# Amanda-Zheng/MR-GNAS

Hardware: AMD Instinct MI355X
Metric: million edges/sec per supernet fwd+bwd step (FB15k-237, dim=200) (higher is better)
Workload: dtype f32

## Files before the change

### include/mrgnas.h

```cpp
#ifndef MRGNAS_H
#define MRGNAS_H

#include <stdint.h>

#ifdef __cplusplus
extern "C" {
#endif

#define MRG_ABI_VERSION 23

#define MRG_OK            0
#define MRG_E_NULLPTR    -1
#define MRG_E_SHAPE      -2
#define MRG_E_ENUM       -3
#define MRG_E_WORKSPACE  -4

#define MRG_COMPOSE_MULT 0
#define MRG_COMPOSE_SUB  1
#define MRG_COMPOSE_ADD  2
#define MRG_REDUCE_SUM   0
#define MRG_REDUCE_MEAN  1
#define MRG_REDUCE_MAX   2
#define MRG_GCS_SUB      0
#define MRG_GCS_MUL      1
#define MRG_GCS_COPY     2
#define MRG_GCS_NEGS     3
#define MRG_GCS_CCORR    4
#define MRG_GCS_CCONV    5
#define MRG_ACT_NONE     0
#define MRG_ACT_RELU     1
#define MRG_ACT_SIGMOID  2

int mrg_abi_version(void);
const char *mrg_error_string(int code);
const char *mrg_target_arch(void);

int mrg_compose_fwd(int op, const float *s, const float *hr, float *out,
                    int64_t rows, int D, void *stream);
int mrg_compose_bwd(int op, const float *gout, const float *s, const float *hr,
                    float *gs, float *ghr, int64_t rows, int D, void *stream);

int mrg_gather_compose_fwd(int op, const float *ent, const float *rel,
                           const int32_t *ent_idx, const int32_t *rel_idx,
                           float *out, int64_t rows, int D, void *stream);

#define MRG_GATE_LD(D) (2 * (D) + 4)

int mrg_gate_collapse3(const float *const *W_host, const float *const *b_host, const float *const *a_host, float *uvc,
                       int D, int in_dim, int fold, void *stream);
int mrg_gate_param_grad3(const float *const *W_host, const float *const *b_host, const float *const *a_host,
                         const float *d_uvc, float *const *gW_host, float *const *gb_host, float *const *ga_host,
                         int D, int in_dim, int fold, void *stream);
int mrg_fold_halves3(const float *const *W_host, float *Wt, int D, void *stream);
int mrg_unfold_halves3(const float *const *gWt_host, float *const *gW_host, int D, void *stream);

int mrg_gate_fwd(const float *s, const float *s_in, const float *norm, const float *uvc,
                 float *out, int64_t b0, int64_t b1, int64_t M, int D, float scale, void *stream);
int64_t mrg_gate_bwd_workspace_bytes(int64_t M, int D);
int mrg_gate_bwd(const float *gout, const float *s, const float *s_in, const float *norm,
                 const float *uvc, float *gs, float *gs_in, float *d_uvc, void *ws,
                 int64_t b0, int64_t b1, int64_t M, int D, float scale, void *stream);
int mrg_gate_row_fwd(const float *s, const float *s_in, const float *norm, const float *uvc, float *fvec, float *hvec,
                     int64_t b0, int64_t b1, int64_t M, int D, float scale, void *stream);
int64_t mrg_gate_row_colsum_blocks(int64_t b0, int64_t b1, int64_t M, int D, int vec4);
int mrg_gate_row_fwd_colsum(const float *s, const float *s_in, const float *norm, const float *uvc, float *fvec, float *hvec,
                            int64_t b0, int64_t b1, int64_t M, int D, float scale, void *stream, double *colsum, int64_t colsum_blocks);
int mrg_gate_row_bwd(const float *q, const float *hvec, const float *s, const float *s_in, const float *uvc, float *gs_in, float *d_uvc,
                     void *ws, int64_t b0, int64_t b1, int64_t M, int D, void *stream);

int64_t mrg_seg_reduce_workspace_bytes(int64_t n_slots, int D);
int mrg_seg_reduce_fwd(int mode, const float *msg, const float *self_rows,
                       const int32_t *eid,
                       const int32_t *chunk_node, const int32_t *chunk_start, const int32_t *chunk_end,
                       const int32_t *chunk_slot, int64_t n_chunks,
                       const int32_t *hub_node, const int32_t *hub_first, const int32_t *hub_count, int64_t n_hubs,
                       int64_t n_slots, const int32_t *in_degree,
                       float *out, int32_t *arg, void *ws,
                       int64_t N, int D, void *stream);
int mrg_seg_reduce_bwd(int mode, const float *gout, const int32_t *dst, const int32_t *in_degree,
                       const int32_t *arg, float *gmsg, float *gself, const float *relu_src,
                       int64_t E, int64_t N, int D, void *stream);
int mrg_seg_reduce_bwd_ordered(int mode, const float *gout, const int32_t *dst, const int32_t *in_degree, const int32_t *arg,
                               float *gmsg, float *gself, const float *relu_src, const unsigned *relu_bits, const int32_t *order,
                               int64_t E, int64_t N, int D, void *stream);
int mrg_segmax_bwd_input_ok(int D, int Kin);
int mrg_segmax_bwd_input(const float *gout, const float *mx, const int32_t *dst, const int32_t *arg, const float *W, float *gmsg,
                         float *gx, const int32_t *order, int64_t E, int64_t N, int D, int Kin, void *stream);

int64_t mrg_seg_std_workspace_bytes(int64_t n_slots, int D);
int mrg_seg_std_fwd(const float *msg, const int32_t *eid, const int32_t *chunk_node, const int32_t *chunk_start,
                    const int32_t *chunk_end, const int32_t *chunk_slot, int64_t n_chunks, const int32_t *hub_node,
                    const int32_t *hub_first, const int32_t *hub_count, int64_t n_hubs, int64_t n_slots,
                    const int32_t *in_degree, float *out, float *mean, float *coef, void *ws, int64_t N, int D, void *stream);
int mrg_seg_std_bwd(const float *gout, const float *msg, const int32_t *dst, const float *mean, const float *coef,
                    const int32_t *order, float *gmsg, int64_t E, int64_t N, int D, void *stream);

int mrg_fused_gcs(int mode, const float *X, const int32_t *xi, const float *Y, const int32_t *yi,
                  const float *scal, const int32_t *eid,
                  const int32_t *chunk_node, const int32_t *chunk_start, const int32_t *chunk_end,
                  const int32_t *chunk_slot, int64_t n_chunks,
                  const int32_t *hub_node, const int32_t *hub_first, const int32_t *hub_count, int64_t n_hubs,
                  int64_t n_slots, const int32_t *seg_len,
                  float *out, void *ws, int64_t nseg, int D, void *stream);

int mrg_span_gcs(int mode, const float *X, const float *Y, const void *meta, const float *ext_scal, int64_t E, int span,
                 const int32_t *span_slot, const int32_t *span_start, int64_t n_spans,
                 const int32_t *hub_seg, const int32_t *hub_first, const int32_t *hub_count, int64_t n_hubs,
                 int64_t n_slots, const int32_t *seg_len,
                 float *out, void *ws, int64_t nseg, int D, void *stream);

int mrg_sum_buffers(const float *const *xs_host, int K, float *out, int64_t n, int accumulate, void *stream);
int mrg_sum_rows_gather(const float *const *xs_host, int K, const float *gather_edge, const float *gather_self,
                        const int32_t *dst, int64_t E, int64_t rows, int D, float *out, void *stream);

int mrg_distmult_score(const float *ent, const float *rel, const int32_t *s_idx, const int32_t *r_idx,
                       const int32_t *o_idx, float *score, int64_t T, int D, void *stream);

int64_t mrg_mix_workspace_bytes(int K, int D);

int mrg_optim_chunk(void);
int mrg_clip_sgd_step(void *const *params, const void *const *grads, void *const *bufs, const int32_t *chunk_tensor,
                      const int64_t *chunk_off, const int32_t *chunk_len, int64_t n_chunks, double *partial, float *norm_coef,
                      float max_norm, float lr, float momentum, float weight_decay, void *stream);
int mrg_adam_step(void *const *params, const void *const *grads, void *const *exp_avg, void *const *exp_avg_sq, int64_t n_tensors,
                  const int32_t *chunk_tensor, const int64_t *chunk_off, const int32_t *chunk_len, int64_t n_chunks, float *step,
                  float *scal, const float *lr, double beta1, double beta2, float eps, float weight_decay, void *stream);
#define MRG_MIX_MAX_CANDIDATES 8
typedef struct mrg_gated_branch {
  int32_t k;
  const float *s;
  const float *rowscale;
  int32_t row_k;
  const float *row_f;
  const float *row_h;
  const float *row_uvc;
  int32_t row_ld;
  int64_t b0, b1;
  float *row_dq;
  int32_t act;
  const int32_t *valid_rows;
  const double *given[MRG_MIX_MAX_CANDIDATES];
  int32_t given_n[MRG_MIX_MAX_CANDIDATES];
  int64_t given_stride[MRG_MIX_MAX_CANDIDATES];
} mrg_gated_branch;
int mrg_mix_colstats(const float *const *y_host, int K, int64_t rows, int D, double *sums, void *ws,
                     const mrg_gated_branch *gated, void *stream);
int mrg_mix_finalize_fwd(const double *sums, const float *const *gamma_host, const float *const *beta_host,
                         float *const *rmean_host, float *const *rvar_host, int K, double total_rows, int D,
                         float eps, float momentum, float *coef, void *stream);
int mrg_mix_stats_coef(const float *const *y, const float *const *gamma, const float *const *beta,
                       float *const *running_mean, float *const *running_var, int K, int64_t rows, double total_rows,
                       int D, float eps, float momentum, float *coef, void *ws, const mrg_gated_branch *gated, void *stream);
int mrg_mix_fwd(const float *const *y_host, int K, const float *coef, const float *w, const float *addend, float *out,
                int64_t rows, int D, const mrg_gated_branch *gated, void *stream);
int mrg_mix_bwd_reduce(const float *g, const float *const *y_host, int K, const float *coef, const float *w,
                       float *red, void *ws, int64_t rows, int D, const mrg_gated_branch *gated, void *stream);
int mrg_mix_finalize_bwd(const float *red, int K, double total_rows, int D, float *coef2,
                         float *const *dgamma_host, float *const *dbeta_host, float *dw, const int32_t *valid_rows, void *stream);
int mrg_mix_bwd_apply(const float *g, const float *const *y_host, float *const *gy_host, int K,
                      const float *coef, const float *coef2, const float *w, const float *const *rs, const float *rs_scale,
                      const float *rs_self, const int64_t *rs_edge_rows, const int *rs_on, const float *const *rs_full,
                      const float *const *fold_s,
                      const float *const *fold_gate, float *const *fold_gs, const int *fold_add_from, int64_t rows, int D,
                      const mrg_gated_branch *gated, void *stream);

int64_t mrg_zero_workspace_bytes(int D);
int mrg_zero_colstats(const float *ent, const float *rel, const int32_t *ent_idx, const int32_t *rel_idx, const int *ops, int K,
                      int64_t rows, int D, double *sums, void *ws, void *stream);
int mrg_zero_stats_coef(const float *ent, const float *rel, const int32_t *ent_idx, const int32_t *rel_idx, const int *ops, int K,
                        const float *const *gamma, const float *const *beta, float *const *running_mean,
                        float *const *running_var, int64_t rows, double total_rows, int D, float eps, float momentum,
                        float *coef, void *ws, const int32_t *valid_rows, void *stream);
int mrg_zero_fwd(const float *ent, const float *rel, const int32_t *ent_idx, const int32_t *rel_idx, const int *ops, int K,
                 const float *coef, const float *w, float *out, int64_t rows, int D, const int32_t *valid_rows, void *stream);
int mrg_zero_bwd_reduce(const float *g, const float *ent, const float *rel, const int32_t *ent_idx, const int32_t *rel_idx,
                        const int *ops, int K, const float *coef, const float *w, float *red, void *ws, int64_t rows, int D,
                        const int32_t *valid_rows, void *stream);
int mrg_zero_bwd_apply(const float *g, const float *ent, const float *rel, const int32_t *ent_idx, const int32_t *rel_idx,
                       const int *ops, int K, const float *coef, const float *coef2, const float *w, float *g_ent_rows,
                       float *g_rel_rows, int64_t rows, int D, const int32_t *valid_rows, void *stream);


int64_t mrg_gemm_workspace_bytes(int K, int Nout);
int mrg_gemm_set_mode(int mode);
int mrg_gemm_set_wide8(int on);
int mrg_gemm_set_q(int on);
int mrg_gemm_set_small(int on);
int mrg_wgrad_set_variant(int variant);
int mrg_linear_fwd(const float *X, const float *W, const float *bias, float *Y, void *ws,
                   int64_t rows, int K, int Nout, int act, void *stream);
int64_t mrg_linear_relu_segmax_workspace_bytes(int64_t N, int K, int Nout);
int mrg_linear_relu_segmax_fwd(const float *X, const float *W, const float *bias, const int32_t *eid, const int32_t *dst,
                               const float *self_rows, float *out, int32_t *arg, float *mx, void *ws,
                               int64_t E, int64_t N, int K, int Nout, void *stream);
int mrg_linear_relu_segsum_fwd(const float *X, const float *W, const float *bias, const int32_t *eid, const int32_t *dst,
                               float *part, unsigned *relu_bits, void *ws, int64_t E, int K, int Nout, void *stream);
int mrg_seg_reduce_heads_fwd(int mode, const float *part, const float *self_rows, const int32_t *rowptr,
                             const int32_t *chunk_node, const int32_t *chunk_start, const int32_t *chunk_end,
                             const int32_t *chunk_slot, int64_t n_chunks, const int32_t *hub_node, const int32_t *hub_first,
                             const int32_t *hub_count, int64_t n_hubs, int64_t n_slots, const int32_t *in_degree, float *out,
                             void *ws, int64_t N, int D, void *stream);
int mrg_seg_reduce_bwd_bits(int mode, const float *gout, const int32_t *dst, const int32_t *in_degree, float *gmsg, float *gself,
                            const unsigned *relu_bits, int64_t E, int64_t N, int D, void *stream);
int64_t mrg_linear_bwd_input_workspace_bytes(int K, int Nout);
int mrg_linear_bwd_input(const float *gY, const float *W, float *gX, void *ws,
                         int64_t rows, int K, int Nout, int ldw, int accumulate, void *stream);
int64_t mrg_linear_bwd_weight_workspace_bytes(int64_t rows, int K, int Nout);
int mrg_linear_bwd_weight(const float *gY, const float *X1, const float *X2, float *gW, float *gbias, void *ws,
                          int64_t rows, int K1, int K2, int Nout, void *stream);
int mrg_linear_bwd_weight_share(const float *gY, const float *X1, const float *X2, float *gW, float *gbias, void *ws,
                                int64_t rows, int K1, int K2, int Nout, int share, void *stream);

int mrg_dense_filter_fwd(int kind, const float *s, const float *s_in, const float *W, const float *bias,
                         const float *rowscale, float scale, float *out, float *gate, void *ws,
                         int64_t rows, int D, void *stream);
int64_t mrg_dense_filter3_workspace_bytes(int D, int K);
int mrg_dense_filter_fwd3(int kind, const float *s, const float *s_in, const float *const *W, const float *const *bias,
                          const float *norm, float scale_edge, float scale_self, float *out, float *gate, void *ws,
                          int64_t b0, int64_t b1, int64_t M, int D, void *stream);
int64_t mrg_dense_filter3_colsum_blocks(int kind, int64_t b0, int64_t b1, int64_t M, int D, int K);
int mrg_dense_filter_fwd3_colsum(int kind, const float *s, const float *s_in, const float *const *W, const float *const *bias,
                                 const float *norm, float scale_edge, float scale_self, float *out, float *gate, void *ws,
                                 int64_t b0, int64_t b1, int64_t M, int D, void *stream, double *colsum, int64_t colsum_blocks);
int mrg_dense_filter_dz3(int kind, const float *g, const float *s, const float *gate, const float *norm, float scale_edge,
                         float scale_self, float *dz, float *gs, int64_t b1, int64_t M, int D, void *stream);
int64_t mrg_linear_bwd_input3_workspace_bytes(int K, int Nout);
int mrg_linear_bwd_input3(const float *gY, const float *const *W, float *gX, void *ws, int64_t b0, int64_t b1, int64_t M,
                          int K, int Nout, int ldw, int accumulate, void *stream);
int64_t mrg_linear_bwd_input3_pair_workspace_bytes(int K, int Nout);
int mrg_linear_bwd_input3_pair(const float *gY1, const float *gY2, const float *const *W1, const float *const *W2, float *gX,
                               void *ws, int64_t b0, int64_t b1, int64_t M, int K, int Nout, int ldw, int accumulate,
                               void *stream);
int64_t mrg_linear_bwd_weight3_workspace_bytes(int64_t b0, int64_t b1, int64_t M, int K1, int K2, int Nout);
int mrg_linear_bwd_weight3(const float *gY, const float *X1, const float *X2, float *const *gW, float *const *gbias, void *ws,
                           int64_t b0, int64_t b1, int64_t M, int K1, int K2, int Nout, void *stream);
int mrg_dense_filter_dz(int kind, const float *g, const float *s, const float *gate, const float *rowscale,
                        float scale, float *dz, float *gs, int64_t rows, int D, void *stream);

int64_t mrg_build_graph_workspace_bytes(int64_t T);
int mrg_build_graph(const int64_t *triples, int64_t T, int64_t N, int R, int sorted,
                    const float *deg_norm_table, int64_t table_len,
                    int64_t *src, int64_t *dst, int64_t *etype, float *norm, int32_t *in_degree,
                    int32_t *src32, int32_t *dst32, int32_t *etype32, int32_t *max_degree,
                    void *ws, int64_t ws_bytes, void *stream);

int64_t mrg_plan_workspace_bytes(int64_t E, int64_t nseg, int span);
int mrg_span_plan_build(const int32_t *seg, int64_t E, int64_t nseg, int span, int snap,
                        int32_t *perm, int32_t *seg_sorted, int32_t *seg_len, int32_t *span_slot, int32_t *span_start,
                        int32_t *hub_seg, int32_t *hub_first, int32_t *hub_count, int32_t *counts,
                        void *ws, int64_t ws_bytes, void *stream);
int mrg_span_meta_pack(const int32_t *perm, const int32_t *seg_sorted, const int32_t *xi, const int32_t *yi,
                       const float *scal, int w_is_index, void *meta, int64_t E, void *stream);

int64_t mrg_chunk_plan_workspace_bytes(int64_t E, int64_t N);
int mrg_chunk_plan_build(const int32_t *dst, int64_t E, int64_t N, int chunk,
                         int32_t *eid, int32_t *rowptr, int32_t *in_degree,
                         int32_t *chunk_node, int32_t *chunk_start, int32_t *chunk_end, int32_t *chunk_slot,
                         int32_t *hub_node, int32_t *hub_first, int32_t *hub_count, int32_t *counts,
                         void *ws, int64_t ws_bytes, void *stream);

int mrg_negative_sampling(const int64_t *pos, int64_t B, int rate, const int64_t *values, const double *choices,
                          int64_t *samples, float *labels, void *stream);
int64_t mrg_sample_neighborhood_workspace_bytes(int64_t N, int64_t T);
int mrg_sample_edge_neighborhood(const int32_t *rowptr, const int32_t *adj_edge, const int32_t *adj_other, const int32_t *degrees,
                                 int64_t N, int64_t T, int64_t sample_size, const double *u_vertex, const int64_t *tries,
                                 int64_t n_tries, const double *u_edge, int32_t *edges, int64_t *status, void *ws,
                                 int64_t ws_bytes, void *stream);
int64_t mrg_relabel_workspace_bytes(int64_t num_nodes);
int mrg_relabel_nodes(const int64_t *src, const int64_t *dst, int64_t n, int64_t num_nodes, int64_t *uniq,
                      int64_t *new_src, int64_t *new_dst, int32_t *count, void *ws, int64_t ws_bytes, void *stream);
int mrg_multi_hot_labels(const int64_t *keys, const int32_t *rowptr, const int32_t *objs, const int64_t *query,
                         int64_t B, int64_t U, int64_t num_ent, float v_zero, float v_one, float *out, void *stream);

int64_t mrg_block_sizes_workspace_bytes(int64_t n_dst);
int mrg_block_sizes(const int32_t *rowptr, const int64_t *dst_nodes, int64_t n_dst, int64_t N, int k, int32_t *first, void *ws,
                    int64_t ws_bytes, void *stream);
int mrg_block_emit(const int32_t *rowptr, const int32_t *in_eid, const int32_t *in_src, const int32_t *in_type,
                   const int64_t *dst_nodes, const int32_t *first, int64_t n_dst, int64_t N, int k, const double *u, int64_t E,
                   int64_t *eid, int64_t *etype, int64_t *ldst, int32_t *gsrc, int32_t *local, int32_t *firstpos, void *stream);
int64_t mrg_block_relabel_workspace_bytes(int64_t E);
int mrg_block_relabel(const int32_t *gsrc, const int64_t *dst_nodes, int64_t n_dst, int64_t N, int64_t E, int32_t *local,
                      int32_t *firstpos, int64_t *src_nodes, int64_t *lsrc, int32_t *n_new, void *ws, int64_t ws_bytes, void *stream);

int mrg_rank_filtered(const float *pred, const float *labels, const int64_t *obj, int64_t B, int64_t N,
                      int64_t *ranks, void *stream);
int64_t mrg_distmult_rank_workspace_bytes(int64_t Q, int64_t N, int D);
int mrg_distmult_rank(const float *ent, const float *rel, const int32_t *a_idx, const int32_t *r_idx, const int32_t *t_idx,
                      const int64_t *qkey, const int32_t *when, const int64_t *keys, const int32_t *rowptr, const int32_t *members,
                      const int32_t *gone_at, int64_t U, int64_t Q, int64_t N, int D, int64_t *ranks, void *ws, int64_t ws_bytes,
                      void *stream);
int64_t mrg_distmult_bce_workspace_bytes(int64_t B, int64_t N, int D);
int mrg_distmult_bce_fwd(const float *q, const float *ent, const int64_t *qkey, const int64_t *keys, const int32_t *rowptr,
                         const int32_t *objs, int64_t U, float v_zero, float v_one, int64_t B, int64_t N, int D, float *loss,
                         void *ws, int64_t ws_bytes, void *stream);
int mrg_distmult_bce_dlogit(const float *q, const float *ent, const int64_t *qkey, const int64_t *keys, const int32_t *rowptr,
                            const int32_t *objs, int64_t U, float v_zero, float v_one, int64_t B, int64_t N, int D, int64_t c0,
                            int64_t c1, const float *gscale, float *dl, void *ws, int64_t ws_bytes, void *stream);
int mrg_rows_rank(const float *q, const float *ent, const int32_t *t_idx, const int64_t *qkey, const int32_t *when, const int64_t *keys,
                  const int32_t *rowptr, const int32_t *members, const int32_t *gone_at, int64_t U, int64_t Q, int64_t N, int D,
                  int64_t *ranks, void *ws, int64_t ws_bytes, void *stream);
int64_t mrg_transe_bce_workspace_bytes(int64_t B, int64_t ncols, int D);
int mrg_transe_bce_fwd(const float *obj, const float *ent, const int64_t *qkey, const int64_t *keys, const int32_t *rowptr,
                       const int32_t *objs, int64_t U, float gamma, float v_zero, float v_one, int64_t B, int64_t N, int D, float *loss,
                       void *ws, int64_t ws_bytes, void *stream);
int mrg_transe_bce_dlogit(const float *obj, const float *ent, const int64_t *qkey, const int64_t *keys, const int32_t *rowptr,
                          const int32_t *objs, int64_t U, float gamma, float v_zero, float v_one, int64_t B, int64_t N, int D,
                          int64_t c0, int64_t c1, const float *gscale, float *dl, void *ws, int64_t ws_bytes, void *stream);
int mrg_transe_dist_bwd(const float *ent_c, const float *obj, const float *dl, int64_t ld, float *gent_c, float *gobj, int accumulate,
                        int64_t B, int64_t nc, int D, void *stream);
int64_t mrg_transe_rank_workspace_bytes(int64_t Q, int64_t N, int D);
int mrg_transe_rank(const float *obj, const float *ent, const int32_t *t_idx, const int64_t *qkey, const int32_t *when,
                    const int64_t *keys, const int32_t *rowptr, const int32_t *members, const int32_t *gone_at, int64_t U, int64_t Q,
                    int64_t N, int D, int64_t *ranks, void *ws, int64_t ws_bytes, void *stream);
int mrg_transe_score_fwd(const float *ent, const float *sub, const float *rel, float gamma, float *score,
                         int64_t B, int64_t N, int D, void *stream);
// ... 50 lines not shown
```

### mr-gnas_amd/_lib.py

```python
import ctypes
import os
import re

import torch

_HERE = os.path.dirname(os.path.abspath(__file__))
LIB_PATH = os.environ.get("MRG_LIB_PATH") or os.path.join(_HERE, "lib", "libmrgnas_hip.so")
HEADER_PATH = os.path.join(os.path.dirname(_HERE), "include", "mrgnas.h")

ABI_VERSION = 23


class MrgnasLibraryError(RuntimeError):
    pass


class MrgnasError(RuntimeError):
    """A C-ABI call returned a non-zero code."""


_P, _I, _L, _F = ctypes.c_void_p, ctypes.c_int, ctypes.c_int64, ctypes.c_float

SIGNATURES = {
    "mrg_abi_version": (_I, []),
    "mrg_error_string": (ctypes.c_char_p, [_I]),
    "mrg_target_arch": (ctypes.c_char_p, []),
    "mrg_compose_fwd": (_I, [_I, _P, _P, _P, _L, _I, _P]),
    "mrg_compose_bwd": (_I, [_I, _P, _P, _P, _P, _P, _L, _I, _P]),
    "mrg_gather_compose_fwd": (_I, [_I, _P, _P, _P, _P, _P, _L, _I, _P]),
    "mrg_gate_collapse3": (_I, [_P, _P, _P, _P, _I, _I, _I, _P]),
    "mrg_gate_param_grad3": (_I, [_P, _P, _P, _P, _P, _P, _P, _I, _I, _I, _P]),
    "mrg_fold_halves3": (_I, [_P, _P, _I, _P]),
    "mrg_unfold_halves3": (_I, [_P, _P, _I, _P]),
    "mrg_gate_fwd": (_I, [_P, _P, _P, _P, _P, _L, _L, _L, _I, _F, _P]),
    "mrg_gate_bwd_workspace_bytes": (_L, [_L, _I]),
    "mrg_gate_bwd": (_I, [_P, _P, _P, _P, _P, _P, _P, _P, _P, _L, _L, _L, _I, _F, _P]),
    "mrg_seg_reduce_workspace_bytes": (_L, [_L, _I]),
    "mrg_seg_reduce_fwd": (_I, [_I, _P, _P, _P, _P, _P, _P, _P, _L, _P, _P, _P, _L, _L, _P, _P, _P, _P, _L, _I, _P]),
    "mrg_seg_reduce_bwd": (_I, [_I, _P, _P, _P, _P, _P, _P, _P, _L, _L, _I, _P]),
    "mrg_fused_gcs": (_I, [_I, _P, _P, _P, _P, _P, _P, _P, _P, _P, _P, _L, _P, _P, _P, _L, _L, _P, _P, _P, _L, _I, _P]),
    "mrg_span_gcs": (_I, [_I, _P, _P, _P, _P, _L, _I, _P, _P, _L, _P, _P, _P, _L, _L, _P, _P, _P, _L, _I, _P]),
    "mrg_sum_buffers": (_I, [_P, _I, _P, _L, _I, _P]),
    "mrg_sum_rows_gather": (_I, [_P, _I, _P, _P, _P, _L, _L, _I, _P, _P]),
    "mrg_distmult_score": (_I, [_P, _P, _P, _P, _P, _P, _L, _I, _P]),
    "mrg_gate_row_fwd": (_I, [_P, _P, _P, _P, _P, _P, _L, _L, _L, _I, _F, _P]),
    "mrg_gate_row_colsum_blocks": (_L, [_L, _L, _L, _I, _I]),
    "mrg_gate_row_fwd_colsum": (_I, [_P, _P, _P, _P, _P, _P, _L, _L, _L, _I, _F, _P, _P, _L]),
    "mrg_gate_row_bwd": (_I, [_P, _P, _P, _P, _P, _P, _P, _P, _L, _L, _L, _I, _P]),
    "mrg_mix_workspace_bytes": (_L, [_I, _I]),
    "mrg_mix_colstats": (_I, [_P, _I, _L, _I, _P, _P, _P, _P]),
    "mrg_mix_finalize_fwd": (_I, [_P, _P, _P, _P, _P, _I, ctypes.c_double, _I, _F, _F, _P, _P]),
    "mrg_mix_stats_coef": (_I, [_P, _P, _P, _P, _P, _I, _L, ctypes.c_double, _I, _F, _F, _P, _P, _P, _P]),
    "mrg_zero_workspace_bytes": (_L, [_I]),
    "mrg_zero_colstats": (_I, [_P, _P, _P, _P, _P, _I, _L, _I, _P, _P, _P]),
    "mrg_zero_stats_coef": (_I, [_P, _P, _P, _P, _P, _I, _P, _P, _P, _P, _L, ctypes.c_double, _I, _F, _F, _P, _P, _P, _P]),
    "mrg_zero_fwd": (_I, [_P, _P, _P, _P, _P, _I, _P, _P, _P, _L, _I, _P, _P]),
    "mrg_zero_bwd_reduce": (_I, [_P, _P, _P, _P, _P, _P, _I, _P, _P, _P, _P, _L, _I, _P, _P]),
    "mrg_zero_bwd_apply": (_I, [_P, _P, _P, _P, _P, _P, _I, _P, _P, _P, _P, _P, _L, _I, _P, _P]),
    "mrg_mix_fwd": (_I, [_P, _I, _P, _P, _P, _P, _L, _I, _P, _P]),
    "mrg_mix_bwd_reduce": (_I, [_P, _P, _I, _P, _P, _P, _P, _L, _I, _P, _P]),
    "mrg_mix_finalize_bwd": (_I, [_P, _I, ctypes.c_double, _I, _P, _P, _P, _P, _P, _P]),
    "mrg_mix_bwd_apply": (_I, [_P, _P, _P, _I, _P, _P, _P, _P, _P, _P, _P, _P, _P, _P, _P, _P, _P, _L, _I, _P, _P]),
    "mrg_dense_filter_fwd": (_I, [_I, _P, _P, _P, _P, _P, _F, _P, _P, _P, _L, _I, _P]),
    "mrg_dense_filter_dz": (_I, [_I, _P, _P, _P, _P, _F, _P, _P, _L, _I, _P]),
    "mrg_gemm_workspace_bytes": (_L, [_I, _I]),
    "mrg_gemm_set_mode": (_I, [_I]),
    "mrg_gemm_set_wide8": (_I, [_I]),
    "mrg_gemm_set_q": (_I, [_I]),
    "mrg_gemm_set_small": (_I, [_I]),
    "mrg_segmax_bwd_input_ok": (_I, [_I, _I]),
    "mrg_segmax_bwd_input": (_I, [_P, _P, _P, _P, _P, _P, _P, _P, _L, _L, _I, _I, _P]),
    "mrg_seg_std_workspace_bytes": (_L, [_L, _I]),
    "mrg_seg_std_fwd": (_I, [_P, _P, _P, _P, _P, _P, _L, _P, _P, _P, _L, _L, _P, _P, _P, _P, _P, _L, _I, _P]),
    "mrg_seg_std_bwd": (_I, [_P, _P, _P, _P, _P, _P, _P, _L, _L, _I, _P]),
    "mrg_optim_chunk": (_I, []),
    "mrg_clip_sgd_step": (_I, [_P, _P, _P, _P, _P, _P, _L, _P, _P, _F, _F, _F, _F, _P]),
    "mrg_adam_step": (_I, [_P, _P, _P, _P, _L, _P, _P, _P, _L, _P, _P, _P, ctypes.c_double, ctypes.c_double, _F, _F, _P]),
    "mrg_act_grad_transpose": (_I, [_P, _P, _P, _L, _L, _I, _P]),
    "mrg_wgrad_set_variant": (_I, [_I]),
    "mrg_linear_fwd": (_I, [_P, _P, _P, _P, _P, _L, _I, _I, _I, _P]),
    "mrg_dense_filter3_workspace_bytes": (_L, [_I, _I]),
    "mrg_dense_filter_fwd3": (_I, [_I, _P, _P, _P, _P, _P, _F, _F, _P, _P, _P, _L, _L, _L, _I, _P]),
    "mrg_dense_filter3_colsum_blocks": (_L, [_I, _L, _L, _L, _I, _I]),
    "mrg_dense_filter_fwd3_colsum": (_I, [_I, _P, _P, _P, _P, _P, _F, _F, _P, _P, _P, _L, _L, _L, _I, _P, _P, _L]),
    "mrg_dense_filter_dz3": (_I, [_I, _P, _P, _P, _P, _F, _F, _P, _P, _L, _L, _I, _P]),
    "mrg_linear_bwd_input3_workspace_bytes": (_L, [_I, _I]),
    "mrg_linear_bwd_input3": (_I, [_P, _P, _P, _P, _L, _L, _L, _I, _I, _I, _I, _P]),
    "mrg_linear_bwd_input3_pair_workspace_bytes": (_L, [_I, _I]),
    "mrg_linear_bwd_input3_pair": (_I, [_P, _P, _P, _P, _P, _P, _L, _L, _L, _I, _I, _I, _I, _P]),
    "mrg_linear_bwd_weight3_workspace_bytes": (_L, [_L, _L, _L, _I, _I, _I]),
    "mrg_linear_bwd_weight3": (_I, [_P, _P, _P, _P, _P, _P, _L, _L, _L, _I, _I, _I, _P]),
    "mrg_linear_relu_segsum_fwd": (_I, [_P, _P, _P, _P, _P, _P, _P, _P, _L, _I, _I, _P]),
    "mrg_seg_reduce_heads_fwd": (_I, [_I, _P, _P, _P, _P, _P, _P, _P, _L, _P, _P, _P, _L, _L, _P, _P, _P, _L, _I, _P]),
    "mrg_seg_reduce_bwd_bits": (_I, [_I, _P, _P, _P, _P, _P, _P, _L, _L, _I, _P]),
    "mrg_seg_reduce_bwd_ordered": (_I, [_I, _P, _P, _P, _P, _P, _P, _P, _P, _P, _L, _L, _I, _P]),
    "mrg_linear_relu_segmax_workspace_bytes": (_L, [_L, _I, _I]),
    "mrg_linear_relu_segmax_fwd": (_I, [_P, _P, _P, _P, _P, _P, _P, _P, _P, _P, _L, _L, _I, _I, _P]),
    "mrg_linear_bwd_input_workspace_bytes": (_L, [_I, _I]),
    "mrg_linear_bwd_input": (_I, [_P, _P, _P, _P, _L, _I, _I, _I, _I, _P]),
    "mrg_linear_bwd_weight_workspace_bytes": (_L, [_L, _I, _I]),
    "mrg_linear_bwd_weight": (_I, [_P, _P, _P, _P, _P, _P, _L, _I, _I, _I, _P]),
    "mrg_linear_bwd_weight_share": (_I, [_P, _P, _P, _P, _P, _P, _L, _I, _I, _I, _I, _P]),
    "mrg_build_graph_workspace_bytes": (_L, [_L]),
    "mrg_build_graph": (_I, [_P, _L, _L, _I, _I, _P, _L, _P, _P, _P, _P, _P, _P, _P, _P, _P, _P, _L, _P]),
    "mrg_plan_workspace_bytes": (_L, [_L, _L, _I]),
    "mrg_span_plan_build": (_I, [_P, _L, _L, _I, _I, _P, _P, _P, _P, _P, _P, _P, _P, _P, _P, _L, _P]),
    "mrg_span_meta_pack": (_I, [_P, _P, _P, _P, _P, _I, _P, _L, _P]),
    "mrg_chunk_plan_workspace_bytes": (_L, [_L, _L]),
    "mrg_chunk_plan_build": (_I, [_P, _L, _L, _I, _P, _P, _P, _P, _P, _P, _P, _P, _P, _P, _P, _P, _L, _P]),
    "mrg_negative_sampling": (_I, [_P, _L, _I, _P, _P, _P, _P, _P]),
    "mrg_sample_neighborhood_workspace_bytes": (_L, [_L, _L]),
    "mrg_sample_edge_neighborhood": (_I, [_P, _P, _P, _P, _L, _L, _L, _P, _P, _L, _P, _P, _P, _P, _L, _P]),
    "mrg_relabel_workspace_bytes": (_L, [_L]),
    "mrg_relabel_nodes": (_I, [_P, _P, _L, _L, _P, _P, _P, _P, _P, _L, _P]),
    "mrg_multi_hot_labels": (_I, [_P, _P, _P, _P, _L, _L, _L, _F, _F, _P, _P]),
    "mrg_rank_filtered": (_I, [_P, _P, _P, _L, _L, _P, _P]),
    "mrg_distmult_rank_workspace_bytes": (_L, [_L, _L, _I]),
    "mrg_distmult_rank": (_I, [_P, _P, _P, _P, _P, _P, _P, _P, _P, _P, _P, _L, _L, _L, _I, _P, _P, _L, _P]),
    "mrg_distmult_bce_workspace_bytes": (_L, [_L, _L, _I]),
    "mrg_distmult_bce_fwd": (_I, [_P, _P, _P, _P, _P, _P, _L, _F, _F, _L, _L, _I, _P, _P, _L, _P]),
    "mrg_distmult_bce_dlogit": (_I, [_P, _P, _P, _P, _P, _P, _L, _F, _F, _L, _L, _I, _L, _L, _P, _P, _P, _L, _P]),
    "mrg_rows_rank": (_I, [_P, _P, _P, _P, _P, _P, _P, _P, _P, _L, _L, _L, _I, _P, _P, _L, _P]),
    "mrg_transe_bce_workspace_bytes": (_L, [_L, _L, _I]),
    "mrg_transe_bce_fwd": (_I, [_P, _P, _P, _P, _P, _P, _L, _F, _F, _F, _L, _L, _I, _P, _P, _L, _P]),
    "mrg_transe_bce_dlogit": (_I, [_P, _P, _P, _P, _P, _P, _L, _F, _F, _F, _L, _L, _I, _L, _L, _P, _P, _P, _L, _P]),
    "mrg_transe_dist_bwd": (_I, [_P, _P, _P, _L, _P, _P, _I, _L, _L, _I, _P]),
    "mrg_transe_rank_workspace_bytes": (_L, [_L, _L, _I]),
    "mrg_transe_rank": (_I, [_P, _P, _P, _P, _P, _P, _P, _P, _P, _L, _L, _L, _I, _P, _P, _L, _P]),
    "mrg_transe_score_fwd": (_I, [_P, _P, _P, _F, _P, _L, _L, _I, _P]),
    "mrg_transe_score_bwd": (_I, [_P, _P, _P, _P, _P, _P, _P, _L, _L, _I, _P]),
    "mrg_ccorr_rows": (_I, [_I, _P, _P, _P, _L, _I, _P]),
    "mrg_ccorr_matrix": (_I, [_I, _P, _P, _I, _P]),
    "mrg_ccorr_matrix_grad": (_I, [_I, _P, _P, _I, _P]),
    "mrg_conve_fc_workspace_bytes": (_L, [_L, _L, _I]),
    "mrg_conve_bwd_workspace_bytes": (_L, [_L, _I, _I, _I]),
    "mrg_conve_bn0_fwd": (_I, [_P, _P, _L, _I, _P, _P, _I, _F, _F, _P, _P]),
    "mrg_conve_conv_fwd": (_I, [_I, _P, _P, _L, _I, _I, _I, _P, _P, _P, _P, _P, _I, _I, _P, _P]),
    "mrg_conve_bn1_fwd": (_I, [_P, _L, _I, _I, _P, _P, _P, _P, _P, _I, _F, _F, _P, _P, _P]),
    "mrg_conve_fc_fwd": (_I, [_P, _P, _P, _P, _P, _P, _L, _L, _I, _P]),
    "mrg_conve_fc_bwd": (_I, [_P, _P, _P, _P, _P, _P, _P, _P, _L, _L, _I, _P]),
    "mrg_conve_bn1_bwd": (_I, [_P, _P, _P, _P, _P, _P, _I, _L, _I, _I, _P, _P, _P]),
    "mrg_conve_conv_bwd": (_I, [_I, _P, _P, _L, _I, _I, _I, _P, _P, _P, _P, _I, _I, _P, _P, _P]),
    "mrg_conve_finish_bwd": (_I, [_I, _P, _P, _L, _I, _I, _I, _P, _P, _I, _P, _P, _P, _P, _P, _P, _P, _P]),
    "mrg_cand_linear_colsum_blocks": (_L, [_L, _I]),
    "mrg_cand_linear_workspace_bytes": (_L, [_I, _I]),
    "mrg_cand_linear_fwd": (_I, [_I, _P, _P, _P, _P, _P, _L, _I, _P, _P, _L]),
    "mrg_cand_linear_bwd_input": (_I, [_I, _P, _P, _P, _P, _L, _I, _P]),
    "mrg_block_sizes_workspace_bytes": (_L, [_L]),
    "mrg_block_sizes": (_I, [_P, _P, _L, _L, _I, _P, _P, _L, _P]),
    "mrg_block_emit": (_I, [_P, _P, _P, _P, _P, _P, _L, _L, _I, _P, _L, _P, _P, _P, _P, _P, _P, _P]),
    "mrg_block_relabel_workspace_bytes": (_L, [_L]),
    "mrg_block_relabel": (_I, [_P, _P, _L, _L, _L, _P, _P, _P, _P, _P, _P, _L, _P]),
}

_lib = None


def declared_symbols():
    with open(HEADER_PATH) as f:
        text = re.sub(r"/\*.*?\*/", "", f.read(), flags=re.S)
    return sorted(set(re.findall(r"\b(mrg_[a-z0-9_]+)\s*\(", text)))


def load():
    global _lib
    if _lib is not None:
        return _lib
    if not os.path.exists(LIB_PATH):
        raise MrgnasLibraryError(
            f"{LIB_PATH} not found: build it with `python -c 'import __graft_entry__ as g; g.build()'` "
            "(or `make -C mr-gnas_amd/csrc`). mr_gnas_amd has no CPU fallback.")
    lib = ctypes.CDLL(LIB_PATH)
    for name, (res, args) in SIGNATURES.items():
        fn = getattr(lib, name)
        fn.restype, fn.argtypes = res, args
    if lib.mrg_abi_version() != ABI_VERSION:
        raise MrgnasLibraryError(f"ABI version {lib.mrg_abi_version()} != expected {ABI_VERSION}; rebuild the library")
    _lib = lib
    return lib


class KernelMeter:

    def __init__(self):
        self.names = None
        self.records = {}

    def start(self, names=None):
        self.names = set(names) if names is not None else True
        self.records = {}

    def active(self, name):
        return self.names is not None and (self.names is True or name in self.names)

    def stop(self):
        torch.cuda.synchronize()
        out = {}
        for name, recs in self.records.items():
            ms = sum(a.elapsed_time(b) for a, b, _, _ in recs)
            out[name] = {"launches": len(recs), "ms": ms, "bytes": sum(r[2] for r in recs), "flops": sum(r[3] for r in recs)}
        self.names, self.records = None, {}
        return out


meter = KernelMeter()


_FN = {}
TRACE = os.environ.get("MRG_TRACE") == "1"


def _trace(name, args):
    import sys
    shown = [hex(a.value) if isinstance(a, ctypes.c_void_p) and a.value else ("NULL" if isinstance(a, ctypes.c_void_p) or a is None else a)
             for a in args]
    print(f"[mrg] {name} {shown}", file=sys.stderr, flush=True)


def call(name, args, nbytes=0, flops=0, symbol=None):
    sym = symbol or name
    fn = _FN.get(sym)
    if fn is None:
        fn = _FN[sym] = getattr(load(), sym)
    if TRACE:
        _trace(name, args)
        code = fn(*args)
        torch.cuda.synchronize()
        if code != 0:
            check(code, name)
        return
    if meter.names is not None and meter.active(name):
        a, b = torch.cuda.Event(enable_timing=True), torch.cuda.Event(enable_timing=True)
        a.record()
        code = fn(*args)
        b.record()
        meter.records.setdefault(name, []).append((a, b, nbytes, flops))
    else:
        code = fn(*args)
    if code != 0:
        check(code, name)


def check(code, what=""):
    if code != 0:
        msg = load().mrg_error_string(code).decode()
        raise MrgnasError(f"{what}: {msg} (code {code})")


def ptr(t):
    return None if t is None else ctypes.c_void_p(t.data_ptr())


def ptr_array(tensors):
    arr = (ctypes.c_void_p * len(tensors))()
    for i, t in enumerate(tensors):
        arr[i] = None if t is None else t.data_ptr()
    return arr


class GatedBranch(ctypes.Structure):
    _fields_ = [("k", ctypes.c_int32), ("s", ctypes.c_void_p), ("rowscale", ctypes.c_void_p),
                ("row_k", ctypes.c_int32), ("row_f", ctypes.c_void_p), ("row_h", ctypes.c_void_p), ("row_uvc", ctypes.c_void_p),
                ("row_ld", ctypes.c_int32), ("b0", ctypes.c_int64), ("b1", ctypes.c_int64), ("row_dq", ctypes.c_void_p),
                ("act", ctypes.c_int32), ("valid_rows", ctypes.c_void_p),
                ("given", ctypes.c_void_p * 8), ("given_n", ctypes.c_int32 * 8), ("given_stride", ctypes.c_int64 * 8)]


class ColSums:

    __slots__ = ("buf", "offset", "n", "stride", "rows")

    def __init__(self, buf, offset, n, stride, rows):
        self.buf, self.offset, self.n, self.stride, self.rows = buf, int(offset), int(n), int(stride), int(rows)


ACTS = {"relu": 0, "tanh": 1}


def gated_branch(spec, row_dq=None, act=0, valid_rows=None, given=None):
    dp = lambda t: None if t is None else t.data_ptr()
    if given is not None and not any(c is not None for c in given):
        given = None
    if spec is None:
        if not act and valid_rows is None and given is None:
            return None
        g = GatedBranch(-1, None, None, -1, None, None, None, 0, 0, 0, None, int(act), dp(valid_rows))
    else:
        g = GatedBranch(int(spec.get("k", -1)), dp(spec["s"]), dp(spec.get("c")), int(spec.get("row_k", -1)), dp(spec.get("row_f")),
                        dp(spec.get("row_h")), dp(spec.get("row_uvc")), int(spec.get("row_ld", 0)), int(spec.get("b0", 0)), int(spec.get("b1", 0)),
                        dp(row_dq), int(act), dp(valid_rows))
    for k, c in enumerate(given or ()):
        if c is not None:
            g.given[k], g.given_n[k], g.given_stride[k] = c.buf.data_ptr() + c.offset, c.n, c.stride
    return ctypes.byref(g)


_RAW_STREAM = getattr(torch._C, "_cuda_getCurrentRawStream", None) if os.environ.get("MRG_RAW_STREAM", "1") == "1" else None


def stream_of(t):
    if _RAW_STREAM is not None:
        return ctypes.c_void_p(_RAW_STREAM(t.device.index if t.device.index is not None else torch.cuda.current_device()))
    return ctypes.c_void_p(torch.cuda.current_stream(t.device).cuda_stream)
# ... 20 lines not shown
```

### mr-gnas_amd/csrc/gate.hip

```cpp
#include "common.hpp"

namespace mrg {

struct SegPlan {
  int64_t lo[3], hi[3];
  int blk[4];
};

static SegPlan make_plan(int64_t b0, int64_t b1, int64_t M, int grid) {
  SegPlan p;
  p.lo[0] = 0;  p.hi[0] = b0;
  p.lo[1] = b0; p.hi[1] = b1;
  p.lo[2] = b1; p.hi[2] = M;
  int nseg = 0;
  for (int s = 0; s < 3; ++s) nseg += (p.hi[s] > p.lo[s]);
  int spare = grid - nseg;
  p.blk[0] = 0;
  for (int s = 0; s < 3; ++s) {
    int64_t rows = p.hi[s] - p.lo[s];
    int nb = rows > 0 ? 1 + (int)((double)spare * (double)rows / (double)M) : 0;
    p.blk[s + 1] = p.blk[s] + nb;
  }
  return p;
}
// ... 222 lines not shown
        }
      }
    }
    const float z = group_sum<LPR>(dot) + cc;
    const float gt = sigmoidf_fast(z);
    const float nv = use_norm ? norm[r] : 1.0f;
    if (sl == 0) {
      fvec[r] = gt * scale * nv;
      const float t = scale * nv;
      hvec[r] = t * gt * (1.0f - gt);
    }
  }
}

template <int VEC, int LPR, bool HAS_IN>
__global__ __launch_bounds__(MRG_BLOCK) void gate_row_fwd_colsum_k(const float* __restrict__ s, const float* __restrict__ sin_,
                                                                   const float* __restrict__ norm, const float* __restrict__ uvc,
                                                                   float* __restrict__ fvec, float* __restrict__ hvec, SegPlan p, int D, float scale,
                                                                   double* __restrict__ colsum) {
  constexpr int RPB = MRG_BLOCK / LPR;
  constexpr int WIDTH = LPR * VEC;
  __shared__ double red[RPB * WIDTH];
  const int b = blockIdx.x;
  if (b >= p.blk[3]) return;
  const int seg = (b >= p.blk[1]) + (b >= p.blk[2]);
  const int jb = b - p.blk[seg], nb = p.blk[seg + 1] - p.blk[seg];
  const int sl = threadIdx.x % LPR, rw = row_group_of_thread<LPR>();
  const int dv = D / VEC;
  const float* u = uvc + (int64_t)seg * MRG_GATE_LD(D);
  const float cc = u[HAS_IN ? 2 * D : D];
  const bool mine = sl < dv;
  const Vec<VEC> uk = mine ? Vec<VEC>::load(u + sl * VEC) : Vec<VEC>::fill(0.f);
  const Vec<VEC> vk = (HAS_IN && mine) ? Vec<VEC>::load(u + D + sl * VEC) : Vec<VEC>::fill(0.f);
  const bool use_norm = norm != nullptr && seg < 2;
  double st[4][VEC];
#pragma unroll
  for (int q = 0; q < 4; ++q)
#pragma unroll
    for (int j = 0; j < VEC; ++j) st[q][j] = 0.0;
  for (int64_t r = p.lo[seg] + (int64_t)jb * RPB + rw; r < p.hi[seg]; r += (int64_t)nb * RPB) {
    float dot = 0.f;
    Vec<VEC> sk = Vec<VEC>::fill(0.f);
    if (mine) {
      sk = Vec<VEC>::load(s + r * D + sl * VEC);
#pragma unroll
      for (int j = 0; j < VEC; ++j) dot += sk[j] * uk[j];
      if (HAS_IN) {
        Vec<VEC> x = Vec<VEC>::load(sin_ + r * D + sl * VEC);
#pragma unroll
        for (int j = 0; j < VEC; ++j) dot += x[j] * vk[j];
      }
    }
    const float z = group_sum<LPR>(dot) + cc;
    const float gt = sigmoidf_fast(z);
    const float nv = use_norm ? norm[r] : 1.0f;
    const float rf = gt * scale * nv;
    if (sl == 0) {
      fvec[r] = rf;
      const float t = scale * nv;
      hvec[r] = t * gt * (1.0f - gt);
    }
#pragma unroll
    for (int j = 0; j < VEC; ++j) {
      double d = (double)sk[j]; st[0][j] += d; st[1][j] += d * d;
      d = (double)(sk[j] * rf); st[2][j] += d; st[3][j] += d * d;
    }
  }
  double* __restrict__ dst = colsum + (int64_t)b * 4 * D;
#pragma unroll
  for (int q = 0; q < 4; ++q) {
#pragma unroll
    for (int j = 0; j < VEC; ++j) red[rw * WIDTH + sl * VEC + j] = st[q][j];
    __syncthreads();
    for (int c = threadIdx.x; c < D; c += MRG_BLOCK) {
      double acc = 0.0;
#pragma unroll
      for (int g = 0; g < RPB; ++g) acc += red[g * WIDTH + c];
      dst[q * D + c] = acc;
    }
    __syncthreads();
  }
}

template <int VEC, int LPR, int KMAX, bool HAS_IN>
__global__ __launch_bounds__(MRG_BLOCK) void gate_row_bwd_k(const float* __restrict__ qv, const float* __restrict__ hv, const float* __restrict__ s,
                                                            const float* __restrict__ sin_, const float* __restrict__ uvc,
                                                            float* __restrict__ gsin, float* __restrict__ ws, SegPlan p, int D) {
  constexpr int RPB = MRG_BLOCK / LPR;
  constexpr int WIDTH = LPR * KMAX * VEC;
  __shared__ float red[RPB * (2 * WIDTH + 1)];
  const int b = blockIdx.x;
  if (b >= p.blk[3]) return;
  const int seg = (b >= p.blk[1]) + (b >= p.blk[2]);
  const int jb = b - p.blk[seg], nb = p.blk[seg + 1] - p.blk[seg];
  const int sl = threadIdx.x % LPR, rw = row_group_of_thread<LPR>();
  const int dv = D / VEC;
  const int ld = MRG_GATE_LD(D);
  const int cidx = HAS_IN ? 2 * D : D;
  const float* u = uvc + (int64_t)seg * ld;
  Vec<VEC> vk[KMAX], du[KMAX], dvv[KMAX];
  double dc = 0.0;
#pragma unroll
  for (int k = 0; k < KMAX; ++k) {
    int c = sl + k * LPR;
    vk[k] = (HAS_IN && c < dv) ? Vec<VEC>::load(u + D + c * VEC) : Vec<VEC>::fill(0.f);
    du[k] = Vec<VEC>::fill(0.f);
    dvv[k] = Vec<VEC>::fill(0.f);
  }
  for (int64_t r = p.lo[seg] + (int64_t)jb * RPB + rw; r < p.hi[seg]; r += (int64_t)nb * RPB) {
    const float dz = qv[r] * hv[r];
    dc += (double)dz;
#pragma unroll
    for (int k = 0; k < KMAX; ++k) {
      int c = sl + k * LPR;
      if (c < dv) {
        const Vec<VEC> sk = Vec<VEC>::load(s + r * D + c * VEC);
#pragma unroll
        for (int j = 0; j < VEC; ++j) du[k][j] += dz * sk[j];
        if (HAS_IN) {
          const Vec<VEC> xk = Vec<VEC>::load(sin_ + r * D + c * VEC);
          Vec<VEC> o2;
#pragma unroll
          for (int j = 0; j < VEC; ++j) {
            o2[j] = dz * vk[k][j];
            dvv[k][j] += dz * xk[j];
          }
          o2.store(gsin + r * D + c * VEC);
        }
      }
    }
  }
  float* mine = red + rw * (2 * WIDTH + 1);
#pragma unroll
  for (int k = 0; k < KMAX; ++k) {
    int c = sl + k * LPR;
#pragma unroll
    for (int j = 0; j < VEC; ++j) {
      mine[c * VEC + j] = du[k][j];
      mine[WIDTH + c * VEC + j] = dvv[k][j];
    }
  }
  if (sl == 0) mine[2 * WIDTH] = (float)dc;
  __syncthreads();
  float* dst = ws + (int64_t)b * ld;
  for (int t = threadIdx.x; t < ld; t += MRG_BLOCK) {
    int srcidx = t < D ? t : ((HAS_IN && t < 2 * D) ? WIDTH + (t - D) : (t == cidx ? 2 * WIDTH : -1));
    double acc = 0.0;
    if (srcidx >= 0) {
#pragma unroll
      for (int q = 0; q < RPB; ++q) acc += (double)red[q * (2 * WIDTH + 1) + srcidx];
    }
    dst[t] = (float)acc;
  }
}

__global__ void gate_reduce_k(const float* __restrict__ ws, float* __restrict__ d_uvc, SegPlan p, int ld) {
  int seg = blockIdx.y;
  int t = blockIdx.x * blockDim.x + threadIdx.x;
  if (t >= ld) return;
  double acc = 0.0;
  for (int b = p.blk[seg]; b < p.blk[seg + 1]; ++b) acc += (double)ws[(int64_t)b * ld + t];
  d_uvc[seg * ld + t] = (float)acc;
}

}

using namespace mrg;

struct Ptr3 { const float* p[3]; };
struct MPtr3 { float* p[3]; };

__global__ void gate_collapse3_k(Ptr3 W, Ptr3 b, Ptr3 a, float* __restrict__ uvc, int D, int in_dim, int fold) {
  __shared__ float part[16][64];
  const int seg = blockIdx.y;
  const int tx = threadIdx.x & 63, ty = threadIdx.x >> 6;
  const int k = blockIdx.x * 64 + tx;
  const int width = fold ? D : in_dim;
  float* out = uvc + (int64_t)seg * MRG_GATE_LD(D);
  const float* Ws = W.p[seg];
  const float* as = a.p[seg];
  const float* bs = b.p[seg];
  float acc = 0.f;
  if (Ws != nullptr) {
    if (k < width) {
      for (int j = ty; j < D; j += 16) {
        float w = Ws[(int64_t)j * in_dim + k];
        if (fold) w += Ws[(int64_t)j * in_dim + k + D];
        acc += w * as[j];
      }
    } else if (k == width && bs) {
      for (int j = ty; j < D; j += 16) acc += as[j] * bs[j];
    }
  }
  part[ty][tx] = acc;
  __syncthreads();
  if (ty == 0 && k <= width) {
    float tot = part[0][tx];
#pragma unroll
    for (int i = 1; i < 16; ++i) tot += part[i][tx];
    out[k] = tot;
  }
}

__global__ void gate_param_grad3_k(Ptr3 W, Ptr3 b, Ptr3 a, const float* __restrict__ d_uvc, MPtr3 gW, MPtr3 gb, MPtr3 ga, int D, int in_dim,
                                   int fold) {
  __shared__ float part[MRG_BLOCK / MRG_WAVE];
  const int seg = blockIdx.y, j = blockIdx.x;
  const float* Ws = W.p[seg];
  if (Ws == nullptr) return;
// ... 113 lines not shown
extern "C" int mrg_gate_bwd(const float* gout, const float* s, const float* s_in, const float* norm, const float* uvc,
                            float* gs, float* gs_in, float* d_uvc, void* ws, int64_t b0, int64_t b1, int64_t M, int D,
                            float scale, void* stream) {
  if (D <= 0 || M < 0 || b0 < 0 || b1 < b0 || M < b1) return MRG_E_SHAPE;
  if (!uvc || !d_uvc) return MRG_E_NULLPTR;
  if (M > 0 && (!gout || !s || !gs)) return MRG_E_NULLPTR;
  if (s_in && !gs_in) return MRG_E_NULLPTR;
  if (!ws) return MRG_E_WORKSPACE;
  hipStream_t st = (hipStream_t)stream;
  const int ld = MRG_GATE_LD(D);
  RowGeom g = row_geom(D, aligned16(gout) && aligned16(s) && aligned16(s_in) && aligned16(gs) && aligned16(gs_in) && aligned16(uvc));
  if (!g.ok) return MRG_E_SHAPE;
  SegPlan p{};
#define CALL(V, L, K)                                                                                                   \
  do {                                                                                                                  \
    int grid = grid_for(M, (MRG_BLOCK / L) * 4);                                                                               \
    if (grid < 3) grid = 3;                                                                                             \
    p = make_plan(b0, b1, M, grid);                                                                                     \
    if (M > 0) {                                                                                                        \
      if (s_in) hipLaunchKernelGGL((gate_bwd_k<V, L, K, true, gate_rpt(L)>), dim3(p.blk[3]), dim3(MRG_BLOCK), 0, st, gout, s, s_in, norm, uvc, gs, gs_in, (float*)ws, p, D, scale); \
      else hipLaunchKernelGGL((gate_bwd_k<V, L, K, false, gate_rpt(L)>), dim3(p.blk[3]), dim3(MRG_BLOCK), 0, st, gout, s, s_in, norm, uvc, gs, gs_in, (float*)ws, p, D, scale); \
    }                                                                                                                   \
  } while (0)
  MRG_DISPATCH_GEOM(g, CALL);
#undef CALL
  MRG_LAUNCH_CHECK();
  launch_ordered_reduce_ranges<float>((const float*)ws, d_uvc, p.blk, 3, ld, ld, ld, st);
  MRG_LAUNCH_CHECK();
  return MRG_OK;
}

static int gate_row_plan(int64_t b0, int64_t b1, int64_t M, int lpr, SegPlan* p) {
  int grid = grid_for(M, (MRG_BLOCK / lpr) * 4);
  if (grid < 3) grid = 3;
  *p = make_plan(b0, b1, M, grid);
  return p->blk[3];
}

static int gate_row_fwd(const float* s, const float* s_in, const float* norm, const float* uvc, float* fvec, float* hvec,
                        int64_t b0, int64_t b1, int64_t M, int D, float scale, void* stream, double* colsum, int64_t colsum_blocks) {
  if (D <= 0 || M < 0 || b0 < 0 || b1 < b0 || M < b1) return MRG_E_SHAPE;
  if (M == 0) return MRG_OK;
  if (!s || !uvc || !fvec || !hvec) return MRG_E_NULLPTR;
  RowGeom g = row_geom(D, aligned16(s) && aligned16(s_in) && aligned16(uvc));
  if (!g.ok) return MRG_E_SHAPE;
  if (colsum && g.kmax != 1) return MRG_E_SHAPE;
  hipStream_t st = (hipStream_t)stream;
#define CALL(V, L, K)                                                                                                   \
  do {                                                                                                                  \
    SegPlan p;                                                                                                          \
    gate_row_plan(b0, b1, M, L, &p);                                                                                    \
    if (colsum && p.blk[3] != colsum_blocks) return MRG_E_SHAPE;     \
    if (colsum) {                                                                                                       \
      if (s_in) hipLaunchKernelGGL((gate_row_fwd_colsum_k<V, L, true>), dim3(p.blk[3]), dim3(MRG_BLOCK), 0, st, s, s_in, norm, uvc, fvec, hvec, p, D, scale, colsum); \
      else hipLaunchKernelGGL((gate_row_fwd_colsum_k<V, L, false>), dim3(p.blk[3]), dim3(MRG_BLOCK), 0, st, s, s_in, norm, uvc, fvec, hvec, p, D, scale, colsum); \
    } else if (s_in) hipLaunchKernelGGL((gate_row_fwd_k<V, L, K, true>), dim3(p.blk[3]), dim3(MRG_BLOCK), 0, st, s, s_in, norm, uvc, fvec, hvec, p, D, scale); \
    else hipLaunchKernelGGL((gate_row_fwd_k<V, L, K, false>), dim3(p.blk[3]), dim3(MRG_BLOCK), 0, st, s, s_in, norm, uvc, fvec, hvec, p, D, scale); \
  } while (0)
  MRG_DISPATCH_GEOM(g, CALL);
#undef CALL
  MRG_LAUNCH_CHECK();
  return MRG_OK;
}

extern "C" int mrg_gate_row_fwd(const float* s, const float* s_in, const float* norm, const float* uvc, float* fvec, float* hvec,
                                int64_t b0, int64_t b1, int64_t M, int D, float scale, void* stream) {
  return gate_row_fwd(s, s_in, norm, uvc, fvec, hvec, b0, b1, M, D, scale, stream, nullptr, 0);
}

extern "C" int64_t mrg_gate_row_colsum_blocks(int64_t b0, int64_t b1, int64_t M, int D, int vec4) {
  if (D <= 0 || M <= 0 || b0 < 0 || b1 < b0 || M < b1) return 0;
  RowGeom g = row_geom(D, vec4 != 0);
  if (!g.ok || g.kmax != 1 || (vec4 && g.vec != 4)) return 0;
  SegPlan p;
  return gate_row_plan(b0, b1, M, g.lpr, &p);
}

extern "C" int mrg_gate_row_fwd_colsum(const float* s, const float* s_in, const float* norm, const float* uvc, float* fvec, float* hvec,
                                       int64_t b0, int64_t b1, int64_t M, int D, float scale, void* stream, double* colsum, int64_t colsum_blocks) {
  if (!colsum) return MRG_E_NULLPTR;
  return gate_row_fwd(s, s_in, norm, uvc, fvec, hvec, b0, b1, M, D, scale, stream, colsum, colsum_blocks);
}

extern "C" int mrg_gate_row_bwd(const float* q, const float* hvec, const float* s, const float* s_in, const float* uvc, float* gs_in, float* d_uvc,
                                void* ws, int64_t b0, int64_t b1, int64_t M, int D, void* stream) {
  if (D <= 0 || M < 0 || b0 < 0 || b1 < b0 || M < b1) return MRG_E_SHAPE;
  if (!uvc || !d_uvc) return MRG_E_NULLPTR;
  if (M > 0 && (!q || !hvec || !s)) return MRG_E_NULLPTR;
  if (s_in && !gs_in) return MRG_E_NULLPTR;
  if (!ws) return MRG_E_WORKSPACE;
  hipStream_t st = (hipStream_t)stream;
  const int ld = MRG_GATE_LD(D);
  RowGeom g = row_geom(D, aligned16(s) && aligned16(s_in) && aligned16(gs_in) && aligned16(uvc));
  if (!g.ok) return MRG_E_SHAPE;
  SegPlan p{};
#define CALL(V, L, K)                                                                                                   \
  do {                                                                                                                  \
    int grid = grid_for(M, (MRG_BLOCK / L) * 4);                                                                        \
    if (grid < 3) grid = 3;                                                                                             \
    p = make_plan(b0, b1, M, grid);                                                                                     \
    if (M > 0) {                                                                                                        \
      if (s_in) hipLaunchKernelGGL((gate_row_bwd_k<V, L, K, true>), dim3(p.blk[3]), dim3(MRG_BLOCK), 0, st, q, hvec, s, s_in, uvc, gs_in, (float*)ws, p, D); \
      else hipLaunchKernelGGL((gate_row_bwd_k<V, L, K, false>), dim3(p.blk[3]), dim3(MRG_BLOCK), 0, st, q, hvec, s, s_in, uvc, gs_in, (float*)ws, p, D); \
    }                                                                                                                   \
  } while (0)
  MRG_DISPATCH_GEOM(g, CALL);
#undef CALL
  MRG_LAUNCH_CHECK();
  launch_ordered_reduce_ranges<float>((const float*)ws, d_uvc, p.blk, 3, ld, ld, ld, st);
  MRG_LAUNCH_CHECK();
  return MRG_OK;
}
```

### mr-gnas_amd/csrc/gemm.hpp

```cpp
#pragma once
#include "common.hpp"

namespace mrg {

typedef float f32x16 __attribute__((ext_vector_type(16)));
typedef float v4f __attribute__((ext_vector_type(4)));
typedef __attribute__((address_space(3))) void* lds_ptr_t;
typedef const __attribute__((address_space(1))) void* gbl_ptr_t;

constexpr int GBM_MAX = 256;

enum { EPI_BIAS_ACT = 0, EPI_GATE = 1, EPI_SCALE = 2, EPI_ACCUM = 3, EPI_SEGMAX = 4, EPI_SEGSUM = 5 };
enum { EPI_GATE_SUMS = 6, EPI_SCALE_SUMS = 7 };
constexpr bool epi_sums(int epi) { return epi == EPI_GATE_SUMS || epi == EPI_SCALE_SUMS; }
constexpr int epi_base(int epi) { return epi == EPI_GATE_SUMS ? EPI_GATE : (epi == EPI_SCALE_SUMS ? EPI_SCALE : epi); }
enum { EPI_RANK = 8, EPI_RANK_DIAG = 9 };
constexpr bool epi_diag(int epi) { return epi == EPI_RANK_DIAG; }
enum { EPI_BCE = 10, EPI_BCE_GRAD = 11 };

struct GemmGroups {
  int n;
  int tile0[4];
  int64_t lo[3], hi[3];
  int64_t bp_stride;
  const float* bias[3];
  float scale[3];
  int use_rowscale[3];
};
inline int gemm_group_tiles(GemmGroups& g, int gbm) {
  g.tile0[0] = 0;
  for (int i = 0; i < 3; ++i) {
    const int64_t r = i < g.n && g.hi[i] > g.lo[i] ? g.hi[i] - g.lo[i] : 0;
    g.tile0[i + 1] = g.tile0[i] + (int)((r + gbm - 1) / gbm);
  }
  return g.tile0[3];
}

struct GemmArgs {
  const float* A1; const float* A2;
  int K1, K2;
  const float* B; int ldb;
  const float* bias;
  float* C; int ldc; int N;
  int64_t rows;
  int act;
  const float* S; int ld_s;
  const float* rowscale; float scale;
  float* aux;
  const float* Cin; int ld_cin;
  const int32_t* row_index;
  const int32_t* row_seg;
  unsigned long long* seg_out;
  float* seg_part;
  unsigned* relu_bits; int bits_ld;
  int pad0;
  int wave_lds_floats;
  GemmGroups grp;
};

inline void gemm_set_colsum(GemmArgs& a, double* colsum) { a.seg_part = reinterpret_cast<float*>(colsum); }
__host__ __device__ __forceinline__ double* gemm_colsum(const GemmArgs& a) { return reinterpret_cast<double*>(a.seg_part); }

template <bool DUAL>
__device__ __forceinline__ const float* gemm_a_ptr(const float* r1, const float* r2, int K1, int K2, int K, int k) {
  if (DUAL) {
    const bool first = k < K1;
    const int kk = first ? k : k - K1, ld = first ? K1 : K2;
    return (first ? r1 : r2) + (kk + 4 <= ld ? kk : ld - 4);
  }
  return r1 + (k + 4 <= K ? k : K - 4);
}

struct RankEpi {
  const float* tscore;
  float* tscore_out;
  const int32_t* qinfo;
  const int32_t* members;
  const int32_t* gone_at;
  unsigned* counts;
};
inline void gemm_set_rank(GemmArgs& a, const RankEpi& r) {
  a.S = r.tscore; a.aux = r.tscore_out; a.row_seg = r.qinfo;
  a.Cin = reinterpret_cast<const float*>(r.members); a.rowscale = reinterpret_cast<const float*>(r.gone_at); a.relu_bits = r.counts;
}
__device__ __forceinline__ RankEpi gemm_rank(const GemmArgs& a) {
  return RankEpi{a.S, a.aux, a.row_seg, reinterpret_cast<const int32_t*>(a.Cin), reinterpret_cast<const int32_t*>(a.rowscale), a.relu_bits};
}

template <int NT>
__device__ __forceinline__ void gemm_epilogue_rank(const GemmArgs& a, f32x16 (&acc)[NT], int64_t rowbase, int col0, int li, int lh) {
  if (rowbase >= a.rows) return;
  const RankEpi k = gemm_rank(a);
  float ts[16];
  int tg[16];
#pragma unroll
  for (int r = 0; r < 16; ++r) {
    const int64_t row = rowbase + (r & 3) + 8 * (r >> 2) + 4 * lh;
    const int64_t rc = row < a.rows ? row : a.rows - 1;
    ts[r] = k.tscore[rc];
    tg[r] = k.qinfo[rc * 4];
  }
  const int lane = lh * 32 + li;
  unsigned word[NT];
#pragma unroll
  for (int n = 0; n < NT; ++n) {
    const int col = col0 + n * 32 + li;
    const bool cok = col < a.N;
    unsigned w = 0;
#pragma unroll
    for (int r = 0; r < 16; ++r) {
      const float x = acc[n][r];
      const bool hit = cok && col != tg[r] && (x > ts[r] || (x == ts[r] && col < tg[r]));
      const unsigned long long ball = __ballot(hit);
      const int rl = (r & 3) + 8 * (r >> 2);
      w = lane == rl ? (unsigned)ball : (lane == rl + 4 ? (unsigned)(ball >> 32) : w);
    }
    word[n] = w;
  }
  const int64_t row = rowbase + lane;
  if (lane >= 32 || row >= a.rows) return;
  const int4 qi = *reinterpret_cast<const int4*>(k.qinfo + row * 4);
  const int hi = qi.z, when = qi.w;
  if (qi.y < hi) {
    const int cend = col0 + NT * 32;
    int b = qi.y, e = hi;
    while (b < e) {
      const int mid = b + ((e - b) >> 1);
      if (k.members[mid] < col0) b = mid + 1; else e = mid;
    }
    for (; b < hi; ++b) {
      const int m = k.members[b];
      if (m >= cend) break;
      if (k.gone_at[b] > when) {
        const int d = m - col0;
#pragma unroll
        for (int n = 0; n < NT; ++n) word[n] &= ~((d >> 5) == n ? 1u << (d & 31) : 0u);
      }
    }
  }
  unsigned cnt = 0;
#pragma unroll
  for (int n = 0; n < NT; ++n) cnt += __popc(word[n]);
// ... 212 lines not shown
  }
}

template <bool VEC4>
__device__ __forceinline__ float4 gemm_raw4(const float* __restrict__ base, int64_t row, int64_t nrows, int k, int K, int ld) {
  const int64_t rc = row < nrows ? row : nrows - 1;
  const float* p = base + rc * ld;
  if (VEC4) {
    const int kc = k + 4 <= K ? k : (K >= 4 ? K - 4 : 0);
    return *reinterpret_cast<const float4*>(p + kc);
  }
  const int km = K - 1;
  return make_float4(p[k < K ? k : km], p[k + 1 < K ? k + 1 : km], p[k + 2 < K ? k + 2 : km], p[k + 3 < K ? k + 3 : km]);
}

template <bool VEC4>
__device__ __forceinline__ float4 gemm_mask4(float4 v, int64_t row, int64_t nrows, int k, int K) {
  const bool rv = row < nrows;
  if (VEC4) {
    const bool ok = rv && k + 4 <= K;
    v.x = ok ? v.x : 0.f; v.y = ok ? v.y : 0.f; v.z = ok ? v.z : 0.f; v.w = ok ? v.w : 0.f;
  } else {
    v.x = (rv && k < K) ? v.x : 0.f; v.y = (rv && k + 1 < K) ? v.y : 0.f;
    v.z = (rv && k + 2 < K) ? v.z : 0.f; v.w = (rv && k + 3 < K) ? v.w : 0.f;
  }
  return v;
}

struct ASel { const float* base; int ld, kk; };
__device__ __forceinline__ ASel gemm_sel_a(const GemmArgs& a, int k) {
  const bool first = k < a.K1 || a.K2 == 0;
  ASel s;
  s.base = first ? a.A1 : a.A2;
  s.ld = first ? a.K1 : a.K2;
  s.kk = first ? k : k - a.K1;
  return s;
}

template <bool VEC4>
__device__ __forceinline__ float4 gemm_raw_a(const GemmArgs& a, int64_t row, int k) {
  if (VEC4) {
    const ASel sa = gemm_sel_a(a, k);
    return gemm_raw4<true>(sa.base, row, a.rows, sa.kk, sa.ld, sa.ld);
  }
  const int64_t rc = row < a.rows ? row : a.rows - 1;
  float v[4];
#pragma unroll
  for (int j = 0; j < 4; ++j) {
    const ASel sa = gemm_sel_a(a, k + j);
    const int kc = sa.kk < sa.ld ? sa.kk : sa.ld - 1;
    v[j] = sa.base[rc * sa.ld + kc];
  }
  return make_float4(v[0], v[1], v[2], v[3]);
}

template <bool VEC4>
__device__ __forceinline__ float4 gemm_mask_a(float4 v, const GemmArgs& a, int64_t row, int k) {
  if (VEC4) {
    const ASel sa = gemm_sel_a(a, k);
    return gemm_mask4<true>(v, row, a.rows, sa.kk, sa.ld);
  }
  const int K = a.K1 + a.K2;
  const bool rv = row < a.rows;
  v.x = (rv && k < K) ? v.x : 0.f; v.y = (rv && k + 1 < K) ? v.y : 0.f;
  v.z = (rv && k + 2 < K) ? v.z : 0.f; v.w = (rv && k + 3 < K) ? v.w : 0.f;
  return v;
}

template <int NT, int EPI, bool SUMS = false>
__device__ __forceinline__ void gemm_epilogue(const GemmArgs& a, f32x16 (&acc)[NT], int64_t rowbase, int col0, int li, int lh,
                                              bool full, double* __restrict__ sums = nullptr) {
  static_assert(!SUMS || EPI == EPI_GATE || EPI == EPI_SCALE, "column sums: gate and scale epilogues only");
  if (rowbase >= a.rows) {
    if constexpr (SUMS) {
#pragma unroll
      for (int n = 0; n < NT; ++n) { sums[(lh * 2 + 0) * NT * 32 + n * 32 + li] = 0.0; sums[(lh * 2 + 1) * NT * 32 + n * 32 + li] = 0.0; }
    }
    return;
  }
  const int last = (int)((a.rows - 1 - rowbase) < 31 ? (a.rows - 1 - rowbase) : 31);
  const int colw = col0 + li < a.N ? col0 + li : a.N - 1;
  float* crow[16];
  const float* srow[16];
  float* xrow[16];
  float cs[16];
  bool rok[16];
  const bool cstore = EPI != EPI_GATE || a.C != nullptr;
#pragma unroll
  for (int r = 0; r < 16; ++r) {
    const int row = (r & 3) + 8 * (r >> 2) + 4 * lh;
    const int rc = row < last ? row : last;
    rok[r] = row <= last;
    crow[r] = a.C + (rowbase + rc) * a.ldc + colw;
    if (EPI == EPI_GATE) srow[r] = a.S + (rowbase + rc) * a.ld_s + colw;
    if (EPI == EPI_ACCUM) srow[r] = a.Cin + (rowbase + rc) * a.ld_cin + colw;
    if (EPI == EPI_GATE) xrow[r] = a.aux ? a.aux + (rowbase + rc) * a.N + colw : nullptr;
    cs[r] = 1.0f;
    if (EPI == EPI_GATE || EPI == EPI_SCALE) cs[r] = a.scale * (a.rowscale ? a.rowscale[rowbase + rc] : 1.0f);
  }
#pragma unroll
  for (int n = 0; n < NT; ++n) {
    const int col = col0 + n * 32 + li;
    const bool cok = col < a.N;
    const int off = cok ? n * 32 : 0;
    const float bv = a.bias ? a.bias[cok ? col : colw] : 0.f;
    float in[16], v[16], g[16];
#pragma unroll
    for (int r = 0; r < 16; ++r) in[r] = 0.f;
    if ((EPI == EPI_GATE && (cstore || SUMS)) || EPI == EPI_ACCUM) {
#pragma unroll
      for (int r = 0; r < 16; ++r) in[r] = srow[r][off];
    }
#pragma unroll
    for (int r = 0; r < 16; ++r) {
      float x = acc[n][r] + bv;
      if (EPI == EPI_BIAS_ACT) {
        v[r] = (a.act == MRG_ACT_RELU) ? (x > 0.f ? x : 0.f) : (a.act == MRG_ACT_SIGMOID ? sigmoidf_fast(x) : x);
      } else if (EPI == EPI_GATE) {
        g[r] = sigmoidf_fast(x);
        v[r] = g[r] * in[r] * cs[r];
      } else if (EPI == EPI_SCALE) {
        v[r] = x * cs[r];
      } else {
        v[r] = x + in[r];
      }
    }
    if constexpr (SUMS) {
      double s1 = 0.0, s2 = 0.0;
#pragma unroll
      for (int r = 0; r < 16; ++r) {
        const double d = (full || rok[r]) ? (double)v[r] : 0.0;
        s1 += d; s2 += d * d;
      }
      sums[(lh * 2 + 0) * NT * 32 + n * 32 + li] = cok ? s1 : 0.0;
      sums[(lh * 2 + 1) * NT * 32 + n * 32 + li] = cok ? s2 : 0.0;
    }
    if (full) {
      if (cok) {
        if (cstore) {
#pragma unroll
          for (int r = 0; r < 16; ++r) crow[r][n * 32] = v[r];
        }
        if (EPI == EPI_GATE && a.aux) {
#pragma unroll
          for (int r = 0; r < 16; ++r) xrow[r][n * 32] = g[r];
        }
      }
    } else {
#pragma unroll
      for (int r = 0; r < 16; ++r) {
        if (cok && rok[r]) {
          if (cstore) crow[r][n * 32] = v[r];
          if (EPI == EPI_GATE && a.aux) xrow[r][n * 32] = g[r];
        }
      }
    }
  }
}

template <int W, int NSLOT>
__device__ __forceinline__ void gemm_colsum_flush(const double* __restrict__ lds, double* __restrict__ colsum, int N, int col0) {
  double* __restrict__ dst = colsum + (int64_t)blockIdx.x * 2 * N;
  for (int t = threadIdx.x; t < 2 * W; t += blockDim.x) {
    const int which = t / W, c = t - which * W;
    if (col0 + c >= N) continue;
    double acc = 0.0;
#pragma unroll
    for (int q = 0; q < NSLOT; ++q) acc += lds[(q * 2 + which) * W + c];
    dst[which * N + col0 + c] = acc;
  }
}

template <int NT, int MT, int GBK, int EPI, bool VEC4>
__global__ __launch_bounds__(MRG_BLOCK, (MT == 1 ? 2 : 1)) void rowgemm_k(GemmArgs a) {
  constexpr int GBM = 128 * MT;
  constexpr int GLD = GBK + 4;
  constexpr int F4R = GBK / 4;
  constexpr int NA = GBM * F4R / MRG_BLOCK;
  constexpr int NBT = NT * 32 * F4R;
  constexpr int NB = (NBT + MRG_BLOCK - 1) / MRG_BLOCK;
  extern __shared__ __align__(16) float smem[];
  constexpr int A_TILE = GBM * GLD, B_TILE = NT * 32 * GLD, STAGE = A_TILE + B_TILE;
  const int tid = threadIdx.x, wave = tid >> 6, lane = tid & 63, li = lane & 31, lh = lane >> 5;
  const int64_t row0 = (int64_t)blockIdx.x * GBM;
  const int col0 = (epi_diag(EPI) ? blockIdx.x : blockIdx.y) * (NT * 32);
  const int K = a.K1 + a.K2;
  const int nkt = (K + GBK - 1) / GBK;

  f32x16 acc[MT][NT];
#pragma unroll
  for (int m = 0; m < MT; ++m)
#pragma unroll
    for (int n = 0; n < NT; ++n)
#pragma unroll
      for (int r = 0; r < 16; ++r) acc[m][n][r] = 0.f;

  float4 pa[NA];
  float4 pb[NB];
  auto fetch = [&](int k0) {
#pragma unroll
    for (int i = 0; i < NA; ++i) {
      int f = tid + i * MRG_BLOCK;
      pa[i] = gemm_raw_a<VEC4>(a, row0 + f / F4R, k0 + (f % F4R) * 4);
    }
#pragma unroll
// ... 269 lines not shown
```

### mr-gnas_amd/csrc/gemm_x3q.hpp

```cpp
#pragma once
#include "gemm_x3.hpp"

namespace mrg {

constexpr int X3Q_CHUNK = X3Q_HT * 3 * 1024;
constexpr int X3Q_ROWS = 64;

inline size_t x3q_bsplit_bytes(int K) { return (size_t)x3q_slabs(K) * 2 * X3Q_CHUNK; }

template <int EPI, bool SUMS = false>
__device__ __forceinline__ void gemm_epilogue_q(const GemmArgs& a, f32x4v (&acc)[X3Q_NT], int64_t rowbase, int li, int lh, bool full,
                                                double* __restrict__ sums = nullptr) {
  static_assert(!SUMS || EPI == EPI_GATE || EPI == EPI_SCALE, "column sums: gate and scale epilogues only");
  constexpr int W = X3Q_HT * 32;
  if (rowbase >= a.rows) {
    if constexpr (SUMS) {
#pragma unroll
      for (int j = 0; j < X3Q_HT; ++j) { sums[(lh * 2 + 0) * W + j * 32 + li] = 0.0; sums[(lh * 2 + 1) * W + j * 32 + li] = 0.0; }
    }
    return;
  }
  const int last = (int)((a.rows - 1 - rowbase) < 15 ? (a.rows - 1 - rowbase) : 15);
  const int colw = li < a.N ? li : a.N - 1;
  float* crow[8];
  const float* srow[8];
  float* xrow[8];
  float cs[8];
  bool rok[8];
  const bool cstore = EPI != EPI_GATE || a.C != nullptr;
#pragma unroll
  for (int i = 0; i < 8; ++i) {
    const int row = i + 8 * lh;
    const int rc = row < last ? row : last;
    rok[i] = row <= last;
    crow[i] = a.C + (rowbase + rc) * a.ldc + colw;
    if (EPI == EPI_GATE) srow[i] = a.S + (rowbase + rc) * a.ld_s + colw;
    if (EPI == EPI_ACCUM) srow[i] = a.Cin + (rowbase + rc) * a.ld_cin + colw;
    if (EPI == EPI_GATE) xrow[i] = a.aux ? a.aux + (rowbase + rc) * a.N + colw : nullptr;
    cs[i] = 1.0f;
    if (EPI == EPI_GATE || EPI == EPI_SCALE) cs[i] = a.scale * (a.rowscale ? a.rowscale[rowbase + rc] : 1.0f);
  }
  const int lc = li & 15;
#pragma unroll
  for (int j = 0; j < X3Q_HT; ++j) {
    const int ca = (2 * j) * 16 + lc, cb = (2 * j + 1) * 16 + lc;
    const float bva = a.bias ? a.bias[ca < a.N ? ca : a.N - 1] : 0.f;
    const float bvb = a.bias ? a.bias[cb < a.N ? cb : a.N - 1] : 0.f;
    float acc8[8];
#pragma unroll
    for (int r = 0; r < 4; ++r) {
      float xa = acc[2 * j][r] + bva, xb = acc[2 * j + 1][r] + bvb;
      asm volatile("s_nop 1\n\tv_permlane16_swap_b32 %0, %1" : "+v"(xa), "+v"(xb));
      acc8[r] = xa;
      acc8[4 + r] = xb;
    }
    const int col = j * 32 + li;
    const bool cok = col < a.N;
    const int off = cok ? j * 32 : 0;
    float in[8], v[8], g[8];
#pragma unroll
    for (int i = 0; i < 8; ++i) in[i] = 0.f;
    if ((EPI == EPI_GATE && (cstore || SUMS)) || EPI == EPI_ACCUM) {
#pragma unroll
      for (int i = 0; i < 8; ++i) in[i] = srow[i][off];
    }
#pragma unroll
    for (int i = 0; i < 8; ++i) {
      const float x = acc8[i];
      if (EPI == EPI_BIAS_ACT) {
        v[i] = (a.act == MRG_ACT_RELU) ? (x > 0.f ? x : 0.f) : (a.act == MRG_ACT_SIGMOID ? sigmoidf_fast(x) : x);
      } else if (EPI == EPI_GATE) {
        g[i] = sigmoidf_fast(x);
        v[i] = g[i] * in[i] * cs[i];
      } else if (EPI == EPI_SCALE) {
        v[i] = x * cs[i];
      } else {
        v[i] = x + in[i];
      }
    }
    if constexpr (SUMS) {
      double s1 = 0.0, s2 = 0.0;
#pragma unroll
      for (int i = 0; i < 8; ++i) {
        const double d = (full || rok[i]) ? (double)v[i] : 0.0;
        s1 += d; s2 += d * d;
      }
      sums[(lh * 2 + 0) * W + j * 32 + li] = cok ? s1 : 0.0;
      sums[(lh * 2 + 1) * W + j * 32 + li] = cok ? s2 : 0.0;
    }
    if (full) {
      if (cok) {
        if (cstore) {
#pragma unroll
          for (int i = 0; i < 8; ++i) crow[i][j * 32] = v[i];
        }
        if (EPI == EPI_GATE && a.aux) {
#pragma unroll
          for (int i = 0; i < 8; ++i) xrow[i][j * 32] = g[i];
        }
      }
    } else {
#pragma unroll
      for (int i = 0; i < 8; ++i) {
        if (cok && rok[i]) {
          if (cstore) crow[i][j * 32] = v[i];
          if (EPI == EPI_GATE && a.aux) xrow[i][j * 32] = g[i];
        }
      }
    }
  }
}

constexpr int X3Q_WPS = 3;

template <int EPI, bool DUAL>
__global__ __launch_bounds__(256, X3Q_WPS) void rowgemm_x3q_k(GemmArgs a, const char* __restrict__ Bp) {
  constexpr int NCH = X3Q_HT * 3;
  constexpr int NBW = (NCH + 3) / 4;
  extern __shared__ __align__(16) char smem_q[];
  const int tid = threadIdx.x, wave = __builtin_amdgcn_readfirstlane(tid >> 6), lane = tid & 63;
  const int lr = lane & 15, lg = lane >> 4;
  MRG_GROUP_SELECT(X3Q_ROWS)
  const int64_t roww = row0 + wave * 16;
  const int K = a.K1 + a.K2;
  const int nslab = (K + 31) >> 5;

  f32x4v acc[X3Q_NT];
#pragma unroll
  for (int n = 0; n < X3Q_NT; ++n)
#pragma unroll
    for (int r = 0; r < 4; ++r) acc[n][r] = 0.f;

  const float* ar1; const float* ar2;
  x3_a_row(a, roww + lr, ar1, ar2);
  v4f xr[2][2];
  auto load_a = [&](int slab, v4f (&x)[2]) { x3_load_a<32, DUAL>(x, slab, nslab, lg, ar1, ar2, a.K1, a.K2, K); };
  auto fetch_b = [&](int c) { x3_fetch_b<NCH>(Bq + (int64_t)c * X3Q_CHUNK, smem_q + (c & 1) * X3Q_CHUNK, wave, lane); };
  const unsigned lds0 = (unsigned)(size_t)(lds_ptr_t)smem_q + (unsigned)lane * 16u;
  u32x4 bq[2][3];
  auto read_b = [&](int t, int buf, u32x4 (&q)[3]) { x3_read_b(lds0 + (unsigned)(buf * X3Q_CHUNK + t * 3072), q); };
  u32x4 ch, cm, cl, nh, nm, nl;
  load_a(0, xr[0]);
  fetch_b(0);
  fetch_b(1);
  load_a(1, xr[1]);
  asm volatile("s_waitcnt vmcnt(%0)" ::"n"(NBW + 2) : "memory");
  __builtin_amdgcn_sched_barrier(0);
#pragma unroll
  for (int q = 0; q < 4; ++q) split_pair_of(xr[0], q, ch, cm, cl);
  __builtin_amdgcn_s_barrier();

  auto half_slab = [&](auto half_c, auto split_c, const v4f (&xn)[2]) {
    constexpr int HF = decltype(half_c)::value;
    constexpr bool SPLIT = decltype(split_c)::value;
    read_b(0, HF, bq[0]);
#pragma unroll
// ... 80 lines not shown
```

### mr-gnas_amd/csrc/linear.hip

```cpp
#include "gemm_dispatch.hpp"

namespace mrg {

__global__ void segmax_finalize_k(const unsigned long long* __restrict__ keys, const float* __restrict__ self_rows,
                                  const int32_t* __restrict__ eid, float* __restrict__ out, int32_t* __restrict__ arg,
                                  float* __restrict__ mx, int64_t total) {
  for (int64_t i = (int64_t)blockIdx.x * blockDim.x + threadIdx.x; i < total; i += (int64_t)gridDim.x * blockDim.x) {
    const unsigned long long k = keys[i];
    const unsigned lo = (unsigned)k;
    const float v = __uint_as_float((unsigned)(k >> 32));
    out[i] = self_rows ? v + self_rows[i] : v;
    if (arg) arg[i] = lo == 0u ? -1 : eid[0xFFFFFFFFu - lo];
    if (mx) mx[i] = v;
  }
}

}

using namespace mrg;

static bool segmax_shape_ok(int K, int Nout) { return K > 48 && K % 4 == 0 && Nout > 0; }

extern "C" int64_t mrg_linear_relu_segmax_workspace_bytes(int64_t N, int K, int Nout) {
  if (N < 0 || !segmax_shape_ok(K, Nout) || gemm_mode() == 1) return 0;
// ... 28 lines not shown
  hipLaunchKernelGGL(segmax_finalize_k, dim3(stream_grid_for(total, 256 * 4)), dim3(256), 0, st, keys, self_rows, eid, out, arg, mx, total);
  MRG_LAUNCH_CHECK();
  return MRG_OK;
}

extern "C" int mrg_linear_relu_segsum_fwd(const float* X, const float* W, const float* bias, const int32_t* eid, const int32_t* dst,
                                          float* part, unsigned* relu_bits, void* ws, int64_t E, int K, int Nout, void* stream) {
  if (E < 0 || K <= 0 || Nout <= 0 || E >= ((int64_t)1 << 31)) return MRG_E_SHAPE;
  if (!segmax_shape_ok(K, Nout)) return MRG_E_SHAPE;
  if (E == 0) return MRG_OK;
  if (!X || !W || !eid || !dst || !part) return MRG_E_NULLPTR;
  if (!ws) return MRG_E_WORKSPACE;
  if (!aligned16(X) || !aligned16(ws)) return MRG_E_SHAPE;
  hipStream_t st = (hipStream_t)stream;
  GemmArgs a{};
  a.A1 = X; a.K1 = K; a.B = W; a.bias = bias; a.N = Nout; a.rows = E; a.act = MRG_ACT_RELU;
  a.row_index = eid; a.row_seg = dst; a.seg_part = part; a.relu_bits = relu_bits; a.bits_ld = (Nout + 31) / 32;
  if (!x3_eligible(a)) return MRG_E_SHAPE;
  launch_bsplit_any(EPI_SEGSUM, E, W, K, 1, Nout, K, ws, st);
  return launch_rowgemm_x3_mode<EPI_SEGSUM>(a, ws, st);
}

extern "C" int64_t mrg_gemm_workspace_bytes(int K, int Nout) {
  if (K <= 0 || Nout <= 0) return 0;
  return (int64_t)gemm_workspace_bytes(K, Nout);
}

extern "C" int mrg_gemm_set_mode(int mode) {
  if (mode < 0 || mode > 2) return MRG_E_ENUM;
  gemm_switches().mode = mode;
  return MRG_OK;
}

extern "C" int mrg_gemm_set_wide8(int on) {
  if (on < 0 || on > 1) return MRG_E_ENUM;
  gemm_switches().wide8 = on;
  return MRG_OK;
}

extern "C" int mrg_gemm_set_small(int on) {
  if (on < 0 || on > 1) return MRG_E_ENUM;
  gemm_switches().small_rows = on ? X3N_MAX_ROWS : 0;
  return MRG_OK;
}

extern "C" int mrg_gemm_set_q(int on) {
  if (on < 0 || on > 2) return MRG_E_ENUM;
  gemm_switches().q = on;
  return MRG_OK;
}

extern "C" int mrg_linear_fwd(const float* X, const float* W, const float* bias, float* Y, void* ws, int64_t rows, int K, int Nout,
                              int act, void* stream) {
  if (rows < 0 || K <= 0 || Nout <= 0) return MRG_E_SHAPE;
  if (act != MRG_ACT_NONE && act != MRG_ACT_RELU && act != MRG_ACT_SIGMOID) return MRG_E_ENUM;
  if (rows == 0) return MRG_OK;
  if (!X || !W || !Y) return MRG_E_NULLPTR;
  GemmArgs a{};
  a.A1 = X; a.K1 = K; a.B = W; a.bias = bias; a.C = Y; a.ldc = Nout; a.N = Nout; a.rows = rows; a.act = act;
  return launch_gemm<EPI_BIAS_ACT>(a, K, 1, ws, (hipStream_t)stream);
}

extern "C" int64_t mrg_linear_bwd_input_workspace_bytes(int K, int Nout) {
  if (K <= 0 || Nout <= 0) return 0;
  return (int64_t)gemm_workspace_bytes(Nout, K);
}

extern "C" int mrg_linear_bwd_input(const float* gY, const float* W, float* gX, void* ws, int64_t rows, int K, int Nout,
                                    int ldw, int accumulate, void* stream) {
  if (rows < 0 || K <= 0 || Nout <= 0 || ldw < K) return MRG_E_SHAPE;
  if (rows == 0) return MRG_OK;
  if (!gY || !W || !gX) return MRG_E_NULLPTR;
  if (!ws) return MRG_E_WORKSPACE;
  hipStream_t st = (hipStream_t)stream;
  GemmArgs a{};
  a.A1 = gY; a.K1 = Nout; a.B = W; a.C = gX; a.ldc = K; a.N = K; a.rows = rows; a.act = MRG_ACT_NONE;
  if (accumulate) {
    a.Cin = gX; a.ld_cin = K;
    return launch_gemm<EPI_ACCUM>(a, 1, ldw, ws, st);
  }
  return launch_gemm<EPI_BIAS_ACT>(a, 1, ldw, ws, st);
}

static size_t bwd_input3_each(int K, int Nred) { return (size_t)(((int64_t)bsplit_bytes_any(K, Nred) + 255) / 256 * 256); }

static int bwd_input3(const float* gY1, const float* gY2, const float* const* W1_host, const float* const* W2_host, float* gX, void* ws,
                      int64_t b0, int64_t b1, int64_t M, int K, int Nout, int ldw, int accumulate, hipStream_t st) {
  const bool pair = gY2 != nullptr;
  const int Nred = pair ? 2 * Nout : Nout;
  GemmArgs a{};
  a.A1 = gY1; a.K1 = Nout; a.C = gX; a.ldc = K; a.N = K; a.rows = M; a.act = MRG_ACT_NONE;
  if (pair) { a.A2 = gY2; a.K2 = Nout; }
  if (accumulate) { a.Cin = gX; a.ld_cin = K; }
  if (!x3_eligible(a)) return MRG_E_SHAPE;
  const int64_t lo[3] = {0, b0, b1}, hi[3] = {b0, b1, M};
  const size_t each = bwd_input3_each(K, Nred);
  const float* Bs[3]; const float* Bs2[3]; void* outs[3];
  a.grp.n = 3;
  a.grp.bp_stride = (int64_t)each;
  for (int i = 0; i < 3; ++i) {
    const bool live = hi[i] > lo[i];
    if (live && (!W1_host[i] || (pair && !W2_host[i]))) return MRG_E_NULLPTR;
    Bs[i] = live ? W1_host[i] : nullptr;
    Bs2[i] = live && pair ? W2_host[i] : nullptr;
    outs[i] = (char*)ws + i * each;
    a.grp.lo[i] = lo[i]; a.grp.hi[i] = live ? hi[i] : lo[i];
    a.grp.scale[i] = 1.0f;
  }
  launch_bsplit3_any(accumulate ? EPI_ACCUM : EPI_BIAS_ACT, M, Bs, 1, ldw, K, Nred, outs, st, pair ? Bs2 : nullptr, pair ? Nout : 0);
  MRG_LAUNCH_CHECK();
  if (accumulate) return launch_rowgemm_x3_mode<EPI_ACCUM>(a, outs[0], st);
  return launch_rowgemm_x3_mode<EPI_BIAS_ACT>(a, outs[0], st);
}

extern "C" int64_t mrg_linear_bwd_input3_workspace_bytes(int K, int Nout) {
  if (K <= 0 || Nout <= 48 || Nout % 4 != 0 || gemm_mode() == 1) return 0;
  return 3 * (int64_t)bwd_input3_each(K, Nout);
}

extern "C" int mrg_linear_bwd_input3(const float* gY, const float* const* W_host, float* gX, void* ws, int64_t b0, int64_t b1, int64_t M,
                                     int K, int Nout, int ldw, int accumulate, void* stream) {
  if (K <= 0 || Nout <= 0 || ldw < K || M < 0 || b0 < 0 || b1 < b0 || M < b1) return MRG_E_SHAPE;
  if (K <= 0 || Nout <= 48 || Nout % 4 != 0) return MRG_E_SHAPE;
  if (M == 0) return MRG_OK;
  if (!gY || !W_host || !gX) return MRG_E_NULLPTR;
  if (!ws) return MRG_E_WORKSPACE;
  return bwd_input3(gY, nullptr, W_host, nullptr, gX, ws, b0, b1, M, K, Nout, ldw, accumulate, (hipStream_t)stream);
}

extern "C" int64_t mrg_linear_bwd_input3_pair_workspace_bytes(int K, int Nout) {
  if (K <= 0 || Nout <= 24 || Nout % 4 != 0 || gemm_mode() == 1) return 0;
  return 3 * (int64_t)bwd_input3_each(K, 2 * Nout);
}

extern "C" int mrg_linear_bwd_input3_pair(const float* gY1, const float* gY2, const float* const* W1_host, const float* const* W2_host, float* gX,
                                          void* ws, int64_t b0, int64_t b1, int64_t M, int K, int Nout, int ldw, int accumulate, void* stream) {
  if (K <= 0 || Nout <= 24 || Nout % 4 != 0 || ldw < K || M < 0 || b0 < 0 || b1 < b0 || M < b1) return MRG_E_SHAPE;
  if (M == 0) return MRG_OK;
  if (!gY1 || !gY2 || !W1_host || !W2_host || !gX) return MRG_E_NULLPTR;
  if (!ws) return MRG_E_WORKSPACE;
  return bwd_input3(gY1, gY2, W1_host, W2_host, gX, ws, b0, b1, M, K, Nout, ldw, accumulate, (hipStream_t)stream);
}
```

### mr-gnas_amd/csrc/segreduce.hip

```cpp
#include "segcommon.hpp"

namespace mrg {

__device__ __forceinline__ bool seg_is_head(int j, int list_start) {
  const int q = j & 31;
  const int prev = (q & 3) ? j - 1 : (q >= 8 ? j - 5 : -1);
  return prev < list_start;
}

template <int VEC, int LPR, int KMAX, bool IS_MAX, bool HEADS = false>
__global__ __launch_bounds__(MRG_BLOCK) void seg_chunk_k(const float* __restrict__ msg, const float* __restrict__ self_rows,
                                                         const int32_t* __restrict__ eid, const int32_t* __restrict__ chunk_node,
                                                         const int32_t* __restrict__ chunk_start, const int32_t* __restrict__ chunk_end,
                                                         const int32_t* __restrict__ chunk_slot, int64_t n_chunks,
                                                         const int32_t* __restrict__ in_degree, float* __restrict__ out,
                                                         int32_t* __restrict__ arg, float* __restrict__ ws_val,
                                                         int32_t* __restrict__ ws_arg, int D, int is_mean,
                                                         const int32_t* __restrict__ head_rowptr = nullptr) {
  constexpr int RPB = MRG_BLOCK / LPR;
  constexpr int U = 4;
  const int sl = threadIdx.x % LPR, rw = row_group_of_thread<LPR>();
  const int dv = D / VEC;
  for (int64_t ch = (int64_t)blockIdx.x * RPB + rw; ch < n_chunks; ch += (int64_t)gridDim.x * RPB) {
    const int v = chunk_node[ch];
// ... 14 lines not shown
#pragma unroll
      for (int q = 0; q < U; ++q) {
#pragma unroll
        for (int k = 0; k < KMAX; ++k) {
          int c = sl + k * LPR;
          if (e[q] >= 0 && c < dv) x[q][k] = Vec<VEC>::load(msg + (int64_t)e[q] * D + c * VEC);
        }
      }
#pragma unroll
      for (int q = 0; q < U; ++q) {
        if (e[q] >= 0) {
#pragma unroll
          for (int k = 0; k < KMAX; ++k) {
            if (sl + k * LPR < dv) acc.take(k, x[q][k], e[q]);
          }
        }
      }
    }
    if (slot < 0) {
      finalize_row<VEC, LPR, KMAX, IS_MAX>(acc, v, in_degree[v], is_mean != 0, self_rows, out, arg, D, sl);
    } else {
#pragma unroll
      for (int k = 0; k < KMAX; ++k) {
        int c = sl + k * LPR;
        if (c < dv) {
          acc.val[k].store(ws_val + (int64_t)slot * D + c * VEC);
          if (IS_MAX) acc.arg[k].store(ws_arg + (int64_t)slot * D + c * VEC);
        }
      }
    }
  }
}

template <int VEC, int LPR, int KMAX, int MODE>
__global__ __launch_bounds__(MRG_BLOCK) void seg_bwd_k(const float* __restrict__ gout, const int32_t* __restrict__ dst,
                                                       const int32_t* __restrict__ in_degree, const int32_t* __restrict__ arg,
                                                       float* __restrict__ gmsg, float* __restrict__ gself,
                                                       const float* __restrict__ relu_src, int64_t E, int64_t rows, int D,
                                                       const unsigned* __restrict__ relu_bits = nullptr,
                                                       const int32_t* __restrict__ order = nullptr) {
  constexpr int RPB = MRG_BLOCK / LPR;
  const int sl = threadIdx.x % LPR, rw = row_group_of_thread<LPR>();
  const int dv = D / VEC;
  for (int64_t pos = (int64_t)blockIdx.x * RPB + rw; pos < rows; pos += (int64_t)gridDim.x * RPB) {
    const bool edge = pos < E;
    const int64_t r = (edge && order) ? (int64_t)order[pos] : pos;
    const int64_t v = edge ? dst[r] : r - E;
    float inv = 1.0f;
    if (MODE == MRG_REDUCE_MEAN && edge) { int d = in_degree[v]; inv = (float)(d > 1 ? d : 1); }
    float* o = edge ? gmsg + r * D : gself + (r - E) * D;
#pragma unroll
    for (int k = 0; k < KMAX; ++k) {
      int c = sl + k * LPR;
      if (c < dv) {
        Vec<VEC> g = Vec<VEC>::load(gout + v * D + c * VEC);
        if (edge) {
          if (MODE == MRG_REDUCE_MEAN) {
#pragma unroll
            for (int j = 0; j < VEC; ++j) g[j] = g[j] / inv;
          } else if (MODE == MRG_REDUCE_MAX) {
            IVec<VEC> a = IVec<VEC>::load(arg + v * D + c * VEC);
#pragma unroll
            for (int j = 0; j < VEC; ++j) g[j] = (a[j] == (int)r) ? g[j] : 0.f;
          }
          if (relu_src) {
            Vec<VEC> y = Vec<VEC>::load(relu_src + r * D + c * VEC);
#pragma unroll
            for (int j = 0; j < VEC; ++j) g[j] = y[j] > 0.f ? g[j] : 0.f;
          } else if (relu_bits) {
            const int bld = (D + 31) >> 5;
#pragma unroll
            for (int j = 0; j < VEC; ++j) {
              const int col = c * VEC + j;
              g[j] = ((relu_bits[r * bld + (col >> 5)] >> (col & 31)) & 1u) ? g[j] : 0.f;
            }
          }
        }
        g.store(o + c * VEC);
      }
    }
  }
}

__global__ __launch_bounds__(1024) void segmax_bwd_gx_k(const float* __restrict__ gout, const float* __restrict__ mx,
                                                      const int32_t* __restrict__ dst, const int32_t* __restrict__ arg,
                                                      const float* __restrict__ W, float* __restrict__ gmsg, float* __restrict__ gx,
                                                      const int32_t* __restrict__ order, int64_t E, int D, int Kin) {
  extern __shared__ __align__(16) float wl[];
  constexpr int THREADS = 1024, WAVES = THREADS / 64;
  const int tid = threadIdx.x, lane = tid & 63, wave = __builtin_amdgcn_readfirstlane(tid >> 6);
  const int n4 = D * Kin / 4;
  for (int i = tid; i < n4; i += THREADS) reinterpret_cast<float4*>(wl)[i] = reinterpret_cast<const float4*>(W)[i];
  __syncthreads();
  const float* __restrict__ wsrc = wl;
  const int dv = D >> 2, kv = Kin >> 2;
  const int64_t stride = (int64_t)gridDim.x * WAVES;
  auto edge_at = [&](int64_t p) -> int { const int64_t q = p < E ? p : E - 1; return order ? order[q] : (int)q; };
  const bool lv = lane < dv;
  auto load_row = [&](int64_t v, float4& g4, int4& a4, float4& x4) {
    g4 = make_float4(0.f, 0.f, 0.f, 0.f); a4 = make_int4(-1, -1, -1, -1); x4 = make_float4(1.f, 1.f, 1.f, 1.f);
    if (lv) {
      g4 = *reinterpret_cast<const float4*>(gout + v * D + lane * 4);
      a4 = *reinterpret_cast<const int4*>(arg + v * D + lane * 4);
      if (mx) x4 = *reinterpret_cast<const float4*>(mx + v * D + lane * 4);
    }
  };
  const int64_t first = (int64_t)blockIdx.x * WAVES + wave;
  if (first >= E) return;
  int r0 = __builtin_amdgcn_readfirstlane(edge_at(first));
  int r1 = __builtin_amdgcn_readfirstlane(edge_at(first + stride));
  int64_t v1 = __builtin_amdgcn_readfirstlane(dst[r1]);
  float4 g4, x4; int4 a4;
  load_row((int64_t)__builtin_amdgcn_readfirstlane(dst[r0]), g4, a4, x4);
  for (int64_t pos = first; pos < E; pos += stride) {
    const int r2 = __builtin_amdgcn_readfirstlane(edge_at(pos + 2 * stride));
    const int v2 = dst[r2];
    float4 gn, xn; int4 an;
    load_row(v1, gn, an, xn);
    const int r = r0;
    float m[4];
    m[0] = (a4.x == r && x4.x > 0.f) ? g4.x : 0.f;
    m[1] = (a4.y == r && x4.y > 0.f) ? g4.y : 0.f;
    m[2] = (a4.z == r && x4.z > 0.f) ? g4.z : 0.f;
    m[3] = (a4.w == r && x4.w > 0.f) ? g4.w : 0.f;
    if (lv && gmsg) *reinterpret_cast<float4*>(gmsg + (int64_t)r * D + lane * 4) = make_float4(m[0], m[1], m[2], m[3]);
    float4 acc = make_float4(0.f, 0.f, 0.f, 0.f);
#pragma unroll
    for (int j = 0; j < 4; ++j) {
      unsigned long long live = __ballot(m[j] != 0.f);
      while (live) {
        const int src = __builtin_amdgcn_readfirstlane((int)__builtin_ctzll(live));
        live &= live - 1;
        const float val = __int_as_float(__builtin_amdgcn_readlane(__float_as_int(m[j]), src));
        const int c = src * 4 + j;
        if (lane < kv) {
          const float4 w4 = *reinterpret_cast<const float4*>(wsrc + c * Kin + lane * 4);
          acc.x += val * w4.x; acc.y += val * w4.y; acc.z += val * w4.z; acc.w += val * w4.w;
        }
      }
    }
    if (lane < kv) *reinterpret_cast<float4*>(gx + (int64_t)r * Kin + lane * 4) = acc;
    g4 = gn; a4 = an; x4 = xn;
    r0 = r1; r1 = r2;
    v1 = __builtin_amdgcn_readfirstlane(v2);
  }
}

}

using namespace mrg;

extern "C" int mrg_segmax_bwd_input_ok(int D, int Kin) {
  return (D > 0 && Kin > 0 && D % 4 == 0 && Kin % 4 == 0 && D <= 256 && Kin <= 256 && (size_t)D * Kin * 4 <= 160 * 1024) ? 1 : 0;
}

extern "C" int mrg_segmax_bwd_input(const float* gout, const float* mx, const int32_t* dst, const int32_t* arg, const float* W, float* gmsg,
                                    float* gx, const int32_t* order, int64_t E, int64_t N, int D, int Kin, void* stream) {
  if (E < 0 || N < 0 || E >= ((int64_t)1 << 31)) return MRG_E_SHAPE;
  if (!mrg_segmax_bwd_input_ok(D, Kin)) return MRG_E_SHAPE;
  if (E == 0) return MRG_OK;
  if (!gout || !dst || !arg || !W || !gx) return MRG_E_NULLPTR;
  if (!aligned16(gout) || !aligned16(arg) || !aligned16(W) || !aligned16(gx) || !aligned16(gmsg) || !aligned16(mx)) return MRG_E_SHAPE;
  const size_t lds = (size_t)D * Kin * sizeof(float);
  (void)hipFuncSetAttribute(reinterpret_cast<const void*>(&segmax_bwd_gx_k), hipFuncAttributeMaxDynamicSharedMemorySize, (int)lds);
  int64_t grid = (E + 15) / 16;
  if (grid > 256) grid = 256;
  hipLaunchKernelGGL(segmax_bwd_gx_k, dim3((unsigned)grid), dim3(1024), lds, (hipStream_t)stream, gout, mx, dst, arg, W, gmsg, gx, order, E, D, Kin);
  MRG_LAUNCH_CHECK();
  return MRG_OK;
}

extern "C" int64_t mrg_seg_reduce_workspace_bytes(int64_t n_slots, int D) {
  if (n_slots < 0 || D <= 0) return 0;
  return (n_slots + 1) * (int64_t)D * 8 + 64;
}

static int seg_reduce_fwd_impl(int mode, const float* msg, const float* self_rows, const int32_t* eid,
                               const int32_t* chunk_node, const int32_t* chunk_start, const int32_t* chunk_end,
                               const int32_t* chunk_slot, int64_t n_chunks, const int32_t* hub_node,
                               const int32_t* hub_first, const int32_t* hub_count, int64_t n_hubs, int64_t n_slots,
                               const int32_t* in_degree, float* out, int32_t* arg, void* ws, int64_t N, int D,
                               void* stream, const int32_t* head_rowptr);

extern "C" int mrg_seg_reduce_fwd(int mode, const float* msg, const float* self_rows, const int32_t* eid,
                                  const int32_t* chunk_node, const int32_t* chunk_start, const int32_t* chunk_end,
                                  const int32_t* chunk_slot, int64_t n_chunks, const int32_t* hub_node,
                                  const int32_t* hub_first, const int32_t* hub_count, int64_t n_hubs, int64_t n_slots,
                                  const int32_t* in_degree, float* out, int32_t* arg, void* ws, int64_t N, int D,
                                  void* stream) {
  return seg_reduce_fwd_impl(mode, msg, self_rows, eid, chunk_node, chunk_start, chunk_end, chunk_slot, n_chunks, hub_node, hub_first,
                             hub_count, n_hubs, n_slots, in_degree, out, arg, ws, N, D, stream, nullptr);
}

extern "C" int mrg_seg_reduce_heads_fwd(int mode, const float* part, const float* self_rows, const int32_t* rowptr,
                                        const int32_t* chunk_node, const int32_t* chunk_start, const int32_t* chunk_end,
                                        const int32_t* chunk_slot, int64_t n_chunks, const int32_t* hub_node,
                                        const int32_t* hub_first, const int32_t* hub_count, int64_t n_hubs, int64_t n_slots,
                                        const int32_t* in_degree, float* out, void* ws, int64_t N, int D, void* stream) {
  if (mode != MRG_REDUCE_SUM && mode != MRG_REDUCE_MEAN) return MRG_E_ENUM;
  if (!rowptr) return MRG_E_NULLPTR;
  return seg_reduce_fwd_impl(mode, part, self_rows, nullptr, chunk_node, chunk_start, chunk_end, chunk_slot, n_chunks, hub_node, hub_first,
                             hub_count, n_hubs, n_slots, in_degree, out, nullptr, ws, N, D, stream, rowptr);
}

static int seg_reduce_fwd_impl(int mode, const float* msg, const float* self_rows, const int32_t* eid,
                               const int32_t* chunk_node, const int32_t* chunk_start, const int32_t* chunk_end,
                               const int32_t* chunk_slot, int64_t n_chunks, const int32_t* hub_node,
                               const int32_t* hub_first, const int32_t* hub_count, int64_t n_hubs, int64_t n_slots,
                               const int32_t* in_degree, float* out, int32_t* arg, void* ws, int64_t N, int D,
                               void* stream, const int32_t* head_rowptr) {
  if (mode < 0 || mode > 2) return MRG_E_ENUM;
  if (N < 0 || D <= 0 || n_chunks < N || n_hubs < 0 || n_slots < 0) return MRG_E_SHAPE;
  if (N == 0) return MRG_OK;
  if (!out || !chunk_node || !chunk_start || !chunk_end || !chunk_slot || !in_degree) return MRG_E_NULLPTR;
  if (mode == MRG_REDUCE_MAX && !arg) return MRG_E_NULLPTR;
  if (n_hubs > 0 && (!hub_node || !hub_first || !hub_count)) return MRG_E_NULLPTR;
  if (n_slots > 0 && !ws) return MRG_E_WORKSPACE;
  hipStream_t st = (hipStream_t)stream;
  float* ws_val = (float*)ws;
  int32_t* ws_arg = ws ? (int32_t*)((float*)ws + (n_slots + 1) * (int64_t)D) : nullptr;
  RowGeom g = row_geom(D, aligned16(msg) && aligned16(self_rows) && aligned16(out) && aligned16(arg) && aligned16(ws));
  if (!g.ok) return MRG_E_SHAPE;
  const int is_mean = mode == MRG_REDUCE_MEAN;
#define CALL(V, L, K)                                                                                                  \
  do {                                                                                                                 \
    int grid = grid_for(n_chunks, MRG_BLOCK / L);                                                                      \
    if (mode == MRG_REDUCE_MAX)                                                                                        \
      hipLaunchKernelGGL((seg_chunk_k<V, L, K, true>), dim3(grid), dim3(MRG_BLOCK), 0, st, msg, self_rows, eid, chunk_node, chunk_start, chunk_end, chunk_slot, n_chunks, in_degree, out, arg, ws_val, ws_arg, D, is_mean); \
    else if (head_rowptr)                                                                                              \
      hipLaunchKernelGGL((seg_chunk_k<V, L, K, false, true>), dim3(grid), dim3(MRG_BLOCK), 0, st, msg, self_rows, eid, chunk_node, chunk_start, chunk_end, chunk_slot, n_chunks, in_degree, out, arg, ws_val, ws_arg, D, is_mean, head_rowptr); \
    else                                                                                                               \
      hipLaunchKernelGGL((seg_chunk_k<V, L, K, false>), dim3(grid), dim3(MRG_BLOCK), 0, st, msg, self_rows, eid, chunk_node, chunk_start, chunk_end, chunk_slot, n_chunks, in_degree, out, arg, ws_val, ws_arg, D, is_mean); \
    if (n_hubs > 0) {                                                                                                  \
      int gh = n_hubs < 4096 ? (int)n_hubs : 4096;                                                                        \
      if (mode == MRG_REDUCE_MAX)                                                                                      \
        hipLaunchKernelGGL((seg_hub_k<V, L, K, true>), dim3(gh), dim3(MRG_BLOCK), 0, st, self_rows, hub_node, hub_first, hub_count, n_hubs, in_degree, out, arg, ws_val, ws_arg, D, is_mean); \
      else                                                                                                             \
        hipLaunchKernelGGL((seg_hub_k<V, L, K, false>), dim3(gh), dim3(MRG_BLOCK), 0, st, self_rows, hub_node, hub_first, hub_count, n_hubs, in_degree, out, arg, ws_val, ws_arg, D, is_mean); \
    }                                                                                                                  \
  } while (0)
  MRG_DISPATCH_GEOM(g, CALL);
#undef CALL
  MRG_LAUNCH_CHECK();
  return MRG_OK;
}

static int seg_reduce_bwd_impl(int mode, const float* gout, const int32_t* dst, const int32_t* in_degree, const int32_t* arg, float* gmsg,
                               float* gself, const float* relu_src, const unsigned* relu_bits, int64_t E, int64_t N, int D, void* stream,
                               const int32_t* order = nullptr);

extern "C" int mrg_seg_reduce_bwd_ordered(int mode, const float* gout, const int32_t* dst, const int32_t* in_degree, const int32_t* arg,
                                          float* gmsg, float* gself, const float* relu_src, const unsigned* relu_bits, const int32_t* order,
// ... 44 lines not shown
```

### mr-gnas_amd/functional/dense.py

```python
import weakref

import torch

from .. import _lib
from .._lib import ptr_array, call, f32c, ptr, require_hip, stream_of
from . import switches as SW
from ._base import Fork, _ws, _ws_bytes, same_rows
from .candidates import Candidate, Link, RowScale, wants_stats


class _DenseFilter(torch.autograd.Function):

    @staticmethod
    def forward(ctx, link, kind, s, s_in, norm, b0, b1, scale_edge, scale_self, *params):
        s, s_in, norm = f32c(s), f32c(s_in), f32c(norm)
        params = tuple(f32c(p) for p in params)
        require_hip(s, s_in, norm, *params)
        M, D = s.shape
        st = stream_of(s)
        out = torch.empty_like(s)
        gate = torch.empty_like(s) if kind == 0 else None
        ctx.link = link
        if link is not None:
            link.s, link.gate = s, (gate.detach() if gate is not None else None)
        K_ = 2 * D if s_in is not None else D
        ws3 = int(_lib.load().mrg_dense_filter3_workspace_bytes(D, K_)) if (SW.GROUPED_SEGMENTS and all(params[2 * i] is not None for i in range(3))) else 0
        if ws3 > 0:
            call("mrg_dense_filter_fwd3", (kind, ptr(s), ptr(s_in), ptr_array([params[0], params[2], params[4]]),
                                           ptr_array([params[1], params[3], params[5]]), ptr(norm), scale_edge, scale_self, ptr(out), ptr(gate),
                                           ptr(_ws(ws3, s)), b0, b1, M, D, st),
                 nbytes=4 * M * (K_ + D * (2 if kind == 0 else 1)), flops=2 * M * K_ * D)
            ctx.cfg = (kind, b0, b1, scale_edge, scale_self)
            ctx.save_for_backward(s, s_in, norm, gate, *params)
            return out
        segs = [(i, lo, hi, scale, edge) for i, (lo, hi, scale, edge) in
                enumerate(((0, b0, scale_edge, True), (b0, b1, scale_edge, True), (b1, M, scale_self, False))) if hi > lo]
        gws = [_ws(_ws_bytes("mrg_gemm_workspace_bytes", K_, D), s) for _ in segs]
        fork = Fork(s.device, len(segs) if M >= SW.FORK_MIN_ROWS else 1)
        for j, (i, lo, hi, scale, edge) in enumerate(segs):
            W, b = params[2 * i], params[2 * i + 1]
            rs = norm[lo:hi] if (edge and norm is not None) else None
            with fork.on(j):
                call("mrg_dense_filter_fwd", (kind, ptr(s[lo:hi]), ptr(s_in[lo:hi]) if s_in is not None else None, ptr(W), ptr(b),
                                              ptr(rs), scale, ptr(out[lo:hi]), ptr(gate[lo:hi]) if gate is not None else None,
                                              ptr(gws[j]), hi - lo, D, stream_of(s)),
                     nbytes=4 * (hi - lo) * (K_ + D * (2 if kind == 0 else 1)), flops=2 * (hi - lo) * K_ * D)
        fork.join()
        ctx.cfg = (kind, b0, b1, scale_edge, scale_self)
        ctx.save_for_backward(s, s_in, norm, gate, *params)
        return out

    @staticmethod
    def backward(ctx, g):
        s, s_in, norm, gate, *params = ctx.saved_tensors
        kind, b0, b1, scale_edge, scale_self = ctx.cfg
        g = f32c(g)
        M, D = s.shape
        st = stream_of(s)
        prescaled = ctx.link is not None and ctx.link.arrived(0, g, "dense filter")
        if prescaled and kind == 0:
            gs = ctx.link.gs_direct
            gs.record_stream(torch.cuda.current_stream())
        else:
            gs = torch.empty_like(s)
        gs_in = torch.empty_like(s) if s_in is not None else None
        K_ = 2 * D if s_in is not None else D
        lib = _lib.load()
        if SW.GROUPED_SEGMENTS and all(params[2 * i] is not None for i in range(3)):
            wsi, wsw = int(lib.mrg_linear_bwd_input3_workspace_bytes(D, D)), int(lib.mrg_linear_bwd_weight3_workspace_bytes(b0, b1, M, D, K_ - D, D))
            if wsi > 0 and wsw > 0:
                Ws = [params[0], params[2], params[4]]
                gWs = [torch.empty_like(W) for W in Ws]
                gbs = [torch.empty_like(params[2 * i + 1]) if params[2 * i + 1] is not None else None for i in range(3)]
                if prescaled:
                    dz = g
                else:
                    dz = torch.empty(M, D, dtype=torch.float32, device=s.device)
                    call("mrg_dense_filter_dz3", (kind, ptr(g), ptr(s), ptr(gate), ptr(norm), scale_edge, scale_self, ptr(dz), ptr(gs), b1, M, D, st),
                         nbytes=4 * M * D * (5 if kind == 0 else 2))
                gwork = dict(nbytes=4 * M * 2 * D + 12 * D * D, flops=2 * M * D * D)
                call("mrg_linear_bwd_input3", (ptr(dz), ptr_array(Ws), ptr(gs), ptr(_ws(wsi, s)), b0, b1, M, D, D, K_, int(kind == 0), st), **gwork)
                if s_in is not None:
                    call("mrg_linear_bwd_input3", (ptr(dz), ptr_array([W[:, D:] for W in Ws]), ptr(gs_in), ptr(_ws(wsi, s)), b0, b1, M, D, D, K_, 0, st),
                         **gwork)
                call("mrg_linear_bwd_weight3", (ptr(dz), ptr(s), ptr(s_in), ptr_array(gWs), ptr_array(gbs), ptr(_ws(wsw, s)), b0, b1, M, D, K_ - D, D, st),
                     nbytes=4 * M * (D + K_), flops=2 * M * K_ * D)
                grads = [t for pair in zip(gWs, gbs) for t in pair]
                return (None, None, gs, gs_in, None, None, None, None, None, *grads)
        grads = []
        segs = ((0, b0, scale_edge, True), (b0, b1, scale_edge, True), (b1, M, scale_self, False))
        work = []
        for i, (lo, hi, scale, edge) in enumerate(segs):
            W, b = params[2 * i], params[2 * i + 1]
            if W is None:
                grads += [None, None]
                continue
            rows = max(hi - lo, 0)
            gW = torch.empty_like(W)
            gb = torch.empty_like(b) if b is not None else None
            grads += [gW, gb]
            work.append(dict(W=W, gW=gW, gb=gb, rows=rows, sl=slice(lo, hi), scale=scale,
                             rs=norm[lo:hi] if (edge and norm is not None and rows > 0) else None,
                             dz=torch.empty(rows, D, dtype=torch.float32, device=s.device),
                             wt=_ws(_ws_bytes("mrg_linear_bwd_input_workspace_bytes", D, D), s),
                             wt2=_ws(_ws_bytes("mrg_linear_bwd_input_workspace_bytes", D, D), s) if s_in is not None else None,
                             ws=_ws(_ws_bytes("mrg_linear_bwd_weight_workspace_bytes", rows, K_, D), s)))
        fork = Fork(s.device, len(work) if M >= SW.FORK_MIN_ROWS else 1)
        share = max(1, min(3, sum(1 for w in work if w["rows"] > 0)))
        for j, w in enumerate(work):
            W, rows, sl = w["W"], w["rows"], w["sl"]
            with fork.on(j):
                st = stream_of(s)
                if prescaled:
                    w["dz"] = g[sl]
                else:
                    call("mrg_dense_filter_dz", (kind, ptr(g[sl]), ptr(s[sl]), ptr(gate[sl]) if gate is not None else None, ptr(w["rs"]),
                                                 w["scale"], ptr(w["dz"]), ptr(gs[sl]), rows, D, st), nbytes=4 * rows * D * (5 if kind == 0 else 2))
                gwork = dict(nbytes=4 * rows * 2 * D + 4 * D * D, flops=2 * rows * D * D)
                call("mrg_linear_bwd_input", (ptr(w["dz"]), ptr(W), ptr(gs[sl]), ptr(w["wt"]), rows, D, D, K_, int(kind == 0), st), **gwork)
                if s_in is not None:
                    call("mrg_linear_bwd_input", (ptr(w["dz"]), ptr(W[:, D:]), ptr(gs_in[sl]), ptr(w["wt2"]), rows, D, D, K_, 0, st), **gwork)
                call("mrg_linear_bwd_weight_share", (ptr(w["dz"]), ptr(s[sl]), ptr(s_in[sl]) if s_in is not None else None, ptr(w["gW"]),
                                                     ptr(w["gb"]), ptr(w["ws"]), rows, D, D if s_in is not None else 0, D, share, st),
                     nbytes=4 * rows * (D + K_), flops=2 * rows * K_ * D)
        fork.join()
        return (None, None, gs, gs_in, None, None, None, None, None, *grads)


class _FoldHalves(torch.autograd.Function):

    @staticmethod
    def forward(ctx, *Ws):
        Ws = tuple(f32c(W) for W in Ws)
        Ws3 = (Ws + (None, None, None))[:3]
        ref = next(W for W in Ws3 if W is not None)
        require_hip(*Ws3)
        D = ref.shape[0]
        buf = torch.empty(3, D, D, dtype=torch.float32, device=ref.device)
        call("mrg_fold_halves3", (ptr_array(Ws3), ptr(buf), D, stream_of(ref)), nbytes=12 * D * D * sum(W is not None for W in Ws3))
        ctx.meta = (D, [W is not None for W in Ws3], len(Ws), ref.device)
        return tuple(buf[i] if Ws3[i] is not None else None for i in range(len(Ws)))

    @staticmethod
    def backward(ctx, *gs):
        D, present, n, dev = ctx.meta
        src = [f32c(gs[i]) if (i < n and present[i] and gs[i] is not None) else None for i in range(3)]
        gWs = [torch.empty(D, 2 * D, dtype=torch.float32, device=dev) if (i < n and present[i]) else None for i in range(3)]
        ref = next(t for t in gWs if t is not None)
        call("mrg_unfold_halves3", (ptr_array(src), ptr_array(gWs), D, stream_of(ref)), nbytes=12 * D * D * sum(present))
        return tuple(gWs[:n])


def dense_filter_comp(kind, s, s_in, norm, b0, b1, W_in, b_in, W_out, b_out, W_self, b_self, self_scale, for_epilogue=False):
    if s_in is not None and same_rows(s, s_in):
        W_in, W_out, W_self = _FoldHalves.apply(W_in, W_out, W_self)
        s_in = None
    norm = f32c(norm)
    if norm is not None and norm.numel() < int(b1):
        raise _lib.MrgnasError(f"dense filter: edge norm has {norm.numel()} entries, the edge rows need {int(b1)}")
    fold = for_epilogue and SW.FOLD_ROW_SCALE and f32c(s).is_cuda and torch.is_grad_enabled()
    link = Link() if fold else None
    y = _DenseFilter.apply(link, kind, s, s_in, norm, int(b0), int(b1), 1.0 / 3.0, float(self_scale),
                           W_in, b_in, W_out, b_out, W_self, b_self)
    if fold and y.requires_grad:
        return Candidate("stored", y, link=link, slot=0, rowscale=RowScale(norm, int(b1), 1.0 / 3.0, float(self_scale), kind == 0))
    return y


class _DensePair(torch.autograd.Function):

    @staticmethod
    def forward(ctx, link, sums, s, s_in, norm, b0, b1, gate_only, *params):
        s, s_in, norm = f32c(s), f32c(s_in), f32c(norm)
        params = tuple(f32c(p) for p in params)
        require_hip(s, s_in, norm, *params)
        M, D = s.shape
        st = stream_of(s)
        K_ = 2 * D if s_in is not None else D
        ws3 = int(_lib.load().mrg_dense_filter3_workspace_bytes(D, K_))
        out_c, gate = torch.empty_like(s), torch.empty_like(s)
        out_d = gate if gate_only else torch.empty_like(s)
        dW, dB, cW = [params[0], params[2], params[4]], [params[1], params[3], params[5]], list(params[6:9])
        work = dict(flops=2 * M * K_ * D)
        wsp = _ws(ws3, s)
        args_d = (0, ptr(s), ptr(s_in), ptr_array(dW), ptr_array(dB), ptr(norm), 1.0 / 3.0, 1.0 / 3.0,
                  None if gate_only else ptr(out_d), ptr(gate), ptr(wsp), b0, b1, M, D, st)
        args_c = (1, ptr(s), ptr(s_in), ptr_array(cW), ptr_array([None, None, None]), ptr(norm), 1.0 / 3.0, 1.0, ptr(out_c), None,
                  ptr(wsp), b0, b1, M, D, st)
        for kind, args, nb in ((0, args_d, 4 * M * (K_ + (1 if gate_only else 2) * D)), (1, args_c, 4 * M * (K_ + D))):
            blocks = int(_lib.load().mrg_dense_filter3_colsum_blocks(kind, b0, b1, M, D, K_)) if sums is not None else 0
            if blocks > 0:
                part = _ws(blocks * 2 * D * 8, s)
                call("mrg_dense_filter_fwd3", args + (ptr(part), blocks), nbytes=nb + part.numel() + (4 * M * D if kind == 0 and gate_only else 0),
                     symbol="mrg_dense_filter_fwd3_colsum", **work)
                sums.append(_lib.ColSums(part, 0, blocks, 2 * D, M))
            else:
                call("mrg_dense_filter_fwd3", args, nbytes=nb, **work)
                if sums is not None:
                    sums.append(None)
        del wsp
        ctx.cfg = (b0, b1)
        ctx.save_for_backward(s, s_in, norm, gate, *params)
        ctx.link = link
        if link is not None:
            link.s, link.gate = s, gate.detach()
        return out_d, out_c

    @staticmethod
    def backward(ctx, g_d, g_c):
        s, s_in, norm, gate, *params = ctx.saved_tensors
        b0, b1 = ctx.cfg
        M, D = s.shape
        st = stream_of(s)
        g_d, g_c = f32c(g_d), f32c(g_c)
        pres = [ctx.link is not None and ctx.link.arrived(i, g, "dense filter pair") for i, g in enumerate((g_d, g_c))]
        K_ = 2 * D if s_in is not None else D
        dW, cW = [params[0], params[2], params[4]], list(params[6:9])
        if pres[0]:
            dz_d, gs = g_d, ctx.link.gs_direct
            gs.record_stream(torch.cuda.current_stream())
        else:
            dz_d, gs = torch.empty_like(s), torch.empty_like(s)
            call("mrg_dense_filter_dz3", (0, ptr(g_d), ptr(s), ptr(gate), ptr(norm), 1.0 / 3.0, 1.0 / 3.0, ptr(dz_d), ptr(gs), b1, M, D, st),
                 nbytes=4 * M * D * 5)
        if pres[1]:
            dz_c = g_c
        else:
            dz_c = torch.empty_like(s)
            call("mrg_dense_filter_dz3", (1, ptr(g_c), ptr(s), None, ptr(norm), 1.0 / 3.0, 1.0, ptr(dz_c), None, b1, M, D, st), nbytes=4 * M * D * 2)
        lib = _lib.load()
        wsp = int(lib.mrg_linear_bwd_input3_pair_workspace_bytes(D, D))
        gwork = dict(nbytes=4 * M * 3 * D + 24 * D * D, flops=4 * M * D * D)
        call("mrg_linear_bwd_input3_pair", (ptr(dz_d), ptr(dz_c), ptr_array(dW), ptr_array(cW), ptr(gs), ptr(_ws(wsp, s)), b0, b1, M, D, D, K_, 1, st),
             nbytes=4 * M * 4 * D + 24 * D * D, flops=4 * M * D * D)
        gs_in = None
        if s_in is not None:
            gs_in = torch.empty_like(s)
            call("mrg_linear_bwd_input3_pair", (ptr(dz_d), ptr(dz_c), ptr_array([W[:, D:] for W in dW]), ptr_array([W[:, D:] for W in cW]), ptr(gs_in),
                                                ptr(_ws(wsp, s)), b0, b1, M, D, D, K_, 0, st), **gwork)
        wsw = int(lib.mrg_linear_bwd_weight3_workspace_bytes(b0, b1, M, D, K_ - D, D))
        g_dW = [torch.empty_like(W) for W in dW]
        g_dB = [torch.empty_like(params[2 * i + 1]) for i in range(3)]
        g_cW = [torch.empty_like(W) for W in cW]
        wwork = dict(nbytes=4 * M * (D + K_), flops=2 * M * K_ * D)
        call("mrg_linear_bwd_weight3", (ptr(dz_d), ptr(s), ptr(s_in), ptr_array(g_dW), ptr_array(g_dB), ptr(_ws(wsw, s)), b0, b1, M, D, K_ - D, D, st), **wwork)
        call("mrg_linear_bwd_weight3", (ptr(dz_c), ptr(s), ptr(s_in), ptr_array(g_cW), ptr_array([None, None, None]), ptr(_ws(wsw, s)), b0, b1, M, D, K_ - D, D, st),
             **wwork)
        grads_d = [t for pair in zip(g_dW, g_dB) for t in pair]
        return (None, None, gs, gs_in, None, None, None, None, *grads_d, *g_cW)


def dense_pair_available(D, tied):
    if not (SW.DENSE_PAIR and SW.GROUPED_SEGMENTS):
        return False
    lib = _lib.load()
    K_ = D if tied else 2 * D
    return (int(lib.mrg_dense_filter3_workspace_bytes(D, K_)) > 0 and int(lib.mrg_linear_bwd_input3_pair_workspace_bytes(D, D)) > 0
            and int(lib.mrg_linear_bwd_weight3_workspace_bytes(1, 2, 3, D, K_ - D, D)) > 0)
_GATED_C = {}


def _gated_rowscale(norm, b1, M, scale_edge, scale_self, device):
    base = None if norm is None else (norm._base if norm._base is not None else norm)
    key = (None if norm is None else (norm.data_ptr(), norm._version), b1, M, scale_edge, scale_self, str(device))
    hit = _GATED_C.get(key)
    if hit is not None and (norm is None or hit[0]() is base):
        return hit[1]
    c = torch.empty(M, dtype=torch.float32, device=device)
    if norm is None:
        c[:b1] = scale_edge
    else:
        torch.mul(norm[:b1], scale_edge, out=c[:b1])
    c[b1:] = scale_self
    if len(_GATED_C) > 64:
        _GATED_C.clear()
    import weakref
    _GATED_C[key] = (weakref.ref(base) if base is not None else None, c)
    return c


def dense_filter_pair(s, s_in, norm, b0, b1, dense_params, comp_weights, gate_only=False, for_epilogue=False):
    dW, dB = list(dense_params[0::2]), list(dense_params[1::2])
    cW = list(comp_weights)
    if s_in is not None and same_rows(s, s_in):
        dW = list(_FoldHalves.apply(*dW))
        cW = list(_FoldHalves.apply(*cW))
        s_in = None
    norm = f32c(norm)
    if norm is not None and norm.numel() < int(b1):
        raise _lib.MrgnasError(f"dense filter: edge norm has {norm.numel()} entries, the edge rows need {int(b1)}")
    s = f32c(s)
    gate_only = bool(gate_only and for_epilogue and s.is_cuda)
    fold = for_epilogue and SW.FOLD_ROW_SCALE and s.is_cuda and torch.is_grad_enabled()
    link = Link(2) if fold else None
    sums = [] if (wants_stats(for_epilogue) and s.is_cuda) else None
    y_d, y_c = _DensePair.apply(link, sums, s, s_in, norm, int(b0), int(b1), gate_only, dW[0], dB[0], dW[1], dB[1], dW[2], dB[2], *cW)
    if not for_epilogue:
        return y_d, y_c
    fold = fold and y_d.requires_grad
    rs_d = RowScale(norm, int(b1), 1.0 / 3.0, 1.0 / 3.0, True) if fold else None
    rs_c = RowScale(norm, int(b1), 1.0 / 3.0, 1.0, False) if fold else None
    sums_d, sums_c = sums if sums else (None, None)
    if gate_only:
        c_d = Candidate("gate", y_d, link=link, slot=0, s=s, c=_gated_rowscale(norm, int(b1), s.shape[0], 1.0 / 3.0, 1.0 / 3.0, s.device), rowscale=rs_d,
                        sums=sums_d)
    else:
        c_d = Candidate("stored", y_d, link=link, slot=0, rowscale=rs_d, sums=sums_d)
    return c_d, Candidate("stored", y_c, link=link, slot=1, rowscale=rs_c, sums=sums_c)


def dense_filter_single(s, s_in, W, b):
    if s_in is not None and same_rows(s, s_in):
        (W,) = _FoldHalves.apply(W)
        s_in = None
    return _DenseFilter.apply(None, 0, s, s_in, None, 0, 0, 1.0, 1.0, None, None, None, None, W, b)
```

### mr-gnas_amd/functional/fanin.py

```python
import weakref

import torch

from .._lib import ptr_array, call, f32c, ptr, require_hip, stream_of
from .reducers import _seg_bwd


def sum_buffers(xs):
    xs = [f32c(x) for x in xs]
    require_hip(*xs)
    out = torch.empty_like(xs[0])
    n = out.numel()
    for i in range(0, len(xs), 8):
        part = xs[i:i + 8]
        call("mrg_sum_buffers", (ptr_array(part), len(part), ptr(out), n, int(i > 0), stream_of(out)),
             nbytes=4 * n * (len(part) + 1 + int(i > 0)))
    return out


class _Fanout(torch.autograd.Function):

    @staticmethod
    def forward(ctx, x, k, box):
        ctx.set_materialize_grads(False)
        ctx.box = box
        return tuple(x.view_as(x) for _ in range(k))

    @staticmethod
    def backward(ctx, *grads):
        gs = [g for g in grads if g is not None]
        gathered = ctx.box.gathered
        if gathered is not None:
            gh, gself, graph, ev = gathered
            ctx.box.gathered = None
            cur = torch.cuda.current_stream(gh.device)
            cur.wait_event(ev)
            for t in (gh, gself):
                if t is not None:
                    t.record_stream(cur)
            E, N, D = graph.num_edges(), graph.number_of_nodes(), gh.shape[1]
            if len(gs) <= 8 and all(g.is_cuda and g.shape == (E + N, D) for g in gs):
                gs = [f32c(g) for g in gs]
                out = torch.empty(E + N, D, dtype=torch.float32, device=gh.device)
                call("mrg_sum_rows_gather", (ptr_array(gs), len(gs), ptr(f32c(gh)), ptr(f32c(gself)), ptr(graph.i32("dst")), E, E + N, D, ptr(out),
                                             stream_of(out)), nbytes=4 * D * (E + N) * (len(gs) + 1))
                return out, None, None
            gx = torch.empty(E + N, D, dtype=torch.float32, device=gh.device)
            if gself is not None:
                gx[E:] = gself
            else:
                gx[E:].zero_()
            _seg_bwd(0, gh, graph, None, gx, None)
            gs.append(gx)
        if not gs:
            return None, None, None
        if len(gs) == 1:
            return gs[0], None, None
        if not gs[0].is_cuda or any(g.shape != gs[0].shape for g in gs):
            tot = gs[0]
            for g in gs[1:]:
                tot = tot + g
            return tot, None, None
        return sum_buffers(gs), None, None


class _FanBox:
    __slots__ = ("gathered",)

    def __init__(self):
        self.gathered = None


class Fan:

    BATCH = 12

    def __init__(self, x, cap):
        self.x = x
        self.left = cap
        self._live = torch.is_grad_enabled() and x.requires_grad and cap > 1
        self._views = []
        self._root = x

    def take(self):
        if not self._live:
            return self.x
        if self.left <= 0:
            raise RuntimeError("Fan: more readers than announced")
        self.left -= 1
        if not self._views:
            self._box = _FanBox()
            views = list(_Fanout.apply(self._root, self.BATCH, self._box))
            self._root = views.pop()
            self._views = views
        v = self._views.pop()
        Fan._remember(v, self._box)
        return v

    _NODE = {}

    @staticmethod
    def _remember(v, box):
        key = id(v)
        Fan._NODE[key] = (weakref.ref(v, lambda _r, key=key: Fan._NODE.pop(key, None)), box)

    @staticmethod
    def node_of(x):
        hit = Fan._NODE.get(id(x))
        return hit[1] if hit is not None and hit[0]() is x else None
```

### mr-gnas_amd/functional/gates.py

```python
import torch

from .. import _lib
from .._lib import ptr_array, call, f32c, ptr, require_hip, stream_of
from ._base import _ws, _ws_bytes, gate_ld, same_rows
from .candidates import Candidate, Link, wants_stats


class _Gate(torch.autograd.Function):

    @staticmethod
    def forward(ctx, s, s_in, norm, b0, b1, scale, *params):
        tied = s_in is not None and same_rows(s, s_in)
        s, s_in, norm = f32c(s), (None if tied else f32c(s_in)), f32c(norm)
        params = tuple(f32c(p) for p in params)
        require_hip(s, s_in, norm, *params)
        M, D = s.shape
        st = stream_of(s)
        in_dim = 2 * D if (s_in is not None or tied) else D
        Ws, bs, as_ = params[0::3], params[1::3], params[2::3]
        uvc = torch.empty(3, gate_ld(D), dtype=torch.float32, device=s.device)
        call("mrg_gate_collapse3", (ptr_array(Ws), ptr_array(bs), ptr_array(as_), ptr(uvc), D, in_dim, int(tied), st),
             nbytes=4 * D * in_dim * sum(W is not None for W in Ws))
        out = torch.empty_like(s)
        nb = 4 * D * M * (3 if s_in is not None else 2) + (4 * b1 if norm is not None else 0)
        call("mrg_gate_fwd", (ptr(s), ptr(s_in), ptr(norm), ptr(uvc), ptr(out), b0, b1, M, D, scale, st), nbytes=nb)
        ctx.save_for_backward(s, s_in, norm, uvc, *params)
        ctx.cfg = (b0, b1, scale, in_dim, tied)
        return out

    @staticmethod
    def backward(ctx, g):
        s, s_in, norm, uvc, *params = ctx.saved_tensors
        b0, b1, scale, in_dim, tied = ctx.cfg
        g = f32c(g)
        M, D = s.shape
        st = stream_of(s)
        gs = torch.empty_like(s)
        gs_in = torch.empty_like(s) if s_in is not None else None
        d_uvc = torch.empty(3, gate_ld(D), dtype=torch.float32, device=s.device)
        ws = _ws(_ws_bytes("mrg_gate_bwd_workspace_bytes", M, D), s)
        nb = 4 * D * M * (5 if s_in is not None else 3) + (4 * b1 if norm is not None else 0)
        call("mrg_gate_bwd", (ptr(g), ptr(s), ptr(s_in), ptr(norm), ptr(uvc), ptr(gs), ptr(gs_in), ptr(d_uvc), ptr(ws),
                              b0, b1, M, D, scale, st), nbytes=nb)
        Ws, bs, as_ = params[0::3], params[1::3], params[2::3]
        gWs = [None if W is None else torch.empty_like(W) for W in Ws]
        gbs = [None if b is None else torch.empty_like(b) for b in bs]
        gas = [None if a is None else torch.empty_like(a) for a in as_]
        call("mrg_gate_param_grad3", (ptr_array(Ws), ptr_array(bs), ptr_array(as_), ptr(d_uvc), ptr_array(gWs), ptr_array(gbs), ptr_array(gas),
                                      D, in_dim, int(tied), st), nbytes=8 * D * in_dim * sum(W is not None for W in Ws))
        gparams = []
        for gW, gb, ga in zip(gWs, gbs, gas):
            gparams += [gW, gb, ga]
        return (gs, gs_in, None, None, None, None, *gparams)


def gate_comp(s, s_in, norm, b0, b1, W_in, b_in, a_in, W_out, b_out, a_out, W_self, b_self, a_self):
    return _Gate.apply(s, s_in, norm, int(b0), int(b1), 1.0 / 3.0, W_in, b_in, a_in, W_out, b_out, a_out, W_self, b_self, a_self)


def gate_last(s, W, b, a):
    return _Gate.apply(s, None, None, 0, 0, 1.0, None, None, None, None, None, None, W, b, a)


class _GateRow(torch.autograd.Function):

    @staticmethod
    def forward(ctx, link, sums, s, s_in, norm, b0, b1, scale, *params):
        tied = s_in is not None and same_rows(s, s_in)
        s, s_in, norm = f32c(s), (None if tied else f32c(s_in)), f32c(norm)
        params = tuple(f32c(p) for p in params)
        require_hip(s, s_in, norm, *params)
        M, D = s.shape
        st = stream_of(s)
        in_dim = 2 * D if (s_in is not None or tied) else D
        Ws, bs, as_ = params[0::3], params[1::3], params[2::3]
        uvc = torch.empty(3, gate_ld(D), dtype=torch.float32, device=s.device)
        call("mrg_gate_collapse3", (ptr_array(Ws), ptr_array(bs), ptr_array(as_), ptr(uvc), D, in_dim, int(tied), st),
             nbytes=4 * D * in_dim * sum(W is not None for W in Ws))
        fvec = torch.empty(M, dtype=torch.float32, device=s.device)
        hvec = torch.empty(M, dtype=torch.float32, device=s.device)
        nb = 4 * D * M * (2 if s_in is not None else 1) + (4 * b1 if norm is not None else 0) + 8 * M
        args = (ptr(s), ptr(s_in), ptr(norm), ptr(uvc), ptr(fvec), ptr(hvec), b0, b1, M, D, scale, st)
        vec4 = D % 4 == 0 and all(t is None or t.data_ptr() % 16 == 0 for t in (s, s_in, uvc))
        blocks = int(_lib.load().mrg_gate_row_colsum_blocks(b0, b1, M, D, int(vec4))) if sums is not None else 0
        if blocks > 0:
            part = _ws(blocks * 4 * D * 8, s)
            call("mrg_gate_row_fwd", args + (ptr(part), blocks), nbytes=nb + part.numel(), symbol="mrg_gate_row_fwd_colsum")
            sums += [_lib.ColSums(part, 0, blocks, 4 * D, M), _lib.ColSums(part, 2 * D * 8, blocks, 4 * D, M)]
        else:
            call("mrg_gate_row_fwd", args, nbytes=nb)
        ctx.save_for_backward(s, s_in, norm, uvc, hvec, *params)
        ctx.cfg = (b0, b1, scale, in_dim, tied)
        ctx.link = link
        if link is not None:
            link.row_h, link.row_uvc = hvec, uvc
        return fvec

    @staticmethod
    def backward(ctx, gq):
        s, s_in, norm, uvc, hvec, *params = ctx.saved_tensors
        b0, b1, scale, in_dim, tied = ctx.cfg
        gq = f32c(gq)
        M, D = s.shape
        st = stream_of(s)
        gs_in = torch.empty_like(s) if s_in is not None else None
        d_uvc = torch.empty(3, gate_ld(D), dtype=torch.float32, device=s.device)
        ws = _ws(_ws_bytes("mrg_gate_bwd_workspace_bytes", M, D), s)
        nb = 4 * D * M * (3 if s_in is not None else 1) + 8 * M
        call("mrg_gate_row_bwd", (ptr(gq), ptr(hvec), ptr(s), ptr(s_in), ptr(uvc), ptr(gs_in), ptr(d_uvc), ptr(ws), b0, b1, M, D, st), nbytes=nb)
        Ws, bs, as_ = params[0::3], params[1::3], params[2::3]
        gWs = [None if W is None else torch.empty_like(W) for W in Ws]
        gbs = [None if b is None else torch.empty_like(b) for b in bs]
        gas = [None if a is None else torch.empty_like(a) for a in as_]
        call("mrg_gate_param_grad3", (ptr_array(Ws), ptr_array(bs), ptr_array(as_), ptr(d_uvc), ptr_array(gWs), ptr_array(gbs), ptr_array(gas),
                                      D, in_dim, int(tied), st), nbytes=8 * D * in_dim * sum(W is not None for W in Ws))
        gparams = []
        for gW, gb, ga in zip(gWs, gbs, gas):
            gparams += [gW, gb, ga]
        gs = None
        folded = ctx.link.row_written if ctx.link is not None else None
        if ctx.link is not None:
            ctx.link.row_written = None
        if folded is not None and folded != gq.data_ptr():
            raise _lib.MrgnasError("f_sparse_comp (row factor): the MixedOp epilogue folded the gradient w.r.t. s, but a different gradient "
                                   "tensor reached the factor's node -- the factor has a second consumer, which the folded form does not support")
        if folded is None:
            dz = gq * hvec
            gs = torch.empty_like(s)
            for seg, (lo, hi) in enumerate(((0, b0), (b0, b1), (b1, M))):
                if hi > lo:
                    torch.mul(dz[lo:hi, None], uvc[seg, :D][None, :], out=gs[lo:hi])
        return (None, None, gs, gs_in, None, None, None, None, *gparams)


def gate_comp_row_factor(s, s_in, norm, b0, b1, W_in, b_in, a_in, W_out, b_out, a_out, W_self, b_self, a_self, for_epilogue=True):
    s = f32c(s)
    link = Link()
    sums = [] if (wants_stats(for_epilogue) and s.is_cuda) else None
    fvec = _GateRow.apply(link, sums, s, s_in, norm, int(b0), int(b1), 1.0 / 3.0, W_in, b_in, a_in, W_out, b_out, a_out, W_self, b_self, a_self)
    s_sums, f_sums = sums if sums else (None, None)
    return Candidate("rowfactor", fvec, link=link, s=s, b0=int(b0), b1=int(b1), sums=f_sums, s_sums=s_sums)
```

### mr-gnas_amd/functional/reducers.py

```python
import os

import torch

from .. import _lib
from .._lib import call, f32c, ptr, require_hip, stream_of
from . import switches as SW
from ._base import REDUCE, _chunk_plan_args, _ws, _ws_bytes
from .gcs import span_gcs


def _seg_fwd(mode, msg, self_rows, p, N, D, want_arg=True):
    out = torch.empty(N, D, dtype=torch.float32, device=msg.device)
    arg = torch.empty(N, D, dtype=torch.int32, device=msg.device) if mode == 2 else None
    plan_args, ws = _chunk_plan_args(p, D, msg, "mrg_seg_reduce_workspace_bytes")
    E = int(p["eid"].numel())
    nb = 4 * D * E + 4 * E + 4 * D * N * (1 + (self_rows is not None) + (mode == 2))
    call("mrg_seg_reduce_fwd", (mode, ptr(msg), ptr(self_rows), ptr(p["eid"]), *plan_args, ptr(p["in_degree"]),
                                ptr(out), ptr(arg), ptr(ws), N, D, stream_of(msg)), nbytes=nb)
    return out, arg


def _heads_fwd(mode, part, self_rows, p, N, D):
    out = torch.empty(N, D, dtype=torch.float32, device=part.device)
    plan_args, ws = _chunk_plan_args(p, D, part, "mrg_seg_reduce_workspace_bytes")
    call("mrg_seg_reduce_heads_fwd", (mode, ptr(part), ptr(self_rows), ptr(p["rowptr"]), *plan_args, ptr(p["in_degree"]), ptr(out), ptr(ws),
                                      N, D, stream_of(part)), nbytes=8 * N * D + 4 * part.shape[0])
    return out


ORDERED_BWD = os.environ.get("MRG_SEG_BWD_ORDERED", "1") == "1"
ORDERED_BWD_MIN_BYTES = int(os.environ.get("MRG_SEG_BWD_ORDERED_MIN_BYTES", str(128 << 20)))


def _seg_bwd(mode, g, graph, arg, gmsg, gself, relu_src=None, relu_bits=None):
    p = graph.plan()
    E, N, D = graph.num_edges(), graph.number_of_nodes(), g.shape[1]
    nb = 4 * D * E * (1 + (relu_src is not None)) + 4 * E + 4 * D * N * (1 + (gself is not None) + (mode == 2))
    big = 4 * D * N * (2 if mode == 2 else 1) > ORDERED_BWD_MIN_BYTES
    order = p["eid"] if (ORDERED_BWD and g.is_cuda and big) else None
    call("mrg_seg_reduce_bwd_ordered", (mode, ptr(g), ptr(graph.i32("dst")), ptr(p["in_degree"]), ptr(arg), ptr(gmsg), ptr(gself),
                                        ptr(relu_src), ptr(relu_bits), ptr(order), E, N, D, stream_of(g)), nbytes=nb)



def _amax_bwd_sparse(g, mx, arg, W, graph, gy, gx):
    E, N, D = graph.num_edges(), graph.number_of_nodes(), g.shape[1]
    if not (SW.SPARSE_AMAX_BWD and g.is_cuda and _lib.load().mrg_segmax_bwd_input_ok(D, W.shape[1])):
        return False
    p = graph.plan()
    big = 4 * D * N * 3 > ORDERED_BWD_MIN_BYTES
    order = p["eid"] if (ORDERED_BWD and big) else None
    call("mrg_segmax_bwd_input", (ptr(g), ptr(mx), ptr(graph.i32("dst")), ptr(arg), ptr(W), ptr(gy), ptr(gx), ptr(order), E, N, D, W.shape[1],
                                  stream_of(g)), nbytes=4 * E * (D + W.shape[1]) + 4 * E + 12 * N * D)
    return True

class _SegReduce(torch.autograd.Function):
    @staticmethod
    def forward(ctx, mode, msg, self_rows, graph):
        msg, self_rows = f32c(msg), f32c(self_rows)
        require_hip(msg, self_rows)
        if msg.shape[0] != graph.num_edges():
            raise _lib.MrgnasError(f"message rows {msg.shape[0]} != number of edges {graph.num_edges()}")
        if mode != 2 and hasattr(graph, "agg_plan"):
            sp, meta = graph.agg_plan("mean" if mode == 1 else "sum")
            out, arg = span_gcs("copy", msg, None, meta, sp), None
            if self_rows is not None:
                out += self_rows
        else:
            out, arg = _seg_fwd(mode, msg, self_rows, graph.plan(), graph.number_of_nodes(), msg.shape[1])
        ctx.mode, ctx.graph, ctx.has_self = mode, graph, self_rows is not None
        ctx.save_for_backward(*((arg,) if arg is not None else ()))
        return out

    @staticmethod
    def backward(ctx, g):
        g = f32c(g)
        arg = ctx.saved_tensors[0] if ctx.mode == 2 else None
        gmsg = torch.empty(ctx.graph.num_edges(), g.shape[1], dtype=torch.float32, device=g.device)
        _seg_bwd(ctx.mode, g, ctx.graph, arg, gmsg, None)
        return None, gmsg, (g if ctx.has_self else None), None


def seg_reduce(kind, msg, self_rows, graph):
    return _SegReduce.apply(REDUCE[kind], msg, self_rows, graph)


class _AggRows(torch.autograd.Function):

    @staticmethod
    def forward(ctx, mode, x, graph, add_self, keep):
        x = f32c(x)
        require_hip(x, keep)
        E, N, D = graph.num_edges(), graph.number_of_nodes(), x.shape[1]
        if x.shape[0] != E + N:
            raise _lib.MrgnasError(f"expected {E + N} rows (E + N), got {x.shape[0]}")
        if mode != 2 and hasattr(graph, "agg_plan"):
            sp, meta = graph.agg_plan("mean" if mode == 1 else "sum")
            out, arg = span_gcs("copy", x, None, meta, sp), None
            if keep is not None:
                out *= keep
            if add_self:
                out += x[E:]
        else:
            out, arg = _seg_fwd(mode, x, x[E:] if (add_self and keep is None) else None, graph.plan(), N, D)
            if keep is not None:
                out *= keep
                if add_self:
                    out += x[E:]
        ctx.mode, ctx.graph, ctx.add_self = mode, graph, add_self
        ctx.save_for_backward(*[t for t in (arg, keep) if t is not None])
        ctx.has = (arg is not None, keep is not None)
        from .fanin import Fan
        ctx.fan_node = Fan.node_of(x) if (SW.LAZY_ASUM and mode == 0 and x.is_cuda) else None
        return out

    @staticmethod
    def backward(ctx, g):
        g = f32c(g)
        graph = ctx.graph
        saved = list(ctx.saved_tensors)
        arg = saved.pop(0) if ctx.has[0] else None
        keep = saved.pop(0) if ctx.has[1] else None
        E, N, D = graph.num_edges(), graph.number_of_nodes(), g.shape[1]
        gh = g * keep if keep is not None else g
        node = ctx.fan_node
        if node is not None and ctx.mode == 0 and node.gathered is None:
            ev = torch.cuda.Event()
            ev.record(torch.cuda.current_stream(g.device))
            node.gathered = (gh, g if ctx.add_self else None, graph, ev)
            return None, None, None, None, None
        gx = torch.empty(E + N, D, dtype=torch.float32, device=g.device)
        if ctx.add_self:
            gx[E:] = g
        else:
            gx[E:].zero_()
        _seg_bwd(ctx.mode, gh, graph, arg, gx, None)
        return None, gx, None, None, None


def aggregate_rows(kind, x, graph, add_self=True, keep=None):
    return _AggRows.apply(REDUCE[kind], x, graph, add_self, keep)


def _fused_agg_ws(N, D):
    return int(_lib.load().mrg_linear_relu_segmax_workspace_bytes(N, D, D))


def _lin_relu_forward(ctx, mode, x, W, b, graph, partial):
    x, W, b = f32c(x), f32c(W), f32c(b)
    require_hip(x, W, b)
    E, N, D = graph.num_edges(), graph.number_of_nodes(), x.shape[1]
    if not partial and x.shape[0] != E + N:
        raise _lib.MrgnasError(f"expected {E + N} rows (E + N), got {x.shape[0]}")
    st = stream_of(x)
    self_rows = None if partial else x[E:]
    ctx.mode, ctx.graph = mode, graph
    run_sums = mode != 2 if partial else (mode == 1 and hasattr(graph, "plan"))
    fused_ws = _fused_agg_ws(N, D) if (mode == 2 and SW.FUSED_AMAX and E >= SW.FUSED_AMAX_MIN_ROWS) else 0
    if fused_ws > 0:
        p = graph.plan()
        out = torch.empty(N, D, dtype=torch.float32, device=x.device)
        arg = torch.empty(N, D, dtype=torch.int32, device=x.device)
        mx = torch.empty(N, D, dtype=torch.float32, device=x.device)
        call("mrg_linear_relu_segmax_fwd", (ptr(x), ptr(W), ptr(b), ptr(p["eid"]), ptr(graph.i32("dst")), ptr(self_rows), ptr(out), ptr(arg),
                                            ptr(mx), ptr(_ws(fused_ws, x)), E, N, D, D, st),
             nbytes=4 * E * D + 8 * E + 4 * D * D + 4 * N * D * (3 if partial else 4), flops=2 * E * D * D)
        ctx.fused = True
        ctx.save_for_backward(x, W, arg, mx)
        if SW.MASK_TAP is not None:
            SW.MASK_TAP(("a_max", W.data_ptr()), [arg, mx > 0])
    elif run_sums and SW.FUSED_AMEAN and E >= SW.FUSED_AMAX_MIN_ROWS and _fused_agg_ws(N, D) > 0:
        p = graph.plan()
        part = torch.empty(E, D, dtype=torch.float32, device=x.device)
        bits = torch.empty(E, (D + 31) // 32, dtype=torch.int32, device=x.device)
        gws = _ws(_ws_bytes("mrg_gemm_workspace_bytes", D, D), x)
        call("mrg_linear_relu_segsum_fwd", (ptr(x), ptr(W), ptr(b), ptr(p["eid"]), ptr(graph.i32("dst")), ptr(part), ptr(bits), ptr(gws),
                                            E, D, D, st), nbytes=4 * E * D + 8 * E + 4 * D * D, flops=2 * E * D * D)
        ctx.fused = "sum" if partial else "mean"
        out = _heads_fwd(REDUCE[ctx.fused], part, self_rows, p, N, D)
        ctx.save_for_backward(x, W, bits)
        if SW.MASK_TAP is not None and not partial:
            SW.MASK_TAP(("a_mean", W.data_ptr()), [bits])
    else:
        y = torch.empty(E, D, dtype=torch.float32, device=x.device)
        gws = _ws(_ws_bytes("mrg_gemm_workspace_bytes", D, D), x)
        call("mrg_linear_fwd", (ptr(x), ptr(W), ptr(b), ptr(y), ptr(gws), E, D, D, 1, st),
             nbytes=4 * E * 2 * D + 4 * D * D, flops=2 * E * D * D)
        if mode == 2:
            out, arg = _seg_fwd(2, y, self_rows, graph.plan(), N, D)
        else:
            sp, meta = graph.agg_plan("mean" if (mode == 1 and not partial) else "sum")
            out, arg = span_gcs("copy", y, None, meta, sp), None
            if not partial:
                out += self_rows
        ctx.fused = False
        ctx.save_for_backward(x, W, y, *((arg,) if arg is not None else ()))
    return (out, x[E:].clone()) if partial else out


def _lin_relu_backward(ctx, g, gself, partial):
    graph, mode, fused = ctx.graph, ctx.mode, ctx.fused
    x, W, *saved = ctx.saved_tensors
    E, N, D = graph.num_edges(), graph.number_of_nodes(), x.shape[1]
    g = f32c(g) if g is not None else torch.zeros(N, D, dtype=torch.float32, device=x.device)
    st = stream_of(x)
    gx = torch.empty_like(x)
    gy = torch.empty(E, D, dtype=torch.float32, device=x.device)
    own = None
    if partial and gself is not None:
        gx[E:] = gself
    elif partial:
        gx[E:].zero_()
    elif fused is True:
        gx[E:] = g
    else:
        own = gx[E:]
    have_gx = False
    if fused is True:
        arg, mx = saved
        have_gx = _amax_bwd_sparse(g, mx, arg, W, graph, gy, gx)
        if not have_gx:
            _seg_bwd(mode, g * (mx > 0), graph, arg, gy, None)
    elif fused:
        _seg_bwd(REDUCE[fused], g, graph, None, gy, own, relu_bits=saved[0])
    else:
        y, *arg = saved
        _seg_bwd(mode, g, graph, arg[0] if arg else None, gy, own, relu_src=y)
    work = dict(nbytes=4 * E * 2 * D + 4 * D * D, flops=2 * E * D * D)
    if not have_gx:
        wt = _ws(_ws_bytes("mrg_linear_bwd_input_workspace_bytes", D, D), x)
        call("mrg_linear_bwd_input", (ptr(gy), ptr(W), ptr(gx), ptr(wt), E, D, D, D, 0, st), **work)
    gW = torch.empty_like(W)
    gb = torch.empty(D, dtype=torch.float32, device=x.device)
    ws = _ws(_ws_bytes("mrg_linear_bwd_weight_workspace_bytes", E, D, D), x)
    call("mrg_linear_bwd_weight", (ptr(gy), ptr(x), None, ptr(gW), ptr(gb), ptr(ws), E, D, 0, D, st), **work)
    return None, gx, gW, gb, None


class _LinReluAgg(torch.autograd.Function):

    @staticmethod
    def forward(ctx, mode, x, W, b, graph):
        return _lin_relu_forward(ctx, mode, x, W, b, graph, partial=False)

    @staticmethod
    def backward(ctx, g):
        return _lin_relu_backward(ctx, g, None, partial=False)


def linear_relu_aggregate(kind, x, W, b, graph):
    return _LinReluAgg.apply(REDUCE[kind], x, W, b, graph)


class _LinReluPartial(torch.autograd.Function):

    @staticmethod
    def forward(ctx, mode, x, W, b, graph):
        return _lin_relu_forward(ctx, mode, x, W, b, graph, partial=True)

    @staticmethod
    def backward(ctx, g, gself):
        return _lin_relu_backward(ctx, g, gself, partial=True)


def linear_relu_partial(kind, x, W, b, graph):
    return _LinReluPartial.apply(REDUCE[kind], x, W, b, graph)


class _SumPartial(torch.autograd.Function):

    @staticmethod
    def forward(ctx, x, graph):
        x = f32c(x)
        require_hip(x)
        E = graph.num_edges()
        sp, meta = graph.agg_plan("sum")
        ctx.graph = graph
        ctx.shape = x.shape
        return span_gcs("copy", x, None, meta, sp), x[E:].clone()

    @staticmethod
    def backward(ctx, g, gself):
        graph = ctx.graph
        E, D = graph.num_edges(), ctx.shape[1]
        gx = torch.empty(ctx.shape, dtype=torch.float32, device=(g if g is not None else gself).device)
        if gself is not None:
            gx[E:] = gself
        else:
            gx[E:].zero_()
        if g is not None:
            _seg_bwd(0, f32c(g), graph, None, gx, None)
        else:
            gx[:E].zero_()
        return gx, None


def sum_partial(x, graph):
    return _SumPartial.apply(x, graph)
```

### mr-gnas_amd/functional/switches.py

```python
import os

ROW_FACTOR = os.environ.get("MRG_ROW_FACTOR", "1") == "1"
LAZY_ASUM = os.environ.get("MRG_LAZY_ASUM", "1") == "1"
FUSED_AMAX = os.environ.get("MRG_FUSED_AMAX", "1") == "1"
FUSED_AMAX_MIN_ROWS = int(os.environ.get("MRG_FUSED_AMAX_MIN_ROWS", "100000"))
FUSED_AMEAN = os.environ.get("MRG_FUSED_AMEAN", "1") == "1"
WIDE_BWD_INPUT = os.environ.get("MRG_WIDE_BWD_INPUT", "1") == "1"
NODE_LINEAR = os.environ.get("MRG_NODE_LINEAR", "1") == "1"
MASK_TAP = None
FOLD_IDENTITY = os.environ.get("MRG_FOLD_IDENTITY", "1") == "1"
CELL_ZERO_FUSED = os.environ.get("MRG_CELL_ZERO_FUSED", "1") == "1"
FORK_MIN_ROWS = int(os.environ.get("MRG_FORK_MIN_ROWS", str(1 << 17)))
SEGMENT_STREAMS = int(os.environ.get("MRG_SEGMENT_STREAMS", "3"))
FOLD_ROW_SCALE = os.environ.get("MRG_FOLD_ROW_SCALE", "1") == "1"
GROUPED_SEGMENTS = os.environ.get("MRG_GROUPED_SEGMENTS", "1") == "1"
DENSE_PAIR = os.environ.get("MRG_DENSE_PAIR", "1") == "1"
GATED_RECOMPUTE = os.environ.get("MRG_GATED_RECOMPUTE", "1") == "1"
PRODUCER_STATS = os.environ.get("MRG_PRODUCER_STATS", "1") == "1"
COMPGCN_TAIL = os.environ.get("MRG_COMPGCN_TAIL", "1") == "1"
SPARSE_AMAX_BWD = os.environ.get("MRG_SPARSE_AMAX_BWD", "1") == "1"
CAND_LINEAR_GROUP = os.environ.get("MRG_CAND_LINEAR_GROUP", "1") == "1"
CCORR_PATH = None
```

Before: 11.73.

## Chain fan-in gradient accumulation into backward producer kernel epilogues

Adds accumulate variants of several backward kernels (linear bwd input, grouped bwd input, segmax sparse bwd, gate row bwd) that add a running gradient total in their epilogue. A fan-in join object lets each consumer's backward write straight into the shared total buffer, so separate gradient sums and temporary buffers are no longer needed. The intent is to cut extra memory passes and kernel launches when one activation feeds several candidate ops in the supernet. The cost is more complex autograd bookkeeping, stream/event handling for gathered tensors, and a fixed left-to-right summation order.

Measured after the change: 12.00 (median of 6 runs). +2.3%, better.

```diff
diff --git a/include/mrgnas.h b/include/mrgnas.h
--- a/include/mrgnas.h
+++ b/include/mrgnas.h
@@ -67,6 +67,8 @@
                             int64_t b0, int64_t b1, int64_t M, int D, float scale, void *stream, double *colsum, int64_t colsum_blocks);
 int mrg_gate_row_bwd(const float *q, const float *hvec, const float *s, const float *s_in, const float *uvc, float *gs_in, float *d_uvc,
                      void *ws, int64_t b0, int64_t b1, int64_t M, int D, void *stream);
+int mrg_gate_row_bwd_acc(const float *q, const float *hvec, const float *s, const float *s_in, const float *uvc, float *gs_in, float *d_uvc,
+                         void *ws, int64_t b0, int64_t b1, int64_t M, int D, void *stream, const float *total);
 
 int64_t mrg_seg_reduce_workspace_bytes(int64_t n_slots, int D);
 int mrg_seg_reduce_fwd(int mode, const float *msg, const float *self_rows,
@@ -86,6 +88,9 @@
 int mrg_segmax_bwd_input_ok(int D, int Kin);
 int mrg_segmax_bwd_input(const float *gout, const float *mx, const int32_t *dst, const int32_t *arg, const float *W, float *gmsg,
                          float *gx, const int32_t *order, int64_t E, int64_t N, int D, int Kin, void *stream);
+int mrg_segmax_bwd_input_chain(const float *gout, const float *mx, const int32_t *dst, const int32_t *arg, const float *W, float *gmsg,
+                               float *gx, const int32_t *order, int64_t E, int64_t N, int D, int Kin, void *stream,
+                               const float *total, const float *gh, const float *gself);
 
 int64_t mrg_seg_std_workspace_bytes(int64_t n_slots, int D);
 int mrg_seg_std_fwd(const float *msg, const int32_t *eid, const int32_t *chunk_node, const int32_t *chunk_start,
@@ -205,6 +210,8 @@
 int64_t mrg_linear_bwd_input_workspace_bytes(int K, int Nout);
 int mrg_linear_bwd_input(const float *gY, const float *W, float *gX, void *ws,
                          int64_t rows, int K, int Nout, int ldw, int accumulate, void *stream);
+int mrg_linear_bwd_input_acc2(const float *gY, const float *W, float *gX, void *ws,
+                              int64_t rows, int K, int Nout, int ldw, int accumulate, void *stream, const float *total);
 int64_t mrg_linear_bwd_weight_workspace_bytes(int64_t rows, int K, int Nout);
 int mrg_linear_bwd_weight(const float *gY, const float *X1, const float *X2, float *gW, float *gbias, void *ws,
                           int64_t rows, int K1, int K2, int Nout, void *stream);
@@ -231,6 +238,11 @@
 int mrg_linear_bwd_input3_pair(const float *gY1, const float *gY2, const float *const *W1, const float *const *W2, float *gX,
                                void *ws, int64_t b0, int64_t b1, int64_t M, int K, int Nout, int ldw, int accumulate,
                                void *stream);
+int mrg_linear_bwd_input3_acc2(const float *gY, const float *const *W, float *gX, void *ws, int64_t b0, int64_t b1, int64_t M,
+                               int K, int Nout, int ldw, int accumulate, void *stream, const float *total);
+int mrg_linear_bwd_input3_pair_acc2(const float *gY1, const float *gY2, const float *const *W1, const float *const *W2, float *gX,
+                                    void *ws, int64_t b0, int64_t b1, int64_t M, int K, int Nout, int ldw, int accumulate,
+                                    void *stream, const float *total);
 int64_t mrg_linear_bwd_weight3_workspace_bytes(int64_t b0, int64_t b1, int64_t M, int K1, int K2, int Nout);
 int mrg_linear_bwd_weight3(const float *gY, const float *X1, const float *X2, float *const *gW, float *const *gbias, void *ws,
                            int64_t b0, int64_t b1, int64_t M, int K1, int K2, int Nout, void *stream);
diff --git a/mr-gnas_amd/_lib.py b/mr-gnas_amd/_lib.py
--- a/mr-gnas_amd/_lib.py
+++ b/mr-gnas_amd/_lib.py
@@ -47,6 +47,7 @@
     "mrg_gate_row_colsum_blocks": (_L, [_L, _L, _L, _I, _I]),
     "mrg_gate_row_fwd_colsum": (_I, [_P, _P, _P, _P, _P, _P, _L, _L, _L, _I, _F, _P, _P, _L]),
     "mrg_gate_row_bwd": (_I, [_P, _P, _P, _P, _P, _P, _P, _P, _L, _L, _L, _I, _P]),
+    "mrg_gate_row_bwd_acc": (_I, [_P, _P, _P, _P, _P, _P, _P, _P, _L, _L, _L, _I, _P, _P]),
     "mrg_mix_workspace_bytes": (_L, [_I, _I]),
     "mrg_mix_colstats": (_I, [_P, _I, _L, _I, _P, _P, _P, _P]),
     "mrg_mix_finalize_fwd": (_I, [_P, _P, _P, _P, _P, _I, ctypes.c_double, _I, _F, _F, _P, _P]),
@@ -70,6 +71,7 @@
     "mrg_gemm_set_small": (_I, [_I]),
     "mrg_segmax_bwd_input_ok": (_I, [_I, _I]),
     "mrg_segmax_bwd_input": (_I, [_P, _P, _P, _P, _P, _P, _P, _P, _L, _L, _I, _I, _P]),
+    "mrg_segmax_bwd_input_chain": (_I, [_P, _P, _P, _P, _P, _P, _P, _P, _L, _L, _I, _I, _P, _P, _P, _P]),
     "mrg_seg_std_workspace_bytes": (_L, [_L, _I]),
     "mrg_seg_std_fwd": (_I, [_P, _P, _P, _P, _P, _P, _L, _P, _P, _P, _L, _L, _P, _P, _P, _P, _P, _L, _I, _P]),
     "mrg_seg_std_bwd": (_I, [_P, _P, _P, _P, _P, _P, _P, _L, _L, _I, _P]),
@@ -86,8 +88,10 @@
     "mrg_dense_filter_dz3": (_I, [_I, _P, _P, _P, _P, _F, _F, _P, _P, _L, _L, _I, _P]),
     "mrg_linear_bwd_input3_workspace_bytes": (_L, [_I, _I]),
     "mrg_linear_bwd_input3": (_I, [_P, _P, _P, _P, _L, _L, _L, _I, _I, _I, _I, _P]),
+    "mrg_linear_bwd_input3_acc2": (_I, [_P, _P, _P, _P, _L, _L, _L, _I, _I, _I, _I, _P, _P]),
     "mrg_linear_bwd_input3_pair_workspace_bytes": (_L, [_I, _I]),
     "mrg_linear_bwd_input3_pair": (_I, [_P, _P, _P, _P, _P, _P, _L, _L, _L, _I, _I, _I, _I, _P]),
+    "mrg_linear_bwd_input3_pair_acc2": (_I, [_P, _P, _P, _P, _P, _P, _L, _L, _L, _I, _I, _I, _I, _P, _P]),
     "mrg_linear_bwd_weight3_workspace_bytes": (_L, [_L, _L, _L, _I, _I, _I]),
     "mrg_linear_bwd_weight3": (_I, [_P, _P, _P, _P, _P, _P, _L, _L, _L, _I, _I, _I, _P]),
     "mrg_linear_relu_segsum_fwd": (_I, [_P, _P, _P, _P, _P, _P, _P, _P, _L, _I, _I, _P]),
@@ -98,6 +102,7 @@
     "mrg_linear_relu_segmax_fwd": (_I, [_P, _P, _P, _P, _P, _P, _P, _P, _P, _P, _L, _L, _I, _I, _P]),
     "mrg_linear_bwd_input_workspace_bytes": (_L, [_I, _I]),
     "mrg_linear_bwd_input": (_I, [_P, _P, _P, _P, _L, _I, _I, _I, _I, _P]),
+    "mrg_linear_bwd_input_acc2": (_I, [_P, _P, _P, _P, _L, _I, _I, _I, _I, _P, _P]),
     "mrg_linear_bwd_weight_workspace_bytes": (_L, [_L, _I, _I]),
     "mrg_linear_bwd_weight": (_I, [_P, _P, _P, _P, _P, _P, _L, _I, _I, _I, _P]),
     "mrg_linear_bwd_weight_share": (_I, [_P, _P, _P, _P, _P, _P, _L, _I, _I, _I, _I, _P]),
@@ -217,8 +222,15 @@
     print(f"[mrg] {name} {shown}", file=sys.stderr, flush=True)
 
 
+_CHAIN_FORMS = {(name, len(SIGNATURES[sym][1])): sym for name, sym in (
+    ("mrg_linear_bwd_input", "mrg_linear_bwd_input_acc2"), ("mrg_linear_bwd_input3", "mrg_linear_bwd_input3_acc2"),
+    ("mrg_linear_bwd_input3_pair", "mrg_linear_bwd_input3_pair_acc2"), ("mrg_segmax_bwd_input", "mrg_segmax_bwd_input_chain"),
+    ("mrg_gate_row_bwd", "mrg_gate_row_bwd_acc"))}
+_CHAIN_NAMES = frozenset(name for name, _ in _CHAIN_FORMS)
+
+
 def call(name, args, nbytes=0, flops=0, symbol=None):
-    sym = symbol or name
+    sym = symbol or (_CHAIN_FORMS.get((name, len(args)), name) if name in _CHAIN_NAMES else name)
     fn = _FN.get(sym)
     if fn is None:
         fn = _FN[sym] = getattr(load(), sym)
diff --git a/mr-gnas_amd/csrc/gate.hip b/mr-gnas_amd/csrc/gate.hip
--- a/mr-gnas_amd/csrc/gate.hip
+++ b/mr-gnas_amd/csrc/gate.hip
@@ -328,10 +328,18 @@
   }
 }
 
-template <int VEC, int LPR, int KMAX, bool HAS_IN>
+template <int VEC>
+__device__ __forceinline__ Vec<VEC> add_rounded(Vec<VEC> a, Vec<VEC> b) {
+#pragma clang fp contract(off)
+#pragma unroll
+  for (int j = 0; j < VEC; ++j) a[j] = a[j] + b[j];
+  return a;
+}
+
+template <int VEC, int LPR, int KMAX, bool HAS_IN, bool ACC = false>
 __global__ __launch_bounds__(MRG_BLOCK) void gate_row_bwd_k(const float* __restrict__ qv, const float* __restrict__ hv, const float* __restrict__ s,
                                                             const float* __restrict__ sin_, const float* __restrict__ uvc,
-                                                            float* __restrict__ gsin, float* __restrict__ ws, SegPlan p, int D) {
+                                                            float* gsin, float* __restrict__ ws, SegPlan p, int D, const float* tot = nullptr) {
   constexpr int RPB = MRG_BLOCK / LPR;
   constexpr int WIDTH = LPR * KMAX * VEC;
   __shared__ float red[RPB * (2 * WIDTH + 1)];
@@ -371,6 +379,7 @@
             o2[j] = dz * vk[k][j];
             dvv[k][j] += dz * xk[j];
           }
+          if (ACC) o2 = add_rounded(Vec<VEC>::load(tot + r * D + c * VEC), o2);
           o2.store(gsin + r * D + c * VEC);
         }
       }
@@ -650,16 +659,17 @@
   return gate_row_fwd(s, s_in, norm, uvc, fvec, hvec, b0, b1, M, D, scale, stream, colsum, colsum_blocks);
 }
 
-extern "C" int mrg_gate_row_bwd(const float* q, const float* hvec, const float* s, const float* s_in, const float* uvc, float* gs_in, float* d_uvc,
-                                void* ws, int64_t b0, int64_t b1, int64_t M, int D, void* stream) {
+static int gate_row_bwd(const float* q, const float* hvec, const float* s, const float* s_in, const float* uvc, float* gs_in, float* d_uvc,
+                        void* ws, int64_t b0, int64_t b1, int64_t M, int D, void* stream, const float* total) {
   if (D <= 0 || M < 0 || b0 < 0 || b1 < b0 || M < b1) return MRG_E_SHAPE;
   if (!uvc || !d_uvc) return MRG_E_NULLPTR;
   if (M > 0 && (!q || !hvec || !s)) return MRG_E_NULLPTR;
   if (s_in && !gs_in) return MRG_E_NULLPTR;
+  if (total && !s_in) return MRG_E_NULLPTR;
   if (!ws) return MRG_E_WORKSPACE;
   hipStream_t st = (hipStream_t)stream;
   const int ld = MRG_GATE_LD(D);
-  RowGeom g = row_geom(D, aligned16(s) && aligned16(s_in) && aligned16(gs_in) && aligned16(uvc));
+  RowGeom g = row_geom(D, aligned16(s) && aligned16(s_in) && aligned16(gs_in) && aligned16(uvc) && aligned16(total));
   if (!g.ok) return MRG_E_SHAPE;
   SegPlan p{};
 #define CALL(V, L, K)                                                                                                   \
@@ -668,8 +678,9 @@
     if (grid < 3) grid = 3;                                                                                             \
     p = make_plan(b0, b1, M, grid);                                                                                     \
     if (M > 0) {                                                                                                        \
-      if (s_in) hipLaunchKernelGGL((gate_row_bwd_k<V, L, K, true>), dim3(p.blk[3]), dim3(MRG_BLOCK), 0, st, q, hvec, s, s_in, uvc, gs_in, (float*)ws, p, D); \
-      else hipLaunchKernelGGL((gate_row_bwd_k<V, L, K, false>), dim3(p.blk[3]), dim3(MRG_BLOCK), 0, st, q, hvec, s, s_in, uvc, gs_in, (float*)ws, p, D); \
+      if (total) hipLaunchKernelGGL((gate_row_bwd_k<V, L, K, true, true>), dim3(p.blk[3]), dim3(MRG_BLOCK), 0, st, q, hvec, s, s_in, uvc, gs_in, (float*)ws, p, D, total); \
+      else if (s_in) hipLaunchKernelGGL((gate_row_bwd_k<V, L, K, true>), dim3(p.blk[3]), dim3(MRG_BLOCK), 0, st, q, hvec, s, s_in, uvc, gs_in, (float*)ws, p, D, nullptr); \
+      else hipLaunchKernelGGL((gate_row_bwd_k<V, L, K, false>), dim3(p.blk[3]), dim3(MRG_BLOCK), 0, st, q, hvec, s, s_in, uvc, gs_in, (float*)ws, p, D, nullptr); \
     }                                                                                                                   \
   } while (0)
   MRG_DISPATCH_GEOM(g, CALL);
@@ -679,3 +690,14 @@
   MRG_LAUNCH_CHECK();
   return MRG_OK;
 }
+
+extern "C" int mrg_gate_row_bwd(const float* q, const float* hvec, const float* s, const float* s_in, const float* uvc, float* gs_in, float* d_uvc,
+                                void* ws, int64_t b0, int64_t b1, int64_t M, int D, void* stream) {
+  return gate_row_bwd(q, hvec, s, s_in, uvc, gs_in, d_uvc, ws, b0, b1, M, D, stream, nullptr);
+}
+
+extern "C" int mrg_gate_row_bwd_acc(const float* q, const float* hvec, const float* s, const float* s_in, const float* uvc, float* gs_in, float* d_uvc,
+                                    void* ws, int64_t b0, int64_t b1, int64_t M, int D, void* stream, const float* total) {
+  if (!total) return MRG_E_NULLPTR;
+  return gate_row_bwd(q, hvec, s, s_in, uvc, gs_in, d_uvc, ws, b0, b1, M, D, stream, total);
+}
diff --git a/mr-gnas_amd/csrc/gemm.hpp b/mr-gnas_amd/csrc/gemm.hpp
--- a/mr-gnas_amd/csrc/gemm.hpp
+++ b/mr-gnas_amd/csrc/gemm.hpp
@@ -17,6 +17,8 @@
 enum { EPI_RANK = 8, EPI_RANK_DIAG = 9 };
 constexpr bool epi_diag(int epi) { return epi == EPI_RANK_DIAG; }
 enum { EPI_BCE = 10, EPI_BCE_GRAD = 11 };
+enum { EPI_ACCUM2 = 12 };
+constexpr bool epi_accum(int epi) { return epi == EPI_ACCUM || epi == EPI_ACCUM2; }
 
 struct GemmGroups {
   int n;
@@ -58,6 +60,7 @@
   GemmGroups grp;
 };
 
+inline void gemm_set_cin2(GemmArgs& a, const float* cin2, int ld) { a.S = cin2; a.ld_s = ld; }
 inline void gemm_set_colsum(GemmArgs& a, double* colsum) { a.seg_part = reinterpret_cast<float*>(colsum); }
 __host__ __device__ __forceinline__ double* gemm_colsum(const GemmArgs& a) { return reinterpret_cast<double*>(a.seg_part); }
 
@@ -436,6 +439,7 @@
   const int colw = col0 + li < a.N ? col0 + li : a.N - 1;
   float* crow[16];
   const float* srow[16];
+  const float* trow[16];
   float* xrow[16];
   float cs[16];
   bool rok[16];
@@ -447,7 +451,8 @@
     rok[r] = row <= last;
     crow[r] = a.C + (rowbase + rc) * a.ldc + colw;
     if (EPI == EPI_GATE) srow[r] = a.S + (rowbase + rc) * a.ld_s + colw;
-    if (EPI == EPI_ACCUM) srow[r] = a.Cin + (rowbase + rc) * a.ld_cin + colw;
+    if (epi_accum(EPI)) srow[r] = a.Cin + (rowbase + rc) * a.ld_cin + colw;
+    if (EPI == EPI_ACCUM2) trow[r] = a.S + (rowbase + rc) * a.ld_s + colw;
     if (EPI == EPI_GATE) xrow[r] = a.aux ? a.aux + (rowbase + rc) * a.N + colw : nullptr;
     cs[r] = 1.0f;
     if (EPI == EPI_GATE || EPI == EPI_SCALE) cs[r] = a.scale * (a.rowscale ? a.rowscale[rowbase + rc] : 1.0f);
@@ -458,12 +463,16 @@
     const bool cok = col < a.N;
     const int off = cok ? n * 32 : 0;
     const float bv = a.bias ? a.bias[cok ? col : colw] : 0.f;
-    float in[16], v[16], g[16];
+    float in[16], in2[16], v[16], g[16];
 #pragma unroll
     for (int r = 0; r < 16; ++r) in[r] = 0.f;
-    if ((EPI == EPI_GATE && (cstore || SUMS)) || EPI == EPI_ACCUM) {
+    if ((EPI == EPI_GATE && (cstore || SUMS)) || epi_accum(EPI)) {
 #pragma unroll
       for (int r = 0; r < 16; ++r) in[r] = srow[r][off];
+    }
+    if (EPI == EPI_ACCUM2) {
+#pragma unroll
+      for (int r = 0; r < 16; ++r) in2[r] = trow[r][off];
     }
 #pragma unroll
     for (int r = 0; r < 16; ++r) {
@@ -475,6 +484,8 @@
         v[r] = g[r] * in[r] * cs[r];
       } else if (EPI == EPI_SCALE) {
         v[r] = x * cs[r];
+      } else if (EPI == EPI_ACCUM2) {
+        v[r] = (x + in[r]) + in2[r];
       } else {
         v[r] = x + in[r];
       }
diff --git a/mr-gnas_amd/csrc/gemm_x3q.hpp b/mr-gnas_amd/csrc/gemm_x3q.hpp
--- a/mr-gnas_amd/csrc/gemm_x3q.hpp
+++ b/mr-gnas_amd/csrc/gemm_x3q.hpp
@@ -24,6 +24,7 @@
   const int colw = li < a.N ? li : a.N - 1;
   float* crow[8];
   const float* srow[8];
+  const float* trow[8];
   float* xrow[8];
   float cs[8];
   bool rok[8];
@@ -35,7 +36,8 @@
     rok[i] = row <= last;
     crow[i] = a.C + (rowbase + rc) * a.ldc + colw;
     if (EPI == EPI_GATE) srow[i] = a.S + (rowbase + rc) * a.ld_s + colw;
-    if (EPI == EPI_ACCUM) srow[i] = a.Cin + (rowbase + rc) * a.ld_cin + colw;
+    if (epi_accum(EPI)) srow[i] = a.Cin + (rowbase + rc) * a.ld_cin + colw;
+    if (EPI == EPI_ACCUM2) trow[i] = a.S + (rowbase + rc) * a.ld_s + colw;
     if (EPI == EPI_GATE) xrow[i] = a.aux ? a.aux + (rowbase + rc) * a.N + colw : nullptr;
     cs[i] = 1.0f;
     if (EPI == EPI_GATE || EPI == EPI_SCALE) cs[i] = a.scale * (a.rowscale ? a.rowscale[rowbase + rc] : 1.0f);
@@ -57,12 +59,16 @@
     const int col = j * 32 + li;
     const bool cok = col < a.N;
     const int off = cok ? j * 32 : 0;
-    float in[8], v[8], g[8];
+    float in[8], in2[8], v[8], g[8];
 #pragma unroll
     for (int i = 0; i < 8; ++i) in[i] = 0.f;
-    if ((EPI == EPI_GATE && (cstore || SUMS)) || EPI == EPI_ACCUM) {
+    if ((EPI == EPI_GATE && (cstore || SUMS)) || epi_accum(EPI)) {
 #pragma unroll
       for (int i = 0; i < 8; ++i) in[i] = srow[i][off];
+    }
+    if (EPI == EPI_ACCUM2) {
+#pragma unroll
+      for (int i = 0; i < 8; ++i) in2[i] = trow[i][off];
     }
 #pragma unroll
     for (int i = 0; i < 8; ++i) {
@@ -72,6 +78,8 @@
       } else if (EPI == EPI_GATE) {
         g[i] = sigmoidf_fast(x);
         v[i] = g[i] * in[i] * cs[i];
+      } else if (EPI == EPI_ACCUM2) {
+        v[i] = (x + in[i]) + in2[i];
       } else if (EPI == EPI_SCALE) {
         v[i] = x * cs[i];
       } else {
diff --git a/mr-gnas_amd/csrc/linear.hip b/mr-gnas_amd/csrc/linear.hip
--- a/mr-gnas_amd/csrc/linear.hip
+++ b/mr-gnas_amd/csrc/linear.hip
@@ -134,16 +134,43 @@
   return launch_gemm<EPI_BIAS_ACT>(a, 1, ldw, ws, st);
 }
 
+extern "C" int mrg_linear_bwd_input_acc2(const float* gY, const float* W, float* gX, void* ws, int64_t rows, int K, int Nout,
+                                         int ldw, int accumulate, void* stream, const float* total) {
+  if (rows < 0 || K <= 0 || Nout <= 0 || ldw < K) return MRG_E_SHAPE;
+  if (rows == 0) return MRG_OK;
+  if (!gY || !W || !gX || !total) return MRG_E_NULLPTR;
+  if (accumulate && total == gX) return MRG_E_SHAPE;
+  if (!ws) return MRG_E_WORKSPACE;
+  hipStream_t st = (hipStream_t)stream;
+  GemmArgs a{};
+  a.A1 = gY; a.K1 = Nout; a.B = W; a.C = gX; a.ldc = K; a.N = K; a.rows = rows; a.act = MRG_ACT_NONE;
+  if (accumulate) {
+    a.Cin = gX; a.ld_cin = K;
+    gemm_set_cin2(a, total, K);
+    return launch_gemm<EPI_ACCUM2>(a, 1, ldw, ws, st);
+  }
+  a.Cin = total; a.ld_cin = K;
+  return launch_gemm<EPI_ACCUM>(a, 1, ldw, ws, st);
+}
+
 static size_t bwd_input3_each(int K, int Nred) { return (size_t)(((int64_t)bsplit_bytes_any(K, Nred) + 255) / 256 * 256); }
 
 static int bwd_input3(const float* gY1, const float* gY2, const float* const* W1_host, const float* const* W2_host, float* gX, void* ws,
-                      int64_t b0, int64_t b1, int64_t M, int K, int Nout, int ldw, int accumulate, hipStream_t st) {
+                      int64_t b0, int64_t b1, int64_t M, int K, int Nout, int ldw, int accumulate, hipStream_t st,
+                      const float* total = nullptr) {
   const bool pair = gY2 != nullptr;
   const int Nred = pair ? 2 * Nout : Nout;
   GemmArgs a{};
   a.A1 = gY1; a.K1 = Nout; a.C = gX; a.ldc = K; a.N = K; a.rows = M; a.act = MRG_ACT_NONE;
   if (pair) { a.A2 = gY2; a.K2 = Nout; }
   if (accumulate) { a.Cin = gX; a.ld_cin = K; }
+  if (total && accumulate) {
+    if (total == gX) return MRG_E_SHAPE;
+    gemm_set_cin2(a, total, K);
+  } else if (total) {
+    a.Cin = total; a.ld_cin = K;
+  }
+  const int epi = total && accumulate ? EPI_ACCUM2 : (total || accumulate ? EPI_ACCUM : EPI_BIAS_ACT);
   if (!x3_eligible(a)) return MRG_E_SHAPE;
   const int64_t lo[3] = {0, b0, b1}, hi[3] = {b0, b1, M};
   const size_t each = bwd_input3_each(K, Nred);
@@ -159,9 +186,10 @@
     a.grp.lo[i] = lo[i]; a.grp.hi[i] = live ? hi[i] : lo[i];
     a.grp.scale[i] = 1.0f;
   }
-  launch_bsplit3_any(accumulate ? EPI_ACCUM : EPI_BIAS_ACT, M, Bs, 1, ldw, K, Nred, outs, st, pair ? Bs2 : nullptr, pair ? Nout : 0);
+  launch_bsplit3_any(epi, M, Bs, 1, ldw, K, Nred, outs, st, pair ? Bs2 : nullptr, pair ? Nout : 0);
   MRG_LAUNCH_CHECK();
-  if (accumulate) return launch_rowgemm_x3_mode<EPI_ACCUM>(a, outs[0], st);
+  if (epi == EPI_ACCUM2) return launch_rowgemm_x3_mode<EPI_ACCUM2>(a, outs[0], st);
+  if (epi == EPI_ACCUM) return launch_rowgemm_x3_mode<EPI_ACCUM>(a, outs[0], st);
   return launch_rowgemm_x3_mode<EPI_BIAS_ACT>(a, outs[0], st);
 }
 
@@ -180,6 +208,16 @@
   return bwd_input3(gY, nullptr, W_host, nullptr, gX, ws, b0, b1, M, K, Nout, ldw, accumulate, (hipStream_t)stream);
 }
 
+extern "C" int mrg_linear_bwd_input3_acc2(const float* gY, const float* const* W_host, float* gX, void* ws, int64_t b0, int64_t b1, int64_t M,
+                                          int K, int Nout, int ldw, int accumulate, void* stream, const float* total) {
+  if (K <= 0 || Nout <= 0 || ldw < K || M < 0 || b0 < 0 || b1 < b0 || M < b1) return MRG_E_SHAPE;
+  if (K <= 0 || Nout <= 48 || Nout % 4 != 0) return MRG_E_SHAPE;
+  if (M == 0) return MRG_OK;
+  if (!gY || !W_host || !gX || !total) return MRG_E_NULLPTR;
+  if (!ws) return MRG_E_WORKSPACE;
+  return bwd_input3(gY, nullptr, W_host, nullptr, gX, ws, b0, b1, M, K, Nout, ldw, accumulate, (hipStream_t)stream, total);
+}
+
 extern "C" int64_t mrg_linear_bwd_input3_pair_workspace_bytes(int K, int Nout) {
   if (K <= 0 || Nout <= 24 || Nout % 4 != 0 || gemm_mode() == 1) return 0;
   return 3 * (int64_t)bwd_input3_each(K, 2 * Nout);
@@ -193,3 +231,13 @@
   if (!ws) return MRG_E_WORKSPACE;
   return bwd_input3(gY1, gY2, W1_host, W2_host, gX, ws, b0, b1, M, K, Nout, ldw, accumulate, (hipStream_t)stream);
 }
+
+extern "C" int mrg_linear_bwd_input3_pair_acc2(const float* gY1, const float* gY2, const float* const* W1_host, const float* const* W2_host, float* gX,
+                                               void* ws, int64_t b0, int64_t b1, int64_t M, int K, int Nout, int ldw, int accumulate, void* stream,
+                                               const float* total) {
+  if (K <= 0 || Nout <= 24 || Nout % 4 != 0 || ldw < K || M < 0 || b0 < 0 || b1 < b0 || M < b1) return MRG_E_SHAPE;
+  if (M == 0) return MRG_OK;
+  if (!gY1 || !gY2 || !W1_host || !W2_host || !gX || !total) return MRG_E_NULLPTR;
+  if (!ws) return MRG_E_WORKSPACE;
+  return bwd_input3(gY1, gY2, W1_host, W2_host, gX, ws, b0, b1, M, K, Nout, ldw, accumulate, (hipStream_t)stream, total);
+}
diff --git a/mr-gnas_amd/csrc/segreduce.hip b/mr-gnas_amd/csrc/segreduce.hip
--- a/mr-gnas_amd/csrc/segreduce.hip
+++ b/mr-gnas_amd/csrc/segreduce.hip
@@ -120,10 +120,13 @@
   }
 }
 
+template <bool CHAIN>
 __global__ __launch_bounds__(1024) void segmax_bwd_gx_k(const float* __restrict__ gout, const float* __restrict__ mx,
                                                       const int32_t* __restrict__ dst, const int32_t* __restrict__ arg,
-                                                      const float* __restrict__ W, float* __restrict__ gmsg, float* __restrict__ gx,
-                                                      const int32_t* __restrict__ order, int64_t E, int D, int Kin) {
+                                                      const float* __restrict__ W, float* __restrict__ gmsg, float* gx,
+                                                      const int32_t* __restrict__ order, int64_t E, int D, int Kin,
+                                                      const float* total, const float* __restrict__ gh, const float* __restrict__ gself,
+                                                      int64_t N) {
   extern __shared__ __align__(16) float wl[];
   constexpr int THREADS = 1024, WAVES = THREADS / 64;
   const int tid = threadIdx.x, lane = tid & 63, wave = __builtin_amdgcn_readfirstlane(tid >> 6);
@@ -144,18 +147,44 @@
     }
   };
   const int64_t first = (int64_t)blockIdx.x * WAVES + wave;
-  if (first >= E) return;
+  auto self_rows = [&]() {
+    for (int64_t n = first; n < N; n += stride) {
+      if (lane < kv) {
+        const int64_t o = (E + n) * Kin + lane * 4;
+        float4 a = *reinterpret_cast<const float4*>(gout + n * D + lane * 4);
+        float4 t = make_float4(0.f, 0.f, 0.f, 0.f), h = t;
+        if (total) t = *reinterpret_cast<const float4*>(total + o);
+        if (gself) h = *reinterpret_cast<const float4*>(gself + n * Kin + lane * 4);
+        if (gself && total) { a.x = (h.x + t.x) + a.x; a.y = (h.y + t.y) + a.y; a.z = (h.z + t.z) + a.z; a.w = (h.w + t.w) + a.w; }
+        else if (gself) { a.x += h.x; a.y += h.y; a.z += h.z; a.w += h.w; }
+        else if (total) { a.x += t.x; a.y += t.y; a.z += t.z; a.w += t.w; }
+        *reinterpret_cast<float4*>(gx + o) = a;
+      }
+    }
+  };
+  if (first >= E) {
+    if constexpr (CHAIN) self_rows();
+    return;
+  }
   int r0 = __builtin_amdgcn_readfirstlane(edge_at(first));
   int r1 = __builtin_amdgcn_readfirstlane(edge_at(first + stride));
   int64_t v1 = __builtin_amdgcn_readfirstlane(dst[r1]);
+  int64_t v0 = __builtin_amdgcn_readfirstlane(dst[r0]);
   float4 g4, x4; int4 a4;
-  load_row((int64_t)__builtin_amdgcn_readfirstlane(dst[r0]), g4, a4, x4);
+  load_row(v0, g4, a4, x4);
   for (int64_t pos = first; pos < E; pos += stride) {
     const int r2 = __builtin_amdgcn_readfirstlane(edge_at(pos + 2 * stride));
     const int v2 = dst[r2];
     float4 gn, xn; int4 an;
     load_row(v1, gn, an, xn);
     const int r = r0;
+    float4 t4 = make_float4(0.f, 0.f, 0.f, 0.f), h4 = t4;
+    if constexpr (CHAIN) {
+      if (lane < kv) {
+        if (total) t4 = *reinterpret_cast<const float4*>(total + (int64_t)r * Kin + lane * 4);
+        if (gh) h4 = *reinterpret_cast<const float4*>(gh + v0 * Kin + lane * 4);
+      }
+    }
     float m[4];
     m[0] = (a4.x == r && x4.x > 0.f) ? g4.x : 0.f;
     m[1] = (a4.y == r && x4.y > 0.f) ? g4.y : 0.f;
@@ -177,11 +206,18 @@
         }
       }
     }
+    if constexpr (CHAIN) {
+      if (gh && total) { acc.x = (h4.x + t4.x) + acc.x; acc.y = (h4.y + t4.y) + acc.y; acc.z = (h4.z + t4.z) + acc.z; acc.w = (h4.w + t4.w) + acc.w; }
+      else if (gh) { acc.x += h4.x; acc.y += h4.y; acc.z += h4.z; acc.w += h4.w; }
+      else if (total) { acc.x += t4.x; acc.y += t4.y; acc.z += t4.z; acc.w += t4.w; }
+    }
     if (lane < kv) *reinterpret_cast<float4*>(gx + (int64_t)r * Kin + lane * 4) = acc;
     g4 = gn; a4 = an; x4 = xn;
     r0 = r1; r1 = r2;
+    v0 = v1;
     v1 = __builtin_amdgcn_readfirstlane(v2);
   }
+  if constexpr (CHAIN) self_rows();
 }
 
 }
@@ -192,20 +228,43 @@
   return (D > 0 && Kin > 0 && D % 4 == 0 && Kin % 4 == 0 && D <= 256 && Kin <= 256 && (size_t)D * Kin * 4 <= 160 * 1024) ? 1 : 0;
 }
 
+static int segmax_bwd_input(const float* gout, const float* mx, const int32_t* dst, const int32_t* arg, const float* W, float* gmsg,
+                            float* gx, const int32_t* order, int64_t E, int64_t N, int D, int Kin, void* stream, bool chain,
+                            const float* total, const float* gh, const float* gself) {
+  if (E < 0 || N < 0 || E >= ((int64_t)1 << 31)) return MRG_E_SHAPE;
+  if (!mrg_segmax_bwd_input_ok(D, Kin)) return MRG_E_SHAPE;
+  if (chain && D != Kin) return MRG_E_SHAPE;
+  const int64_t work = chain && N > E ? N : E;
+  if (work == 0) return MRG_OK;
+  if (!gout || !arg || !W || !gx || (E > 0 && !dst)) return MRG_E_NULLPTR;
+  if (gself && !gh) return MRG_E_NULLPTR;
+  if (!aligned16(gout) || !aligned16(arg) || !aligned16(W) || !aligned16(gx) || !aligned16(gmsg) || !aligned16(mx)) return MRG_E_SHAPE;
+  if (!aligned16(total) || !aligned16(gh) || !aligned16(gself)) return MRG_E_SHAPE;
+  const size_t lds = (size_t)D * Kin * sizeof(float);
+  int64_t grid = (work + 15) / 16;
+  if (grid > 256) grid = 256;
+  if (chain) {
+    (void)hipFuncSetAttribute(reinterpret_cast<const void*>(&segmax_bwd_gx_k<true>), hipFuncAttributeMaxDynamicSharedMemorySize, (int)lds);
+    hipLaunchKernelGGL(segmax_bwd_gx_k<true>, dim3((unsigned)grid), dim3(1024), lds, (hipStream_t)stream, gout, mx, dst, arg, W, gmsg, gx, order, E, D,
+                       Kin, total, gh, gself, N);
+  } else {
+    (void)hipFuncSetAttribute(reinterpret_cast<const void*>(&segmax_bwd_gx_k<false>), hipFuncAttributeMaxDynamicSharedMemorySize, (int)lds);
+    hipLaunchKernelGGL(segmax_bwd_gx_k<false>, dim3((unsigned)grid), dim3(1024), lds, (hipStream_t)stream, gout, mx, dst, arg, W, gmsg, gx, order, E, D,
+                       Kin, nullptr, nullptr, nullptr, N);
+  }
+  MRG_LAUNCH_CHECK();
+  return MRG_OK;
+}
+
 extern "C" int mrg_segmax_bwd_input(const float* gout, const float* mx, const int32_t* dst, const int32_t* arg, const float* W, float* gmsg,
                                     float* gx, const int32_t* order, int64_t E, int64_t N, int D, int Kin, void* stream) {
-  if (E < 0 || N < 0 || E >= ((int64_t)1 << 31)) return MRG_E_SHAPE;
-  if (!mrg_segmax_bwd_input_ok(D, Kin)) return MRG_E_SHAPE;
-  if (E == 0) return MRG_OK;
-  if (!gout || !dst || !arg || !W || !gx) return MRG_E_NULLPTR;
-  if (!aligned16(gout) || !aligned16(arg) || !aligned16(W) || !aligned16(gx) || !aligned16(gmsg) || !aligned16(mx)) return MRG_E_SHAPE;
-  const size_t lds = (size_t)D * Kin * sizeof(float);
-  (void)hipFuncSetAttribute(reinterpret_cast<const void*>(&segmax_bwd_gx_k), hipFuncAttributeMaxDynamicSharedMemorySize, (int)lds);
-  int64_t grid = (E + 15) / 16;
-  if (grid > 256) grid = 256;
-  hipLaunchKernelGGL(segmax_bwd_gx_k, dim3((unsigned)grid), dim3(1024), lds, (hipStream_t)stream, gout, mx, dst, arg, W, gmsg, gx, order, E, D, Kin);
-  MRG_LAUNCH_CHECK();
-  return MRG_OK;
+  return segmax_bwd_input(gout, mx, dst, arg, W, gmsg, gx, order, E, N, D, Kin, stream, false, nullptr, nullptr, nullptr);
+}
+
+extern "C" int mrg_segmax_bwd_input_chain(const float* gout, const float* mx, const int32_t* dst, const int32_t* arg, const float* W, float* gmsg,
+                                          float* gx, const int32_t* order, int64_t E, int64_t N, int D, int Kin, void* stream,
+                                          const float* total, const float* gh, const float* gself) {
+  return segmax_bwd_input(gout, mx, dst, arg, W, gmsg, gx, order, E, N, D, Kin, stream, true, total, gh, gself);
 }
 
 extern "C" int64_t mrg_seg_reduce_workspace_bytes(int64_t n_slots, int D) {
diff --git a/mr-gnas_amd/functional/dense.py b/mr-gnas_amd/functional/dense.py
--- a/mr-gnas_amd/functional/dense.py
+++ b/mr-gnas_amd/functional/dense.py
@@ -7,12 +7,30 @@
 from . import switches as SW
 from ._base import Fork, _ws, _ws_bytes, same_rows
 from .candidates import Candidate, Link, RowScale, wants_stats
+from .fanin import Fan, join
+
+
+def _bwd_input3(name, head, tail, gX, accumulate, jn, **work):
+    st = stream_of(gX if gX is not None else jn.total)
+    if jn is None or jn.total is None:
+        call(name, (*head, ptr(gX), *tail, accumulate, st), **work)
+        if jn is None:
+            return gX
+        jn.deposit(gX)
+        return None
+    tot = jn.total
+    out = gX if accumulate else tot
+    work["nbytes"] = work.get("nbytes", 0) + 4 * tot.numel()
+    call(name, (*head, ptr(out), *tail, accumulate, st, ptr(tot)), **work)
+    jn.deposit(out)
+    return None
 
 
 class _DenseFilter(torch.autograd.Function):
 
     @staticmethod
     def forward(ctx, link, kind, s, s_in, norm, b0, b1, scale_edge, scale_self, *params):
+        ctx.fan = (Fan.node_of(s), Fan.node_of(s_in))
         s, s_in, norm = f32c(s), f32c(s_in), f32c(norm)
         params = tuple(f32c(p) for p in params)
         require_hip(s, s_in, norm, *params)
@@ -62,8 +80,7 @@
             gs = ctx.link.gs_direct
             gs.record_stream(torch.cuda.current_stream())
         else:
-            gs = torch.empty_like(s)
-        gs_in = torch.empty_like(s) if s_in is not None else None
+            gs = torch.empty_like(s) if kind == 0 else None
         K_ = 2 * D if s_in is not None else D
         lib = _lib.load()
         if SW.GROUPED_SEGMENTS and all(params[2 * i] is not None for i in range(3)):
@@ -79,14 +96,24 @@
                     call("mrg_dense_filter_dz3", (kind, ptr(g), ptr(s), ptr(gate), ptr(norm), scale_edge, scale_self, ptr(dz), ptr(gs), b1, M, D, st),
                          nbytes=4 * M * D * (5 if kind == 0 else 2))
                 gwork = dict(nbytes=4 * M * 2 * D + 12 * D * D, flops=2 * M * D * D)
-                call("mrg_linear_bwd_input3", (ptr(dz), ptr_array(Ws), ptr(gs), ptr(_ws(wsi, s)), b0, b1, M, D, D, K_, int(kind == 0), st), **gwork)
+                jn = join(ctx.fan[0], s)
+                if kind != 0 and (jn is None or jn.total is None):
+                    gs = torch.empty_like(s)
+                gs = _bwd_input3("mrg_linear_bwd_input3", (ptr(dz), ptr_array(Ws)), (ptr(_ws(wsi, s)), b0, b1, M, D, D, K_), gs, int(kind == 0), jn,
+                                 **gwork)
+                gs_in = None
                 if s_in is not None:
-                    call("mrg_linear_bwd_input3", (ptr(dz), ptr_array([W[:, D:] for W in Ws]), ptr(gs_in), ptr(_ws(wsi, s)), b0, b1, M, D, D, K_, 0, st),
-                         **gwork)
+                    jn = join(ctx.fan[1], s)
+                    gs_in = torch.empty_like(s) if (jn is None or jn.total is None) else None
+                    gs_in = _bwd_input3("mrg_linear_bwd_input3", (ptr(dz), ptr_array([W[:, D:] for W in Ws])), (ptr(_ws(wsi, s)), b0, b1, M, D, D, K_),
+                                        gs_in, 0, jn, **gwork)
                 call("mrg_linear_bwd_weight3", (ptr(dz), ptr(s), ptr(s_in), ptr_array(gWs), ptr_array(gbs), ptr(_ws(wsw, s)), b0, b1, M, D, K_ - D, D, st),
                      nbytes=4 * M * (D + K_), flops=2 * M * K_ * D)
                 grads = [t for pair in zip(gWs, gbs) for t in pair]
                 return (None, None, gs, gs_in, None, None, None, None, None, *grads)
+        if gs is None:
+            gs = torch.empty_like(s)
+        gs_in = torch.empty_like(s) if s_in is not None else None
         grads = []
         segs = ((0, b0, scale_edge, True), (b0, b1, scale_edge, True), (b1, M, scale_self, False))
         work = []
@@ -171,6 +198,7 @@
 
     @staticmethod
     def forward(ctx, link, sums, s, s_in, norm, b0, b1, gate_only, *params):
+        ctx.fan = (Fan.node_of(s), Fan.node_of(s_in))
         s, s_in, norm = f32c(s), f32c(s_in), f32c(norm)
         params = tuple(f32c(p) for p in params)
         require_hip(s, s_in, norm, *params)
@@ -231,13 +259,14 @@
         lib = _lib.load()
         wsp = int(lib.mrg_linear_bwd_input3_pair_workspace_bytes(D, D))
         gwork = dict(nbytes=4 * M * 3 * D + 24 * D * D, flops=4 * M * D * D)
-        call("mrg_linear_bwd_input3_pair", (ptr(dz_d), ptr(dz_c), ptr_array(dW), ptr_array(cW), ptr(gs), ptr(_ws(wsp, s)), b0, b1, M, D, D, K_, 1, st),
-             nbytes=4 * M * 4 * D + 24 * D * D, flops=4 * M * D * D)
+        gs = _bwd_input3("mrg_linear_bwd_input3_pair", (ptr(dz_d), ptr(dz_c), ptr_array(dW), ptr_array(cW)), (ptr(_ws(wsp, s)), b0, b1, M, D, D, K_),
+                         gs, 1, join(ctx.fan[0], s), nbytes=4 * M * 4 * D + 24 * D * D, flops=4 * M * D * D)
         gs_in = None
         if s_in is not None:
-            gs_in = torch.empty_like(s)
-            call("mrg_linear_bwd_input3_pair", (ptr(dz_d), ptr(dz_c), ptr_array([W[:, D:] for W in dW]), ptr_array([W[:, D:] for W in cW]), ptr(gs_in),
-                                                ptr(_ws(wsp, s)), b0, b1, M, D, D, K_, 0, st), **gwork)
+            jn = join(ctx.fan[1], s)
+            gs_in = torch.empty_like(s) if (jn is None or jn.total is None) else None
+            gs_in = _bwd_input3("mrg_linear_bwd_input3_pair", (ptr(dz_d), ptr(dz_c), ptr_array([W[:, D:] for W in dW]), ptr_array([W[:, D:] for W in cW])),
+                                (ptr(_ws(wsp, s)), b0, b1, M, D, D, K_), gs_in, 0, jn, **gwork)
         wsw = int(lib.mrg_linear_bwd_weight3_workspace_bytes(b0, b1, M, D, K_ - D, D))
         g_dW = [torch.empty_like(W) for W in dW]
         g_dB = [torch.empty_like(params[2 * i + 1]) for i in range(3)]
diff --git a/mr-gnas_amd/functional/fanin.py b/mr-gnas_amd/functional/fanin.py
--- a/mr-gnas_amd/functional/fanin.py
+++ b/mr-gnas_amd/functional/fanin.py
@@ -3,6 +3,7 @@
 import torch
 
 from .._lib import ptr_array, call, f32c, ptr, require_hip, stream_of
+from . import switches as SW
 from .reducers import _seg_bwd
 
 
@@ -28,11 +29,20 @@
 
     @staticmethod
     def backward(ctx, *grads):
+        box = ctx.box
         gs = [g for g in grads if g is not None]
-        gathered = ctx.box.gathered
+        tot = box.take_total(None)
+        box.spent = True
+        return _Fanout._sum(box, gs, tot), None, None
+
+    @staticmethod
+    def _sum(box, gs, tot):
+        if tot is not None:
+            gs = [tot] + gs
+        gathered = box.gathered
         if gathered is not None:
             gh, gself, graph, ev = gathered
-            ctx.box.gathered = None
+            box.gathered = None
             cur = torch.cuda.current_stream(gh.device)
             cur.wait_event(ev)
             for t in (gh, gself):
@@ -44,7 +54,7 @@
                 out = torch.empty(E + N, D, dtype=torch.float32, device=gh.device)
                 call("mrg_sum_rows_gather", (ptr_array(gs), len(gs), ptr(f32c(gh)), ptr(f32c(gself)), ptr(graph.i32("dst")), E, E + N, D, ptr(out),
                                              stream_of(out)), nbytes=4 * D * (E + N) * (len(gs) + 1))
-                return out, None, None
+                return out
             gx = torch.empty(E + N, D, dtype=torch.float32, device=gh.device)
             if gself is not None:
                 gx[E:] = gself
@@ -53,22 +63,73 @@
             _seg_bwd(0, gh, graph, None, gx, None)
             gs.append(gx)
         if not gs:
-            return None, None, None
+            return None
         if len(gs) == 1:
-            return gs[0], None, None
+            return gs[0]
         if not gs[0].is_cuda or any(g.shape != gs[0].shape for g in gs):
-            tot = gs[0]
+            out = gs[0]
             for g in gs[1:]:
-                tot = tot + g
-            return tot, None, None
-        return sum_buffers(gs), None, None
+                out = out + g
+            return out
+        return sum_buffers(gs)
+
+
+_RAW_STREAM = torch._C._cuda_getCurrentRawStream
+
+
+def _graph_task():
+    return torch._C._current_graph_task_id()
 
 
 class _FanBox:
-    __slots__ = ("gathered",)
+    __slots__ = ("gathered", "total", "spent")
 
     def __init__(self):
         self.gathered = None
+        self.total = None
+        self.spent = False
+
+    def take_total(self, like):
+        if self.total is None:
+            return None
+        buf, stream, task = self.total
+        if task != _graph_task():
+            self.total = None
+            return None
+        if like is not None and (buf.shape != like.shape or buf.device != like.device or buf.dtype != like.dtype):
+            return None
+        self.total = None
+        if stream is not None and _RAW_STREAM(buf.get_device()) != stream:
+            cur = torch.cuda.current_stream(buf.device)
+            ev = torch.cuda.Event()
+            ev.record(torch.cuda.ExternalStream(stream, device=buf.device))
+            cur.wait_event(ev)
+            buf.record_stream(cur)
+        return buf
+
+    def deposit(self, buf):
+        self.total = (buf, _RAW_STREAM(buf.get_device()) if buf.is_cuda else None, _graph_task())
+
+
+class _Join:
+    __slots__ = ("box", "total")
+
+    def __init__(self, box, total):
+        self.box, self.total = box, total
+
+    def deposit(self, buf):
+        self.box.deposit(buf)
+
+
+def join(box, like, absorbs_gather=False):
+    if box is None or not SW.FANIN_CHAIN or box.spent or not like.is_cuda or torch.is_grad_enabled() or _graph_task() < 0:
+        return None
+    if box.gathered is not None and not absorbs_gather:
+        return None
+    tot = box.take_total(like)
+    if tot is None and box.total is not None:
+        return None
+    return _Join(box, tot)
 
 
 class Fan:
diff --git a/mr-gnas_amd/functional/gates.py b/mr-gnas_amd/functional/gates.py
--- a/mr-gnas_amd/functional/gates.py
+++ b/mr-gnas_amd/functional/gates.py
@@ -4,6 +4,7 @@
 from .._lib import ptr_array, call, f32c, ptr, require_hip, stream_of
 from ._base import _ws, _ws_bytes, gate_ld, same_rows
 from .candidates import Candidate, Link, wants_stats
+from .fanin import Fan, join
 
 
 class _Gate(torch.autograd.Function):
@@ -66,6 +67,7 @@
 
     @staticmethod
     def forward(ctx, link, sums, s, s_in, norm, b0, b1, scale, *params):
+        ctx.fan_in = Fan.node_of(s_in)
         tied = s_in is not None and same_rows(s, s_in)
         s, s_in, norm = f32c(s), (None if tied else f32c(s_in)), f32c(norm)
         params = tuple(f32c(p) for p in params)
@@ -103,11 +105,20 @@
         gq = f32c(gq)
         M, D = s.shape
         st = stream_of(s)
-        gs_in = torch.empty_like(s) if s_in is not None else None
+        jn = join(ctx.fan_in, s) if s_in is not None else None
+        tot = jn.total if jn is not None else None
+        gs_in = tot if tot is not None else (torch.empty_like(s) if s_in is not None else None)
         d_uvc = torch.empty(3, gate_ld(D), dtype=torch.float32, device=s.device)
         ws = _ws(_ws_bytes("mrg_gate_bwd_workspace_bytes", M, D), s)
         nb = 4 * D * M * (3 if s_in is not None else 1) + 8 * M
-        call("mrg_gate_row_bwd", (ptr(gq), ptr(hvec), ptr(s), ptr(s_in), ptr(uvc), ptr(gs_in), ptr(d_uvc), ptr(ws), b0, b1, M, D, st), nbytes=nb)
+        args = (ptr(gq), ptr(hvec), ptr(s), ptr(s_in), ptr(uvc), ptr(gs_in), ptr(d_uvc), ptr(ws), b0, b1, M, D, st)
+        if tot is not None:
+            call("mrg_gate_row_bwd", args + (ptr(tot),), nbytes=nb + 4 * D * M)
+        else:
+            call("mrg_gate_row_bwd", args, nbytes=nb)
+        if jn is not None:
+            jn.deposit(gs_in)
+            gs_in = None
         Ws, bs, as_ = params[0::3], params[1::3], params[2::3]
         gWs = [None if W is None else torch.empty_like(W) for W in Ws]
         gbs = [None if b is None else torch.empty_like(b) for b in bs]
diff --git a/mr-gnas_amd/functional/reducers.py b/mr-gnas_amd/functional/reducers.py
--- a/mr-gnas_amd/functional/reducers.py
+++ b/mr-gnas_amd/functional/reducers.py
@@ -43,15 +43,25 @@
 
 
 
-def _amax_bwd_sparse(g, mx, arg, W, graph, gy, gx):
+def _amax_bwd_ok(g, W):
+    return bool(SW.SPARSE_AMAX_BWD and g.is_cuda and _lib.load().mrg_segmax_bwd_input_ok(g.shape[1], W.shape[1]))
+
+
+def _amax_bwd_sparse(g, mx, arg, W, graph, gy, gx, chain=None):
     E, N, D = graph.num_edges(), graph.number_of_nodes(), g.shape[1]
-    if not (SW.SPARSE_AMAX_BWD and g.is_cuda and _lib.load().mrg_segmax_bwd_input_ok(D, W.shape[1])):
+    if not _amax_bwd_ok(g, W):
         return False
     p = graph.plan()
     big = 4 * D * N * 3 > ORDERED_BWD_MIN_BYTES
     order = p["eid"] if (ORDERED_BWD and big) else None
-    call("mrg_segmax_bwd_input", (ptr(g), ptr(mx), ptr(graph.i32("dst")), ptr(arg), ptr(W), ptr(gy), ptr(gx), ptr(order), E, N, D, W.shape[1],
-                                  stream_of(g)), nbytes=4 * E * (D + W.shape[1]) + 4 * E + 12 * N * D)
+    args = (ptr(g), ptr(mx), ptr(graph.i32("dst")), ptr(arg), ptr(W), ptr(gy), ptr(gx), ptr(order), E, N, D, W.shape[1], stream_of(g))
+    nb = 4 * E * (D + W.shape[1]) + 4 * E + 12 * N * D
+    if chain is None:
+        call("mrg_segmax_bwd_input", args, nbytes=nb)
+    else:
+        total, gh, gself = chain
+        nb += 8 * N * D + (4 * (E + N) * D if total is not None else 0) + 4 * N * D * ((gh is not None) + (gself is not None))
+        call("mrg_segmax_bwd_input", args + (ptr(total), ptr(gh), ptr(gself)), nbytes=nb)
     return True
 
 class _SegReduce(torch.autograd.Function):
@@ -112,6 +122,7 @@
         ctx.has = (arg is not None, keep is not None)
         from .fanin import Fan
         ctx.fan_node = Fan.node_of(x) if (SW.LAZY_ASUM and mode == 0 and x.is_cuda) else None
+        ctx.box = Fan.node_of(x) if x.is_cuda else None
         return out
 
     @staticmethod
@@ -135,6 +146,14 @@
         else:
             gx[E:].zero_()
         _seg_bwd(ctx.mode, gh, graph, arg, gx, None)
+        from .fanin import join
+        jn = join(ctx.box, gx)
+        if jn is not None:
+            if jn.total is not None:
+                call("mrg_sum_buffers", (_lib.ptr_array([gx]), 1, ptr(jn.total), gx.numel(), 1, stream_of(gx)), nbytes=12 * gx.numel())
+                gx = jn.total
+            jn.deposit(gx)
+            gx = None
         return None, gx, None, None, None
 
 
@@ -147,6 +166,8 @@
 
 
 def _lin_relu_forward(ctx, mode, x, W, b, graph, partial):
+    from .fanin import Fan
+    ctx.fan_node = Fan.node_of(x) if x.is_cuda else None
     x, W, b = f32c(x), f32c(W), f32c(b)
     require_hip(x, W, b)
     E, N, D = graph.num_edges(), graph.number_of_nodes(), x.shape[1]
@@ -204,36 +225,63 @@
     E, N, D = graph.num_edges(), graph.number_of_nodes(), x.shape[1]
     g = f32c(g) if g is not None else torch.zeros(N, D, dtype=torch.float32, device=x.device)
     st = stream_of(x)
-    gx = torch.empty_like(x)
+    from .fanin import join
+    sparse = fused is True and _amax_bwd_ok(g, W)
+    jn = join(ctx.fan_node, x, absorbs_gather=sparse) if not partial else None
+    tot = jn.total if jn is not None else None
+    gx = tot if tot is not None else torch.empty_like(x)
     gy = torch.empty(E, D, dtype=torch.float32, device=x.device)
-    own = None
-    if partial and gself is not None:
-        gx[E:] = gself
-    elif partial:
-        gx[E:].zero_()
-    elif fused is True:
-        gx[E:] = g
+    have_gx = False
+    if jn is not None and sparse:
+        gat = ctx.fan_node.gathered
+        gh = gs_ = None
+        if gat is not None and gat[2] is graph and gat[0].shape == (N, D):
+            gh, gs_, _, ev = gat
+            ctx.fan_node.gathered = None
+            cur = torch.cuda.current_stream(x.device)
+            cur.wait_event(ev)
+            for t in (gh, gs_):
+                if t is not None:
+                    t.record_stream(cur)
+        arg, mx = saved
+        have_gx = _amax_bwd_sparse(g, mx, arg, W, graph, gy, gx, chain=(tot, f32c(gh), f32c(gs_)))
     else:
-        own = gx[E:]
-    have_gx = False
-    if fused is True:
-        arg, mx = saved
-        have_gx = _amax_bwd_sparse(g, mx, arg, W, graph, gy, gx)
-        if not have_gx:
-            _seg_bwd(mode, g * (mx > 0), graph, arg, gy, None)
-    elif fused:
-        _seg_bwd(REDUCE[fused], g, graph, None, gy, own, relu_bits=saved[0])
-    else:
-        y, *arg = saved
-        _seg_bwd(mode, g, graph, arg[0] if arg else None, gy, own, relu_src=y)
+        own = None
+        if tot is not None:
+            gx[E:] += g
+        elif partial and gself is not None:
+            gx[E:] = gself
+        elif partial:
+            gx[E:].zero_()
+        elif fused is True:
+            gx[E:] = g
+        else:
+            own = gx[E:]
+        if fused is True:
+            arg, mx = saved
+            have_gx = tot is None and _amax_bwd_sparse(g, mx, arg, W, graph, gy, gx)
+            if not have_gx:
+                _seg_bwd(mode, g * (mx > 0), graph, arg, gy, None)
+        elif fused:
+            _seg_bwd(REDUCE[fused], g, graph, None, gy, own, relu_bits=saved[0])
+        else:
+            y, *arg = saved
+            _seg_bwd(mode, g, graph, arg[0] if arg else None, gy, own, relu_src=y)
     work = dict(nbytes=4 * E * 2 * D + 4 * D * D, flops=2 * E * D * D)
     if not have_gx:
         wt = _ws(_ws_bytes("mrg_linear_bwd_input_workspace_bytes", D, D), x)
-        call("mrg_linear_bwd_input", (ptr(gy), ptr(W), ptr(gx), ptr(wt), E, D, D, D, 0, st), **work)
+        if tot is not None:
+            call("mrg_linear_bwd_input", (ptr(gy), ptr(W), ptr(gx), ptr(wt), E, D, D, D, 0, st, ptr(gx)),
+                 nbytes=work["nbytes"] + 4 * E * D, flops=work["flops"])
+        else:
+            call("mrg_linear_bwd_input", (ptr(gy), ptr(W), ptr(gx), ptr(wt), E, D, D, D, 0, st), **work)
     gW = torch.empty_like(W)
     gb = torch.empty(D, dtype=torch.float32, device=x.device)
     ws = _ws(_ws_bytes("mrg_linear_bwd_weight_workspace_bytes", E, D, D), x)
     call("mrg_linear_bwd_weight", (ptr(gy), ptr(x), None, ptr(gW), ptr(gb), ptr(ws), E, D, 0, D, st), **work)
+    if jn is not None:
+        jn.deposit(gx)
+        gx = None
     return None, gx, gW, gb, None
 
 
diff --git a/mr-gnas_amd/functional/switches.py b/mr-gnas_amd/functional/switches.py
--- a/mr-gnas_amd/functional/switches.py
+++ b/mr-gnas_amd/functional/switches.py
@@ -2,6 +2,7 @@
 
 ROW_FACTOR = os.environ.get("MRG_ROW_FACTOR", "1") == "1"
 LAZY_ASUM = os.environ.get("MRG_LAZY_ASUM", "1") == "1"
+FANIN_CHAIN = os.environ.get("MRG_FANIN_CHAIN", "1") == "1"
 FUSED_AMAX = os.environ.get("MRG_FUSED_AMAX", "1") == "1"
 FUSED_AMAX_MIN_ROWS = int(os.environ.get("MRG_FUSED_AMAX_MIN_ROWS", "100000"))
 FUSED_AMEAN = os.environ.get("MRG_FUSED_AMEAN", "1") == "1"
```
